# SpectacularAI/3dgs-deblur

Hardware: AMD Instinct MI355X
Metric: fwd+bwd rasterize MPix/s at 1M Gaussians, 1080p, 5 sub-poses (higher is better)
Workload: dtype f32

## Files before the change

### 3dgs-deblur_amd/csrc/binning.hip

```cpp
#include <algorithm>
#include <atomic>
#include "gs_common.h"

namespace gs {

constexpr int kScanItems = 8;
constexpr int kScanBlock = 256 * kScanItems;

__device__ __forceinline__ unsigned block_excl_scan(unsigned v, unsigned& total, unsigned* lds ) {
  const int lane = lane_id(), wave = threadIdx.x >> 6;
  unsigned inc = v;
#pragma unroll
  for (int o = 1; o < 64; o <<= 1) {
    unsigned t = __shfl_up(inc, o);
    if (lane >= o) inc += t;
  }
  if (lane == 63) lds[wave] = inc;
  __syncthreads();
  unsigned w0 = lds[0], w1 = lds[1], w2 = lds[2], w3 = lds[3];
  unsigned woff = wave == 0 ? 0u : (wave == 1 ? w0 : (wave == 2 ? w0 + w1 : w0 + w1 + w2));
  total = w0 + w1 + w2 + w3;
  __syncthreads();
  return woff + inc - v;
}
// ... 961 lines not shown
        Ellipse el2;
        el2.gx = s_gx[a]; el2.gy = s_gy[a]; el2.a = s_a[a]; el2.b = s_b[a]; el2.c = s_c[a]; el2.tau = s_tau[a];
        ellipse_derive(el2);
        if (!tile_hit(el2, tx, ty, W, H)) key = invalid_key;
      }
      keys[e] = key;
      vals[e] = s_gi[a];
    }
  }
}

template <typename KeyT, int SHIFT>
__global__ __launch_bounds__(256) void bin_edges_kernel(size_t n, const KeyT* __restrict__ keys,
                                                        int2* __restrict__ bins, unsigned num_bins,
                                                        const unsigned* __restrict__ n_dev = nullptr) {
  if (n_dev) n = min(n, (size_t)*n_dev);
  const int2 z = make_int2(0, 0);
  if (n == 0) {
    for (size_t b = (size_t)blockIdx.x * 256 + threadIdx.x; b < num_bins; b += (size_t)gridDim.x * 256) bins[b] = z;
    return;
  }
  const int lane = lane_id();
  for (size_t base = (size_t)blockIdx.x * 256 + (threadIdx.x & ~63u); base < n; base += (size_t)gridDim.x * 256) {
    const size_t i = base + lane;
    const bool valid = i < n;
    unsigned t = 0, lo = 0, hi = 0;
    if (valid) {
      t = min((unsigned)(keys[i] >> SHIFT), num_bins);
      if (i == 0) {
        if (t < num_bins) bins[t].x = 0;
        hi = t;
      } else {
        const unsigned tp = min((unsigned)(keys[i - 1] >> SHIFT), num_bins);
        if (tp != t) {
          if (t < num_bins) bins[t].x = (int)i;
          if (tp < num_bins) bins[tp].y = (int)i;
          lo = min(tp + 1u, num_bins); hi = t;
        }
      }
      if (i == n - 1 && t < num_bins) bins[t].y = (int)n;
    }
    unsigned long long m = __ballot(hi > lo);
    while (m) {
      const int src = __ffsll((long long)m) - 1;
      m &= m - 1;
      const unsigned g_lo = (unsigned)readlane_i((int)lo, src), g_hi = (unsigned)readlane_i((int)hi, src);
      for (unsigned b = g_lo + lane; b < g_hi; b += 64) bins[b] = z;
    }
    const unsigned long long last = __ballot(valid && i == n - 1);
    if (last) {
      const unsigned g_lo = min((unsigned)readlane_i((int)t, __ffsll((long long)last) - 1) + 1u, num_bins);
      for (unsigned b = g_lo + lane; b < num_bins; b += 64) bins[b] = z;
    }
  }
}

__global__ __launch_bounds__(256) void bin_edges_ids_kernel(size_t n, const unsigned* __restrict__ keys,
                                                            int2* __restrict__ bins,
                                                            const unsigned* __restrict__ sorted_vals,
                                                            const unsigned* __restrict__ gi_of_e,
                                                            unsigned* __restrict__ ids) {
  size_t i = (size_t)blockIdx.x * 256 + threadIdx.x;
  if (i >= n) {
    if (i < n + 8) ids[i] = 0u;
    return;
  }
  ids[i] = gi_of_e[sorted_vals[i]];
  unsigned t = keys[i];
  if (i == 0) {
    bins[t].x = 0;
  } else {
    unsigned tp = keys[i - 1];
    if (tp != t) { bins[t].x = (int)i; bins[tp].y = (int)i; }
  }
  if (i == n - 1) bins[t].y = (int)n;
}


__global__ void slice_plan_kernel(int P, int N, int K, const unsigned* __restrict__ cum,
                                  const unsigned* __restrict__ total, unsigned long long base,
                                  int* __restrict__ bounds, unsigned* __restrict__ rels,
                                  unsigned* __restrict__ seg_totals, const unsigned* __restrict__ n_live,
                                  unsigned* __restrict__ tail ,
                                  const unsigned* __restrict__ grand ) {
  int i = blockIdx.x * blockDim.x + threadIdx.x;
  if (i >= P * K) return;
  const int p = i / K, k = i % K;
  const unsigned* c = cum + (size_t)p * N;
  const unsigned long long tgt = base << k;
  const unsigned c0 = c[0];
  const int M = n_live ? (int)min((unsigned)N, n_live[p]) : N;
  int lo = 0, hi = M;
  while (lo < hi) {
    int mid = (lo + hi) >> 1;
    if ((unsigned long long)(unsigned)(c[mid] - c0) >= tgt) hi = mid; else lo = mid + 1;
  }
  bounds[i] = lo;
  const unsigned seg_end = (p + 1 < P) ? c[N] : *total;
  rels[i] = (lo < M ? c[lo] : seg_end) - c0;
  if (k == 0 && seg_totals) seg_totals[p] = seg_end - c0;
  if (tail) {
    if (k == 0) tail[p] = (unsigned)M;
    if (i == 0) tail[P] = grand ? *grand : *total;
  }
}

__global__ __launch_bounds__(256) void tile_sat_kernel(int tiles_x, int tiles_y, const unsigned char* __restrict__ done,
                                                       int* __restrict__ sat, unsigned long long* __restrict__ open_bits,
                                                       const int* __restrict__ gate) {
  extern __shared__ int s[];
  if (gate && *gate == 0) return;
  const int p = blockIdx.x;
  const int T = tiles_x * tiles_y, SW = tiles_x + 1, SH = tiles_y + 1;
  const unsigned char* d = done + (size_t)p * T;
  if (open_bits) {
    const int W64 = (tiles_x + 63) >> 6;
    for (int i = threadIdx.x; i < tiles_y * W64; i += 256) {
      const int y = i / W64, w = i - y * W64;
      unsigned long long m = 0ull;
      for (int b = 0; b < 64; ++b) {
        const int x = w * 64 + b;
        if (x < tiles_x && d[y * tiles_x + x] == 0) m |= 1ull << b;
      }
      open_bits[((size_t)p * tiles_y + y) * W64 + w] = m;
    }
  }
  for (int i = threadIdx.x; i < SW * SH; i += 256) {
    int y = i / SW, x = i % SW;
    s[i] = (y > 0 && x > 0) ? (d[(y - 1) * tiles_x + (x - 1)] ? 0 : 1) : 0;
  }
  __syncthreads();
  for (int y = threadIdx.x; y < SH; y += 256) {
    int run = 0;
    for (int x = 0; x < SW; ++x) { run += s[y * SW + x]; s[y * SW + x] = run; }
  }
  __syncthreads();
  for (int x = threadIdx.x; x < SW; x += 256) {
    int run = 0;
    for (int y = 0; y < SH; ++y) { run += s[y * SW + x]; s[y * SW + x] = run; }
  }
  __syncthreads();
  int* o = sat + (size_t)p * SW * SH;
  for (int i = threadIdx.x; i < SW * SH; i += 256) o[i] = s[i];
}

__global__ __launch_bounds__(256) void slice_counts_kernel(int n_slice, SliceDesc sd, int N, int tiles_x, int tiles_y,
                                                           const unsigned* __restrict__ sorted_gi,
                                                           const float* __restrict__ records,
                                                           const int* __restrict__ sat,
                                                           unsigned* __restrict__ slice_gi,
                                                           unsigned* __restrict__ counts) {
  int j = blockIdx.x * 256 + threadIdx.x;
  if (j >= n_slice) return;
  unsigned gi = sorted_gi[slice_rank(sd, j)];
  const float* rec = records + (size_t)gi * kRecFloats;
  unsigned lo = (unsigned)__float_as_int(rec[10]), hi = (unsigned)__float_as_int(rec[11]);
  int x0 = lo & 0xFFFF, y0 = lo >> 16, x1 = hi & 0xFFFF, y1 = hi >> 16;
  unsigned c = (unsigned)((x1 - x0) * (y1 - y0));
  if (sat && c) {
    const int SW = tiles_x + 1;
    const int* s = sat + (size_t)(gi / (unsigned)N) * SW * (tiles_y + 1);
    c = (unsigned)(s[y1 * SW + x1] - s[y0 * SW + x1] - s[y1 * SW + x0] + s[y0 * SW + x0]);
  }
  slice_gi[j] = gi;
  counts[j] = c;
}

constexpr int kCountSolo = 12;
constexpr int kCountSoloMax = 64;
constexpr int kCountSoloMany = 4;
constexpr int kCountMidMax = 256;
constexpr int kMaskWords = 512;

__device__ __forceinline__ unsigned long long row_window(const unsigned long long* __restrict__ row, int x0, int w) {
  const int wi = x0 >> 6, sh = x0 & 63;
  unsigned long long v = row[wi] >> sh;
  if (sh && sh + w > 64) v |= row[wi + 1] << (64 - sh);
  return w == 64 ? v : (v & ((1ull << w) - 1ull));
}

struct SweepP { const float* pix_vel; float t_min, t_max, rs_time; };

template <bool WAVE_PER_G, bool SWEEP = false>
__global__ __launch_bounds__(256) void slice_counts_exact_kernel(int n_slice, SliceDesc sd, int N, int tiles_x,
                                                                 int tiles_y, const unsigned* __restrict__ sorted_gi,
                                                                 const float* __restrict__ records,
                                                                 const int* __restrict__ sat,
                                                                 const unsigned char* __restrict__ done,
                                                                 int W, int H, unsigned* __restrict__ slice_gi,
                                                                 unsigned* __restrict__ counts,
                                                                 const unsigned* __restrict__ cum_rank,
                                                                 unsigned long long* __restrict__ masks,
                                                                 unsigned* __restrict__ mask_off,
                                                                 const unsigned long long* __restrict__ open_bits,
                                                                 const int* __restrict__ gate, SweepP sw) {
  __shared__ unsigned long long s_words[4][kMaskWords];
  __shared__ unsigned long long s_mid[WAVE_PER_G ? 1 : 4][256];
  const int lane = lane_id();
  const int j = WAVE_PER_G ? (lane == 0 ? (int)(blockIdx.x * 4 + (threadIdx.x >> 6)) : n_slice)
                           : (int)(blockIdx.x * 256 + threadIdx.x);
  if (gate && *gate == 0) {
    if (j < n_slice) counts[j] = 0u;
    return;
  }
  unsigned gi = 0, lo = 0, hi = 0, moff = 0;
  int area = 0;
  Ellipse el = {0.f, 0.f, 1.f, 0.f, 1.f, -1.f, 1.f, 1.f, 0.f, 0.f, 0.f};
  if (j < n_slice) {
    const int rank = slice_rank(sd, j);
    gi = sorted_gi[rank];
    if (masks) { moff = (cum_rank[rank] >> 6) + (unsigned)j; mask_off[j] = moff; }
    const float* rec = records + (size_t)gi * kRecFloats;
    lo = (unsigned)__float_as_int(rec[10]); hi = (unsigned)__float_as_int(rec[11]);
    const int x0 = lo & 0xFFFF, y0 = lo >> 16, x1 = hi & 0xFFFF, y1 = hi >> 16;
    area = (x1 - x0) * (y1 - y0);
    if (area > 0 && sat) {
      const int SW = tiles_x + 1;
      const int* s = sat + (size_t)(gi / (unsigned)N) * SW * (tiles_y + 1);
      if (s[y1 * SW + x1] - s[y0 * SW + x1] - s[y1 * SW + x0] + s[y0 * SW + x0] == 0) area = 0;
    }
    if (area > 0) el = make_ellipse(rec);
    if (el.tau < 0.f) area = 0;
    if (SWEEP && area > 0) {
      const unsigned g = gi % (unsigned)N;
      el.pvx = sw.pix_vel[2 * (size_t)g]; el.pvy = sw.pix_vel[2 * (size_t)g + 1];
      el.st0 = sw.t_min; el.st1 = sw.t_max; el.srs = sw.rs_time;
    }
  }
  const unsigned T = (unsigned)(tiles_x * tiles_y);
  const int W64 = (tiles_x + 63) >> 6;
  unsigned cnt = 0;
  const int solo_limit =
      (!WAVE_PER_G && __popcll(__ballot(area > kCountSolo && area <= kCountSoloMax)) >= kCountSoloMany) ? kCountSoloMax
                                                                                                       : kCountSolo;
  const int box_w = (int)(hi & 0xFFFF) - (int)(lo & 0xFFFF);
  const bool mid_box = !WAVE_PER_G && area > solo_limit && area <= kCountMidMax && box_w <= 64;
  const bool mid = mid_box && __popcll(__ballot(mid_box)) >= kCountSoloMany;
  if (area > 0 && (area <= solo_limit || mid)) {
    const int x0 = lo & 0xFFFF, y0 = lo >> 16, x1 = hi & 0xFFFF, y1 = hi >> 16;
    const int w = x1 - x0;
    const unsigned pidx = gi / (unsigned)N;
    unsigned long long m = 0ull;
    unsigned long long* mw = &s_mid[0][threadIdx.x];
    if (mid) { mw[0] = 0ull; mw[256] = 0ull; mw[512] = 0ull; mw[768] = 0ull; }
    auto put = [&](int y, unsigned long long rowbits) {
      cnt += (unsigned)__popcll(rowbits);
      const int bit0 = (y - y0) * w;
      if (!mid) { m |= rowbits << bit0; return; }
      const int wi = bit0 >> 6, sh = bit0 & 63;
      mw[wi * 256] |= rowbits << sh;
      if (sh && (rowbits >> (64 - sh))) mw[(wi + 1) * 256] |= rowbits >> (64 - sh);
    };
    if (open_bits) {
      const int wi = x0 >> 6, sh = x0 & 63, wi1 = min(wi + 1, W64 - 1);
      const unsigned long long wmask = w == 64 ? ~0ull : ((1ull << w) - 1ull);
      const unsigned long long* base = open_bits + (size_t)pidx * tiles_y * W64;
      for (int yb = y0; yb < y1; yb += 4) {
        unsigned long long a[4], b[4];
#pragma unroll
        for (int k = 0; k < 4; ++k) {
          const unsigned long long* row = base + (size_t)min(yb + k, y1 - 1) * W64;
          a[k] = row[wi]; b[k] = row[wi1];
        }
#pragma unroll
        for (int k = 0; k < 4; ++k) {
          const int y = yb + k;
          if (y >= y1) break;
          int t0, t1;
          span_tiles(el, row_span<SWEEP>(el, y, H), x0, x1, t0, t1);
          if (t1 <= t0) continue;
          unsigned long long rowbits = (t1 - t0 >= 64 ? ~0ull : ((1ull << (t1 - t0)) - 1ull)) << (t0 - x0);
          unsigned long long win = a[k] >> sh;
          if (sh && sh + w > 64) win |= b[k] << (64 - sh);
          rowbits &= win & wmask;
          if (rowbits) put(y, rowbits);
        }
      }
    } else {
      for (int y = y0; y < y1; ++y) {
        int t0, t1;
        span_tiles(el, row_span<SWEEP>(el, y, H), x0, x1, t0, t1);
        if (t1 <= t0) continue;
        put(y, (t1 - t0 >= 64 ? ~0ull : ((1ull << (t1 - t0)) - 1ull)) << (t0 - x0));
      }
    }
    if (masks) {
      if (!mid) masks[moff] = m;
      else {
        const int nwords = (area + 63) >> 6;
        for (int k = 0; k < nwords; ++k) masks[moff + (unsigned)k] = mw[k * 256];
      }
    }
  }
  unsigned long long big = __ballot(area > solo_limit && !mid);
  unsigned long long* words = s_words[threadIdx.x >> 6];
  while (big) {
    const int src = __ffsll((long long)big) - 1;
    big &= big - 1;
    const unsigned g = (unsigned)readlane_i((int)gi, src);
    const unsigned l = (unsigned)readlane_i((int)lo, src), h = (unsigned)readlane_i((int)hi, src);
    Ellipse eg;
    eg.gx = readlane_f(el.gx, src); eg.gy = readlane_f(el.gy, src); eg.a = readlane_f(el.a, src);
    eg.b = readlane_f(el.b, src); eg.c = readlane_f(el.c, src); eg.tau = readlane_f(el.tau, src);
    ellipse_derive(eg);
    if (SWEEP) {
      eg.pvx = readlane_f(el.pvx, src); eg.pvy = readlane_f(el.pvy, src);
      eg.st0 = sw.t_min; eg.st1 = sw.t_max; eg.srs = sw.rs_time;
    }
    const int x0 = l & 0xFFFF, y0 = l >> 16, x1 = h & 0xFFFF, y1 = h >> 16;
    const int w = x1 - x0, rows = y1 - y0, a = w * rows;
    const unsigned pidx = g / (unsigned)N;
    const unsigned mo = (unsigned)readlane_i((int)moff, src);
    const int nwords = (a + 63) >> 6;
    unsigned c = 0;
    if (nwords <= kMaskWords) {
      __builtin_amdgcn_wave_barrier();
      for (int k = lane; k < nwords; k += 64) words[k] = 0ull;
      __builtin_amdgcn_wave_barrier();
      for (int r = lane; r < rows; r += 64) {
        int t0, t1;
        span_tiles(eg, row_span<SWEEP>(eg, y0 + r, H), x0, x1, t0, t1);
        const unsigned long long* orow = open_bits ? open_bits + ((size_t)pidx * tiles_y + (y0 + r)) * W64 : nullptr;
        for (int c0 = 0; c0 < w; c0 += 64) {
          const int cw = min(64, w - c0);
          const int lo_c = max(t0 - x0 - c0, 0), hi_c = min(t1 - x0 - c0, cw);
          if (hi_c <= lo_c) continue;
          unsigned long long bits = (hi_c - lo_c == 64 ? ~0ull : ((1ull << (hi_c - lo_c)) - 1ull)) << lo_c;
          if (orow) bits &= row_window(orow, x0 + c0, cw);
          if (!bits) continue;
          const int bit0 = r * w + c0;
          const int wi = bit0 >> 6, sh = bit0 & 63;
          atomicOr(&words[wi], bits << sh);
          if (sh && (bits >> (64 - sh))) atomicOr(&words[wi + 1], bits >> (64 - sh));
        }
      }
      __builtin_amdgcn_wave_barrier();
      for (int k = lane; k < nwords; k += 64) {
        const unsigned long long m = words[k];
        if (masks) masks[mo + (unsigned)k] = m;
        c += (unsigned)__popcll(m);
      }
      c = (unsigned)wave_sum_i((int)c);
    } else {
      const float rw = 1.0f / (float)w;
      const unsigned pbase = pidx * T;
      for (int base = 0; base < a; base += 64) {
        const int t = base + lane;
        bool ok = false;
        if (t < a) {
          const int q = (int)(((float)t + 0.5f) * rw);
          const int tx = x0 + (t - q * w), ty = y0 + q;
          ok = tile_hit<SWEEP>(eg, tx, ty, W, H) && (!done || done[pbase + (unsigned)(ty * tiles_x + tx)] == 0);
        }
        const unsigned long long m = __ballot(ok);
        if (masks && lane == 0) masks[mo + (unsigned)(base >> 6)] = m;
        c += (unsigned)__popcll(m);
      }
    }
    if (lane == src) cnt = c;
  }
  if (j < n_slice) { slice_gi[j] = gi; counts[j] = cnt; }
}

template <bool WAVE_PER_G>
__global__ __launch_bounds__(256) void emit_open_kernel(int n_slice, int N, int T, int tiles_x,
                                                        const unsigned* __restrict__ slice_gi,
                                                        const unsigned* __restrict__ counts,
                                                        const unsigned* __restrict__ cum,
                                                        const float* __restrict__ records,
                                                        const unsigned char* __restrict__ done,
                                                        unsigned* __restrict__ keys, unsigned* __restrict__ vals,
                                                        int W, int H, unsigned invalid_key, int compact,
                                                        const unsigned long long* __restrict__ masks,
                                                        const unsigned* __restrict__ mask_off,
                                                        unsigned char* __restrict__ tile_hot) {
  const int lane = lane_id();
  const int j = WAVE_PER_G ? (lane == 0 ? (int)(blockIdx.x * 4 + (threadIdx.x >> 6)) : n_slice)
                           : (int)(blockIdx.x * 256 + threadIdx.x);
  unsigned cnt = 0, gi = 0, e0 = 0, lo = 0, hi = 0, moff = 0;
  int hot = 0;
  Ellipse el = {0.f, 0.f, 1.f, 0.f, 1.f, -1.f, 1.f, 1.f, 0.f, 0.f, 0.f};
  if (j < n_slice) {
    cnt = counts[j];
    if (cnt) {
      gi = slice_gi[j];
      e0 = cum[j];
      const float* rec = records + (size_t)gi * kRecFloats;
      lo = (unsigned)__float_as_int(rec[10]);
      hi = (unsigned)__float_as_int(rec[11]);
      hot = (tile_hot != nullptr && rec[5] > K::kAlphaMax) ? 1 : 0;
      if (masks) moff = mask_off[j];
      else if (invalid_key) el = make_ellipse(rec);
    }
  }
  if (masks && !WAVE_PER_G) {
    const int x0 = lo & 0xFFFF, y0 = lo >> 16, x1 = hi & 0xFFFF, y1 = hi >> 16;
    const int w = x1 - x0, area = w * (y1 - y0);
    const bool small = cnt != 0 && area <= kCountSoloMax;
    if (__popcll(__ballot(small)) >= kCountSoloMany) {
      if (small) {
        unsigned long long m = masks[moff];
        const float rw = 1.0f / (float)w;
        const unsigned pbase = (gi / (unsigned)N) * (unsigned)T;
        unsigned e = e0;
        while (m) {
          const int b = __ffsll((long long)m) - 1;
          m &= m - 1;
          const int q = (int)(((float)b + 0.5f) * rw);
          const unsigned k = pbase + (unsigned)((y0 + q) * tiles_x + x0 + (b - q * w));
          keys[e] = k;
          vals[e] = gi;
          if (hot) tile_hot[k] = 1;
          ++e;
        }
        cnt = 0;
      }
    }
  }
  unsigned long long todo = __ballot(cnt != 0);
  const unsigned long long lt_mask = (1ull << lane) - 1ull;
  while (todo) {
    const int src = __ffsll((long long)todo) - 1;
    todo &= todo - 1;
    const unsigned g = (unsigned)readlane_i((int)gi, src);
    unsigned e = (unsigned)readlane_i((int)e0, src);
    const unsigned l = (unsigned)readlane_i((int)lo, src), h = (unsigned)readlane_i((int)hi, src);
    Ellipse eg;
    eg.gx = readlane_f(el.gx, src); eg.gy = readlane_f(el.gy, src); eg.a = readlane_f(el.a, src);
    eg.b = readlane_f(el.b, src); eg.c = readlane_f(el.c, src); eg.tau = readlane_f(el.tau, src);
    ellipse_derive(eg);
    const int x0 = l & 0xFFFF, y0 = l >> 16, x1 = h & 0xFFFF, y1 = h >> 16;
    const int w = x1 - x0, area = w * (y1 - y0);
    const float rw = 1.0f / (float)w;
    const unsigned pbase = (g / (unsigned)N) * (unsigned)T;
    const bool hot_g = readlane_i(hot, src) != 0;
    if (masks) {
      const unsigned mo = (unsigned)readlane_i((int)moff, src);
      for (int base = 0; base < area; base += 64) {
        const unsigned long long m = masks[mo + (unsigned)(base >> 6)];
        if ((m >> lane) & 1ull) {
          const int t = base + lane;
          const int q = (int)(((float)t + 0.5f) * rw);
          const int tx = x0 + (t - q * w), ty = y0 + q;
          const unsigned dst = e + (unsigned)__popcll(m & lt_mask);
          const unsigned k = pbase + (unsigned)(ty * tiles_x + tx);
          keys[dst] = k;
          vals[dst] = g;
          if (hot_g) tile_hot[k] = 1;
        }
        e += (unsigned)__popcll(m);
      }
      continue;
    }
    for (int base = 0; base < area; base += 64) {
      const int t = base + lane;
      bool open = false;
      unsigned k = 0;
      if (t < area) {
        const int q = (int)(((float)t + 0.5f) * rw);
        const int tx = x0 + (t - q * w), ty = y0 + q;
        k = pbase + (unsigned)(ty * tiles_x + tx);
        open = !done || done[k] == 0;
        if (open && invalid_key && !tile_hit(eg, tx, ty, W, H)) {
          if (compact) open = false;
          else k = invalid_key;
        }
      }
      const unsigned long long m = __ballot(open);
      if (open) {
        const unsigned dst = e + (unsigned)__popcll(m & lt_mask);
        keys[dst] = k;
        vals[dst] = g;
        if (hot_g && (invalid_key == 0u || k != invalid_key)) tile_hot[k] = 1;
      }
      e += (unsigned)__popcll(m);
    }
  }
}

constexpr int kSelBits = 11, kSelBins = 1 << kSelBits;
struct SelSeg {
  unsigned long long hist[2][kSelBins];
};

__device__ __forceinline__ unsigned long long block_excl_scan64(unsigned long long v, unsigned long long& total,
                                                               unsigned long long* lds ) {
  const int lane = lane_id(), wave = threadIdx.x >> 6;
  unsigned long long inc = v;
#pragma unroll
  for (int o = 1; o < 64; o <<= 1) {
    const unsigned long long t = __shfl_up(inc, o);
    if (lane >= o) inc += t;
  }
  if (lane == 63) lds[wave] = inc;
  __syncthreads();
  const unsigned long long w0 = lds[0], w1 = lds[1], w2 = lds[2], w3 = lds[3];
  const unsigned long long woff = wave == 0 ? 0ull : (wave == 1 ? w0 : (wave == 2 ? w0 + w1 : w0 + w1 + w2));
  total = w0 + w1 + w2 + w3;
  __syncthreads();
  return woff + inc - v;
}

__device__ __forceinline__ unsigned sel_crossing(const unsigned long long* __restrict__ hist, unsigned long long target,
                                                 unsigned long long* s_scan , unsigned long long* s_res ,
                                                 unsigned long long& before, unsigned long long& total) {
  constexpr int PER = kSelBins / 256;
  if (threadIdx.x == 0) { s_res[0] = (unsigned long long)kSelBins; s_res[1] = 0ull; }
  unsigned long long c[PER], sum = 0ull;
#pragma unroll
  for (int j = 0; j < PER; ++j) { c[j] = hist[threadIdx.x * PER + j]; sum += c[j]; }
  unsigned long long run = block_excl_scan64(sum, total, s_scan);
#pragma unroll
  for (int j = 0; j < PER; ++j) {
    if (run < target && run + c[j] >= target) { s_res[0] = (unsigned long long)(threadIdx.x * PER + j); s_res[1] = run; }
    run += c[j];
  }
  __syncthreads();
  before = s_res[1];
  const unsigned found = (unsigned)s_res[0];
  __syncthreads();
  return found;
}

constexpr int kSelRounds = 8;
template <int LEVEL>
__global__ __launch_bounds__(256) void depth_hist_kernel(size_t seg_len, const unsigned* __restrict__ keys,
                                                         const unsigned* __restrict__ weights,
                                                         unsigned long long budget, SelSeg* __restrict__ ws) {
  __shared__ unsigned long long h[kSelBins];
  __shared__ unsigned long long s_scan[8], s_res[2];
  const unsigned seg = blockIdx.y;
  SelSeg& S = ws[seg];
  unsigned b1 = 0;
  if (LEVEL == 1) {
    unsigned long long before, total;
    b1 = sel_crossing(S.hist[0], budget, s_scan, s_res, before, total);
    if (b1 >= (unsigned)kSelBins) return;
  }
  for (int d = threadIdx.x; d < kSelBins; d += 256) h[d] = 0ull;
  __syncthreads();
  const size_t seg_base = (size_t)seg * seg_len, limit = seg_base + seg_len;
  for (size_t base = seg_base + (size_t)blockIdx.x * (256 * kSelRounds); base < limit;
       base += (size_t)gridDim.x * (256 * kSelRounds)) {
    unsigned k[kSelRounds], w[kSelRounds];
#pragma unroll
    for (int r = 0; r < kSelRounds; ++r) {
      const size_t i = base + (size_t)r * 256 + threadIdx.x;
      k[r] = keys[min(i, limit - 1)];
      if (i >= limit) k[r] = 0xFFFFFFFFu;
    }
#pragma unroll
    for (int r = 0; r < kSelRounds; ++r) {
      const size_t i = base + (size_t)r * 256 + threadIdx.x;
      const bool ok = (k[r] >> 31) == 0u && (LEVEL == 0 || (k[r] >> 20) == b1);
      w[r] = ok ? weights[min(i, limit - 1)] : 0u;
// ... 162 lines not shown
}

GS_EXPORT int gs_make_depth_keys64(long long n, int N, const unsigned* depth_keys, unsigned long long* out,
                                   void* stream) {
  if (n <= 0 || N <= 0) return GS_ERR_INVALID;
  hipLaunchKernelGGL(depth_keys64_kernel, dim3((unsigned)((n + 255) / 256)), dim3(256), 0, (hipStream_t)stream,
                     (size_t)n, N, depth_keys, out);
  return gs_launch_status();
}

GS_EXPORT int gs_gather_counts(long long n, const unsigned* sorted_gi, const int* num_tiles_hit, unsigned* counts_out,
                               void* stream) {
  if (n <= 0) return GS_ERR_INVALID;
  hipLaunchKernelGGL(gather_counts_kernel, dim3((unsigned)((n + 255) / 256)), dim3(256), 0, (hipStream_t)stream,
                     (size_t)n, sorted_gi, num_tiles_hit, counts_out);
  return gs_launch_status();
}

GS_EXPORT int gs_emit_intersects(long long n_ranked, int N, int H, int W, const unsigned* sorted_gi,
                                 const unsigned* cum_excl, const float* records, long long n_isect, unsigned* keys,
                                 unsigned* vals, unsigned invalid_key, void* stream) {
  if (n_ranked <= 0 || N <= 0) return GS_ERR_INVALID;
  if (n_isect <= 0) return GS_OK;
  int tiles_x = (W + K::kTile - 1) / K::kTile, tiles_y = (H + K::kTile - 1) / K::kTile;
  hipLaunchKernelGGL(emit_kernel, dim3((unsigned)((n_isect + kEmitChunk - 1) / kEmitChunk)), dim3(256), 0,
                     (hipStream_t)stream, (size_t)n_ranked, N, tiles_x * tiles_y, tiles_x, sorted_gi, cum_excl, records,
                     (size_t)n_isect, keys, vals, W, H, invalid_key);
  return gs_launch_status();
}

GS_EXPORT int gs_tile_bin_edges_u32(long long n, const unsigned* sorted_keys, int num_bins, int* bins,
                                    const unsigned* n_dev, void* stream) {
  if (num_bins <= 0) return GS_ERR_INVALID;
  if (n <= 0) {
    hipError_t e = hipMemsetAsync(bins, 0, (size_t)num_bins * 2 * sizeof(int), (hipStream_t)stream);
    return e == hipSuccess ? GS_OK : 1000 + (int)e;
  }
  unsigned blocks = (unsigned)((n + 255) / 256);
  if (n_dev && blocks > 8192u) blocks = 8192u;
  hipLaunchKernelGGL((bin_edges_kernel<unsigned, 0>), dim3(blocks), dim3(256), 0,
                     (hipStream_t)stream, (size_t)n, sorted_keys, reinterpret_cast<int2*>(bins), (unsigned)num_bins, n_dev);
  return gs_launch_status();
}

GS_EXPORT int gs_tile_bin_edges_ids_u32(long long n, const unsigned* sorted_keys, int num_bins, int* bins,
                                        const unsigned* sorted_vals, const unsigned* gi_of_e, unsigned* ids_out,
                                        void* stream) {
  if (num_bins <= 0 || !sorted_vals || !gi_of_e || !ids_out) return GS_ERR_INVALID;
  hipError_t e = hipMemsetAsync(bins, 0, (size_t)num_bins * 2 * sizeof(int), (hipStream_t)stream);
  if (e != hipSuccess) return 1000 + (int)e;
  if (n < 0) return GS_ERR_INVALID;
  hipLaunchKernelGGL(bin_edges_ids_kernel, dim3((unsigned)((n + 8 + 255) / 256)), dim3(256), 0, (hipStream_t)stream,
                     (size_t)n, sorted_keys, reinterpret_cast<int2*>(bins), sorted_vals, gi_of_e, ids_out);
  return gs_launch_status();
}

GS_EXPORT int gs_tile_bin_edges_u64(long long n, const unsigned long long* sorted_ids, int num_bins, int* bins,
                                    void* stream) {
  if (num_bins <= 0) return GS_ERR_INVALID;
  if (n <= 0) {
    hipError_t e = hipMemsetAsync(bins, 0, (size_t)num_bins * 2 * sizeof(int), (hipStream_t)stream);
    return e == hipSuccess ? GS_OK : 1000 + (int)e;
  }
  hipLaunchKernelGGL((bin_edges_kernel<unsigned long long, 32>), dim3((unsigned)((n + 255) / 256)), dim3(256), 0,
                     (hipStream_t)stream, (size_t)n, sorted_ids, reinterpret_cast<int2*>(bins), (unsigned)num_bins);
  return gs_launch_status();
}

GS_EXPORT int gs_map_gaussian_to_intersects(int N, const float* xys, const float* depths, const int* radii,
                                            const int* cum_tiles_hit, int H, int W, long long* isect_ids,
                                            int* gaussian_ids, void* stream) {
  if (N <= 0) return GS_ERR_INVALID;
  int tiles_x = (W + K::kTile - 1) / K::kTile, tiles_y = (H + K::kTile - 1) / K::kTile;
  hipLaunchKernelGGL(map_isect_kernel, dim3((N + 255) / 256), dim3(256), 0, (hipStream_t)stream, N, xys, depths,
                     radii, cum_tiles_hit, tiles_x, tiles_y, isect_ids, gaussian_ids);
  return gs_launch_status();
}

GS_EXPORT int gs_slice_plan(int P, int N, int K, const unsigned* cum_excl, const unsigned* total, long long base,
                            int* bounds, unsigned* rels, unsigned* seg_totals, const unsigned* n_live,
                            unsigned* tail, void* stream) {
  if (P <= 0 || N <= 0 || K <= 0 || K > 32 || base <= 0) return GS_ERR_INVALID;
  hipLaunchKernelGGL(slice_plan_kernel, dim3((P * K + 63) / 64), dim3(64), 0, (hipStream_t)stream, P, N, K, cum_excl,
                     total, (unsigned long long)base, bounds, rels, seg_totals, n_live, tail, (const unsigned*)nullptr);
  return gs_launch_status();
}

GS_EXPORT int gs_slice_plan_select(int P, int N, int K, const unsigned* cum_excl, const unsigned* total, int* bounds,
                                   unsigned* rels, unsigned* seg_totals, const unsigned* n_live, unsigned* tail,
                                   const unsigned* grand, void* stream) {
  if (P <= 0 || N <= 0 || K <= 0 || K > 32 || !n_live || !grand) return GS_ERR_INVALID;
  hipLaunchKernelGGL(slice_plan_kernel, dim3((P * K + 63) / 64), dim3(64), 0, (hipStream_t)stream, P, N, K, cum_excl,
                     total, 1ull << 40, bounds, rels, seg_totals, n_live, tail, grand);
  return gs_launch_status();
}

GS_EXPORT long long gs_depth_select_workspace_bytes(int segments) {
  return segments > 0 ? (long long)segments * (long long)sizeof(SelSeg) + 256 : 0;
}

GS_EXPORT int gs_depth_select(long long n, long long seg_len, const unsigned* keys, const unsigned* weights,
                              long long budget, unsigned* thr_out, unsigned* grand_out, void* ws, long long ws_bytes,
                              void* stream) {
  if (n <= 0 || seg_len <= 0 || n % seg_len != 0 || budget <= 0 || !keys || !weights || !thr_out || !ws)
    return GS_ERR_INVALID;
  const long long segs = n / seg_len;
  if (segs > 65535) return GS_ERR_INVALID;
  if (ws_bytes < gs_depth_select_workspace_bytes((int)segs)) return GS_ERR_WORKSPACE;
  const long long chunks = (seg_len + 256 * kSelRounds - 1) / (256 * kSelRounds);
  const unsigned gx = (unsigned)std::max(1ll, std::min((chunks + 1) / 2, std::max(1ll, 1024 / segs)));
  SelSeg* S = reinterpret_cast<SelSeg*>(ws);
  hipLaunchKernelGGL(depth_hist_kernel<0>, dim3(gx, (unsigned)segs), dim3(256), 0, (hipStream_t)stream, (size_t)seg_len,
                     keys, weights, (unsigned long long)budget, S);
  hipLaunchKernelGGL(depth_hist_kernel<1>, dim3(gx, (unsigned)segs), dim3(256), 0, (hipStream_t)stream, (size_t)seg_len,
                     keys, weights, (unsigned long long)budget, S);
  hipLaunchKernelGGL(depth_find_kernel, dim3((unsigned)segs), dim3(256), 0, (hipStream_t)stream,
                     (unsigned long long)budget, S, thr_out, grand_out);
  return gs_launch_status();
}

GS_EXPORT int gs_segmented_sort_select_u32(long long n, long long seg_len, const unsigned* keys_src, unsigned* keys0,
                                           unsigned* vals0, unsigned* keys1, unsigned* vals1, int begin_bit, int end_bit,
                                           int max_digit_bits, unsigned skip_key, const unsigned* key_lo,
                                           const unsigned* key_hi, unsigned* seg_counts, const unsigned* gather_src,
                                           unsigned* gather_out, void* ws, long long ws_bytes, int* result_buf,
                                           long long tail_cap, void* stream) {
  if (n <= 0 || seg_len <= 0 || n % seg_len != 0 || begin_bit < 0 || end_bit > 32 || !seg_counts || !keys_src ||
      tail_cap < 0)
    return GS_ERR_INVALID;
  if ((gather_src != nullptr) != (gather_out != nullptr)) return GS_ERR_INVALID;
  return radix_sort<unsigned>((size_t)n, (size_t)seg_len, keys0, vals0, keys1, vals1, 1, begin_bit, end_bit, ws,
                              (size_t)ws_bytes, result_buf, (hipStream_t)stream, max_digit_bits, gather_src,
                              gather_out, nullptr, seg_counts, (unsigned long long)skip_key, nullptr, nullptr, nullptr,
                              nullptr, keys_src, key_lo, key_hi,
                              tail_cap > 0 ? (unsigned)((tail_cap + sort_block_keys<unsigned>() - 1) / sort_block_keys<unsigned>()) : 0u);
}

GS_EXPORT int gs_tile_open_sat(int P, int H, int W, const unsigned char* tile_done, int* sat,
                               unsigned long long* open_bits, const int* gate, void* stream) {
  if (P <= 0) return GS_ERR_INVALID;
  int tiles_x = (W + K::kTile - 1) / K::kTile, tiles_y = (H + K::kTile - 1) / K::kTile;
  size_t lds = (size_t)(tiles_x + 1) * (tiles_y + 1) * sizeof(int);
  if (lds > 160 * 1024) return GS_ERR_INVALID;
  if (lds > 48 * 1024)
    (void)hipFuncSetAttribute(reinterpret_cast<const void*>(tile_sat_kernel), hipFuncAttributeMaxDynamicSharedMemorySize,
                              (int)lds);
  hipLaunchKernelGGL(tile_sat_kernel, dim3(P), dim3(256), lds, (hipStream_t)stream, tiles_x, tiles_y, tile_done, sat,
                     open_bits, gate);
  return gs_launch_status();
}

GS_EXPORT int gs_slice_counts(int n_slice, int P, int N, const int* slice_begin, const int* slice_prefix,
                              const unsigned* sorted_gi, const float* records, const int* sat, int H, int W,
                              unsigned* slice_gi, unsigned* counts, void* stream) {
  SliceDesc sd;
  if (n_slice <= 0 || !make_slice_desc(P, slice_begin, slice_prefix, sd)) return GS_ERR_INVALID;
  int tiles_x = (W + K::kTile - 1) / K::kTile, tiles_y = (H + K::kTile - 1) / K::kTile;
  hipLaunchKernelGGL(slice_counts_kernel, dim3((n_slice + 255) / 256), dim3(256), 0, (hipStream_t)stream, n_slice, sd,
                     N, tiles_x, tiles_y, sorted_gi, records, sat, slice_gi, counts);
  return gs_launch_status();
}

GS_EXPORT int gs_slice_counts_exact(int n_slice, int P, int N, const int* slice_begin, const int* slice_prefix,
                                    const unsigned* sorted_gi, const float* records, const int* sat,
                                    const unsigned char* tile_done, int H, int W, unsigned* slice_gi,
                                    unsigned* counts, int wave_per_gaussian, const unsigned* cum_rank,
                                    unsigned long long* hit_masks, unsigned* mask_off,
                                    const unsigned long long* open_bits, const int* gate, void* stream) {
  SliceDesc sd;
  if (n_slice <= 0 || !make_slice_desc(P, slice_begin, slice_prefix, sd)) return GS_ERR_INVALID;
  if (hit_masks && (!cum_rank || !mask_off)) return GS_ERR_INVALID;
  if ((tile_done != nullptr) != (open_bits != nullptr)) return GS_ERR_INVALID;
  int tiles_x = (W + K::kTile - 1) / K::kTile, tiles_y = (H + K::kTile - 1) / K::kTile;
  const SweepP none{nullptr, 0.f, 0.f, 0.f};
  if (wave_per_gaussian)
    hipLaunchKernelGGL(slice_counts_exact_kernel<true>, dim3((n_slice + 3) / 4), dim3(256), 0, (hipStream_t)stream,
                       n_slice, sd, N, tiles_x, tiles_y, sorted_gi, records, sat, tile_done, W, H, slice_gi, counts,
                       cum_rank, hit_masks, mask_off, open_bits, gate, none);
  else
    hipLaunchKernelGGL(slice_counts_exact_kernel<false>, dim3((n_slice + 255) / 256), dim3(256), 0,
                       (hipStream_t)stream, n_slice, sd, N, tiles_x, tiles_y, sorted_gi, records, sat, tile_done, W,
                       H, slice_gi, counts, cum_rank, hit_masks, mask_off, open_bits, gate, none);
  return gs_launch_status();
}

GS_EXPORT int gs_slice_counts_exact_swept(int n_slice, int P, int N, const int* slice_begin, const int* slice_prefix,
                                          const unsigned* sorted_gi, const float* records, const int* sat,
                                          const unsigned char* tile_done, int H, int W, unsigned* slice_gi,
                                          unsigned* counts, int wave_per_gaussian, const unsigned* cum_rank,
                                          unsigned long long* hit_masks, unsigned* mask_off,
                                          const unsigned long long* open_bits, const float* pix_vel, float t_min,
                                          float t_max, float rolling_shutter_time, void* stream) {
  SliceDesc sd;
  if (n_slice <= 0 || N <= 0 || !pix_vel || !hit_masks || !cum_rank || !mask_off ||
      !make_slice_desc(P, slice_begin, slice_prefix, sd))
    return GS_ERR_INVALID;
  if ((tile_done != nullptr) != (open_bits != nullptr)) return GS_ERR_INVALID;
  int tiles_x = (W + K::kTile - 1) / K::kTile, tiles_y = (H + K::kTile - 1) / K::kTile;
  const SweepP sw{pix_vel, fminf(t_min, t_max), fmaxf(t_min, t_max), rolling_shutter_time};
  if (wave_per_gaussian)
    hipLaunchKernelGGL((slice_counts_exact_kernel<true, true>), dim3((n_slice + 3) / 4), dim3(256), 0, (hipStream_t)stream,
                       n_slice, sd, N, tiles_x, tiles_y, sorted_gi, records, sat, tile_done, W, H, slice_gi, counts,
                       cum_rank, hit_masks, mask_off, open_bits, (const int*)nullptr, sw);
  else
    hipLaunchKernelGGL((slice_counts_exact_kernel<false, true>), dim3((n_slice + 255) / 256), dim3(256), 0,
                       (hipStream_t)stream, n_slice, sd, N, tiles_x, tiles_y, sorted_gi, records, sat, tile_done, W,
                       H, slice_gi, counts, cum_rank, hit_masks, mask_off, open_bits, (const int*)nullptr, sw);
  return gs_launch_status();
}

GS_EXPORT int gs_emit_open_intersects(int n_slice, int N, int H, int W, const unsigned* slice_gi,
                                      const unsigned* counts, const unsigned* cum_excl, const float* records,
                                      const unsigned char* tile_done, unsigned* keys, unsigned* vals,
                                      unsigned invalid_key, int compact, int wave_per_gaussian,
                                      const unsigned long long* hit_masks, const unsigned* mask_off,
                                      unsigned char* tile_hot, void* stream) {
  if (n_slice <= 0) return GS_ERR_INVALID;
  if (hit_masks && (!mask_off || !compact)) return GS_ERR_INVALID;
  int tiles_x = (W + K::kTile - 1) / K::kTile, tiles_y = (H + K::kTile - 1) / K::kTile;
  if (wave_per_gaussian)
    hipLaunchKernelGGL(emit_open_kernel<true>, dim3((n_slice + 3) / 4), dim3(256), 0, (hipStream_t)stream, n_slice, N,
                       tiles_x * tiles_y, tiles_x, slice_gi, counts, cum_excl, records, tile_done, keys, vals, W, H,
                       invalid_key, compact, hit_masks, mask_off, tile_hot);
  else
    hipLaunchKernelGGL(emit_open_kernel<false>, dim3((n_slice + 255) / 256), dim3(256), 0, (hipStream_t)stream, n_slice,
                       N, tiles_x * tiles_y, tiles_x, slice_gi, counts, cum_excl, records, tile_done, keys, vals, W, H,
                       invalid_key, compact, hit_masks, mask_off, tile_hot);
  return gs_launch_status();
}

GS_EXPORT const char* gs_version(void) { return "gsdeblur-hip 0.1 (gfx950, wave64)"; }
```

### 3dgs-deblur_amd/csrc/frame.hip

```cpp
#include <hip/hip_runtime.h>
#include <stdint.h>
#include <string.h>
#include <time.h>
#include <algorithm>
#include <atomic>
#include <mutex>
#include <vector>
#include "gs_internal.h"
#include "gs_math.h"

namespace {

constexpr int kTile = gs::K::kTile;
constexpr int kKMax = GS_FRAME_MAX_SLICES;
constexpr int kIdsPad = 8;

struct Arena {
  char* base;
  long long cap, off;
  bool ok;
  Arena(void* b, long long c, long long start = 0) : base((char*)b), cap(c), off(start), ok(true) {}
  static long long up(long long x) { return (x + 255) & ~255ll; }
  template <typename T> T* take(long long count) {
    const long long a = up(off), bytes = count * (long long)sizeof(T);
    if (!ok || a + bytes > cap) { ok = false; off = a + bytes; return nullptr; }
    off = a + bytes;
    return reinterpret_cast<T*>(base + a);
  }
  long long offset_of(const void* p) const { return p ? (long long)((const char*)p - base) : -1; }
};

inline int bits_for(long long n) {
  int b = 1;
  while ((1ll << b) < std::max(2ll, n)) ++b;
  return b;
}

inline int hip_status(hipError_t e) { return e == hipSuccess ? GS_OK : 1000 + (int)e; }

struct StageEvents { int stage; hipEvent_t a, b; };
std::atomic<unsigned> g_profile_mask{0};
std::mutex g_profile_mu;
std::vector<StageEvents> g_events;
std::vector<StageEvents> g_pool;

struct StageScope {
  hipStream_t st;
  bool on;
  StageEvents ev;
  StageScope(int stage, hipStream_t s) : st(s), on((g_profile_mask.load(std::memory_order_relaxed) >> stage) & 1u) {
    if (!on) return;
    bool have = false;
    {
      std::lock_guard<std::mutex> lk(g_profile_mu);
      if (!g_pool.empty()) { ev = g_pool.back(); g_pool.pop_back(); have = true; }
    }
    if (!have) { (void)hipEventCreate(&ev.a); (void)hipEventCreate(&ev.b); }
    ev.stage = stage;
    (void)hipEventRecord(ev.a, st);
  }
  ~StageScope() {
    if (!on) return;
    (void)hipEventRecord(ev.b, st);
    std::lock_guard<std::mutex> lk(g_profile_mu);
    g_events.push_back(ev);
  }
};

constexpr long long kPollTimeoutUs = 50000;

__global__ __launch_bounds__(256) void publish_words_kernel(const unsigned* __restrict__ src, unsigned* dst, int n,
                                                            unsigned seq) {
  for (int i = threadIdx.x; i < n; i += 256)
    __hip_atomic_store(dst + 1 + i, src[i], __ATOMIC_RELAXED, __HIP_MEMORY_SCOPE_SYSTEM);
  __threadfence_system();
  __syncthreads();
  if (threadIdx.x == 0) __hip_atomic_store(dst, seq, __ATOMIC_RELEASE, __HIP_MEMORY_SCOPE_SYSTEM);
}

inline long long now_us() {
  timespec ts;
  clock_gettime(CLOCK_MONOTONIC, &ts);
  return (long long)ts.tv_sec * 1000000ll + ts.tv_nsec / 1000;
}

__global__ void and_tile_done_kernel(int S, int T, const unsigned char* __restrict__ done_s, unsigned char* __restrict__ done) {
  const int t = blockIdx.x * blockDim.x + threadIdx.x;
  if (t >= T) return;
  unsigned char a = 1;
  for (int s = 0; s < S; ++s) a &= done_s[(size_t)s * T + t] != 0;
  done[t] = a;
}

inline void cpu_relax() {
#if defined(__x86_64__) || defined(__i386__)
  __builtin_ia32_pause();
#elif defined(__aarch64__)
  asm volatile("yield" ::: "memory");
#else
  asm volatile("" ::: "memory");
#endif
}

template <class Between>
inline int read_back(const unsigned* src_dev, unsigned* host_pinned, int n, bool poll, hipStream_t st, Between between) {
  if (!poll) {
    hipError_t e = hipMemcpyAsync(host_pinned + 1, src_dev, 4ll * n, hipMemcpyDeviceToHost, st);
    if (e != hipSuccess) return 1000 + (int)e;
    int rb = between();
    if (rb != GS_OK) return rb;
    return hip_status(hipStreamSynchronize(st));
  }
  volatile unsigned* seqw = host_pinned;
  *seqw = 0u;
  __atomic_thread_fence(__ATOMIC_SEQ_CST);
  hipLaunchKernelGGL(publish_words_kernel, dim3(1), dim3(256), 0, st, src_dev, host_pinned, n, 1u);
  hipError_t e = hipGetLastError();
  if (e != hipSuccess) return 1000 + (int)e;
  int rb = between();
  if (rb != GS_OK) return rb;
  const long long t0 = now_us();
  unsigned spins = 0;
  while (__atomic_load_n(host_pinned, __ATOMIC_ACQUIRE) != 1u) {
    cpu_relax();
    if ((++spins & 1023u) == 0 && now_us() - t0 > kPollTimeoutUs) {
      int r = hip_status(hipStreamSynchronize(st));
      if (r != GS_OK) return r;
      return __atomic_load_n(host_pinned, __ATOMIC_ACQUIRE) == 1u ? GS_OK : GS_ERR_INVALID;
    }
  }
  return GS_OK;
}

inline int read_back(const unsigned* src_dev, unsigned* host_pinned, int n, bool poll, hipStream_t st) {
  return read_back(src_dev, host_pinned, n, poll, st, [] { return GS_OK; });
}

#define CHECK(call)            \
  do {                         \
    int _st = (call);          \
    if (_st != GS_OK) return _st; \
  } while (0)

}

enum { ST_DEPTH_SORT = 0, ST_COUNT_SCAN, ST_PLAN, ST_COUNT, ST_EMIT, ST_TILE_SORT, ST_BIN_EDGES, ST_RASTER_FWD, ST_SAT,
       ST_RASTER_BWD, ST_REDUCE, ST_N };

GS_EXPORT int gs_frame_profile_enable(unsigned stage_mask) {
  g_profile_mask.store(stage_mask, std::memory_order_relaxed);
  return GS_OK;
}

GS_EXPORT int gs_frame_profile_read(int max_events, int* stage_ids, float* ms) {
  int n = 0;
  std::lock_guard<std::mutex> lk(g_profile_mu);
  for (StageEvents& e : g_events) {
    if (n < max_events && stage_ids && ms) {
      (void)hipEventSynchronize(e.b);
      float t = 0.f;
      (void)hipEventElapsedTime(&t, e.a, e.b);
      stage_ids[n] = e.stage;
      ms[n] = t;
      ++n;
    }
    g_pool.push_back(e);
  }
  g_events.clear();
  return n;
}

static long long slice_bytes(const gs_frame_desc& d, long long n_k, long long I_k, bool masks, long long true_total) {
  const long long P = d.P, T = (long long)((d.W + kTile - 1) / kTile) * ((d.H + kTile - 1) / kTile);
  long long b = 0;
  auto add = [&](long long bytes) { b = Arena::up(b) + bytes; };
  if (n_k > 0) {
    add(4 * n_k); add(4 * n_k);
    if (masks) { add(8 * (true_total / 64 + n_k + 2)); add(4 * n_k); }
    add(4 * n_k); add(4); add(gs_scan_workspace_bytes(n_k));
  }
  if (I_k > 0) {
    add(4 * I_k); add(4 * (I_k + kIdsPad));
    add(4 * (I_k + kIdsPad)); add(4 * I_k); add(4 * (I_k + kIdsPad));
    add(4 * (I_k + kIdsPad)); add(4 * (I_k + kIdsPad));
    add(gs_radix_sort_workspace_bytes(I_k, 0, bits_for(P * T + 1)));
    add(8 * (P * T + 1));
  } else {
    add(4); add(8 * (d.shared_list ? (long long)d.S : P) * T);
  }
  add(4ll * d.S * d.H * d.W);
  return Arena::up(b) + 256;
}

GS_EXPORT long long gs_frame_backward_bytes(const gs_frame_state* state) {
  if (!state) return 0;
  long long maxI = 0;
  for (int k = 0; k < state->n_slices; ++k) maxI = std::max(maxI, state->slice[k].I);
  const long long tpe = state->shared_list ? state->S : 1;
  long long b = Arena::up(48 * maxI * tpe) + Arena::up(maxI * tpe) + 512;
  if (state->n_slices > 1) b += 2 * Arena::up(4ll * state->S * state->H * state->W);
  return b;
}

GS_EXPORT int gs_frame_forward(const gs_frame_desc* dp, float* records, unsigned* depth_keys, const int* num_tiles_hit,
                               const float* background, const int* band_edges, const unsigned char* band_tile_done,
                               const float* color_means, const float* color_sh, const float* color_sh_rest, int color_K,
                               int color_degree,
                               const float* color_viewmats, const float* pix_vel, const float* sample_times,
                               float* out_img, float* out_T,
                               float* out_depth, float* out_combined, void* arena_ptr, long long arena_bytes, void* host_pinned, long long host_pinned_bytes,
                               gs_frame_state* state, void* stream_) {
  if (!dp || !records || !depth_keys || !num_tiles_hit || !background || !band_edges || !out_img || !out_T ||
      !arena_ptr || !host_pinned || !state)
    return GS_ERR_INVALID;
  const gs_frame_desc d = *dp;
  const bool shared = d.shared_list != 0;
  if (d.N <= 0 || d.P <= 0 || d.S <= 0 || d.R <= 0 || d.H <= 0 || d.W <= 0 || d.P > 256 || d.S > 256) return GS_ERR_INVALID;
  if (shared ? (d.P != 1 || d.R != 1 || !pix_vel || !sample_times) : (d.P != d.S * d.R)) return GS_ERR_INVALID;
  if (d.R > 1 && !band_tile_done) return GS_ERR_INVALID;
  if ((long long)d.S * d.H * d.W >= (1ll << 30)) return GS_ERR_INVALID;
  const int cams = d.cameras > 1 ? d.cameras : 1;
  if (cams > 1 && (d.S % cams != 0 || shared || pix_vel)) return GS_ERR_INVALID;
  const bool rs = pix_vel != nullptr && (d.rolling_shutter_time != 0.f || shared);
  if (rs && d.R != 1) return GS_ERR_INVALID;
  const gs_project_inputs* lazy = d.lazy_records;
  if (lazy && (pix_vel || shared)) return GS_ERR_INVALID;
  hipStream_t st = (hipStream_t)stream_;
  const int P = d.P, N = d.N, S = d.S, R = d.R, H = d.H, W = d.W;
  const long long n = (long long)P * N;
  const int tx = (W + kTile - 1) / kTile, ty = (H + kTile - 1) / kTile;
  const long long T = (long long)tx * ty;
  const long long plan_ints = 2ll * P * kKMax + 2 * P + 1;
  if (host_pinned_bytes < 4 * (plan_ints + 1) + 64) return GS_ERR_INVALID;
  memset(state, 0, sizeof(*state));
  state->P = P; state->N = N; state->S = S; state->R = R; state->H = H; state->W = W;
  state->cameras = cams;
  state->rolling_shutter_time = rs ? d.rolling_shutter_time : 0.f;
  state->shared_list = shared ? 1 : 0;
  Arena A(arena_ptr, arena_bytes);

  const bool planned = d.slice_base > 0;
  const bool select = planned && d.depth_select != 0;
  unsigned* k0s = select ? A.take<unsigned>(n) : nullptr;
  unsigned* v0 = A.take<unsigned>(n);
  unsigned* k1 = A.take<unsigned>(n);
  unsigned* v1 = A.take<unsigned>(n);
  unsigned* counts_r = A.take<unsigned>(n);
  unsigned* n_live = A.take<unsigned>(P);
  const int digit = d.depth_sort_digit >= 8 && d.depth_sort_digit <= 11 ? d.depth_sort_digit : 8;
  const long long sort_ws_b = gs_segmented_sort_compact_workspace_bytes(n, N, 0, 31, digit);
  char* sort_ws = A.take<char>(sort_ws_b);
  unsigned* cum = A.take<unsigned>(n);
  unsigned* total = A.take<unsigned>(1);
  const long long scan_ws_b = gs_scan_workspace_bytes(n);
  char* scan_ws = A.take<char>(scan_ws_b);
  float* live_T = A.take<float>((long long)S * H * W);
  int* sat = A.take<int>((long long)P * (ty + 1) * (tx + 1));
  const long long w64 = (tx + 63) / 64;
  unsigned long long* open_bits = A.take<unsigned long long>((long long)P * ty * w64);
  const long long sel_b = select ? Arena::up(gs_depth_select_workspace_bytes(P)) + 256 : 0;
  const long long flag_off = ((1 + kKMax) * P * T + 3) & ~3ll;
  char* zero_blk = A.take<char>(sel_b + flag_off + 4 * kKMax);
  unsigned char* zeros_u8 = reinterpret_cast<unsigned char*>(zero_blk) + sel_b;
  unsigned* sel_grand = select ? reinterpret_cast<unsigned*>(zero_blk + sel_b - 256) : nullptr;
  unsigned* thr_dev = select ? A.take<unsigned>(P) : nullptr;
  int* plan_dev = A.take<int>(plan_ints);
  unsigned char* tile_done_rs = R > 1 ? A.take<unsigned char>(P * T) : nullptr;
  unsigned char* tile_done_samples = shared ? A.take<unsigned char>((long long)S * T) : nullptr;
  if (!A.ok) { state->arena_required = 2 * A.off; return GS_ERR_WORKSPACE; }
  if (shared) CHECK(hip_status(hipMemsetAsync(tile_done_samples, 0, (long long)S * T, st)));
  CHECK(hip_status(hipMemsetAsync(zero_blk, 0, sel_b + flag_off + 4 * kKMax, st)));
  int* open_flags = reinterpret_cast<int*>(zeros_u8 + flag_off);
  const long long plan_tiles = (d.band_clipped && R > 1) ? (T + R - 1) / R : T;
  const long long base0 = plan_tiles * (long long)std::max(1, d.slice_base);

  const unsigned* sorted_gi = nullptr;
  bool bound_known = false;
  auto presort = [&](int phase, long long tail_cap) -> int {
    int res = 0;
    {
      StageScope sc(ST_DEPTH_SORT, st);
      if (!select) {
        CHECK(gs_segmented_sort_compact_u32(n, N, depth_keys, v0, k1, v1, 0, 31, digit, 0xFFFFFFFFu, n_live,
                                            reinterpret_cast<const unsigned*>(num_tiles_hit), counts_r, sort_ws, sort_ws_b,
                                            &res, st));
      } else {
        if (phase == 0 && !bound_known) {
          CHECK(gs_depth_select(n, N, depth_keys, reinterpret_cast<const unsigned*>(num_tiles_hit), base0, thr_dev,
                                sel_grand, zero_blk, sel_b - 256, st));
          bound_known = true;
        }
        CHECK(gs_segmented_sort_select_u32(n, N, depth_keys, k0s, v0, k1, v1, 0, 31, digit, 0xFFFFFFFFu,
                                           phase == 0 ? nullptr : thr_dev, phase == 0 ? thr_dev : nullptr, n_live,
                                           reinterpret_cast<const unsigned*>(num_tiles_hit), counts_r, sort_ws, sort_ws_b,
                                           &res, phase == 0 ? tail_cap : 0, st));
      }
    }
    sorted_gi = res == 1 ? v1 : v0;
    StageScope sc(ST_COUNT_SCAN, st);
    CHECK(gs_exclusive_scan_segments_u32(n, N, n_live, counts_r, cum, total, scan_ws, scan_ws_b, st));
    return GS_OK;
  };
  long long tail_cap = (select && d.select_cap > 0) ? (long long)d.select_cap : 0;
  CHECK(presort(0, tail_cap));

  unsigned* hp = reinterpret_cast<unsigned*>(host_pinned) + 1;
  unsigned* hp_seq = reinterpret_cast<unsigned*>(host_pinned);
  const bool poll = d.poll_readback != 0;
  const long long PK = (long long)P * kKMax;
  std::vector<long long> NV(P), seg_totals(P);
  std::vector<std::vector<long long>> bnd(P), rel(P);
  long long n_total = 0, true_total = 0;
  int K = 1;
  bool use_masks = false, rs_exact = false;
  std::vector<std::vector<int>> begins, prefixes;
  std::vector<long long> n_of, I_of;
  auto make_plan = [&](int phase) -> int {
    if (planned) {
      StageScope sc(ST_PLAN, st);
      if (select && phase == 0)
        CHECK(gs_slice_plan_select(P, N, kKMax, cum, total, plan_dev, reinterpret_cast<unsigned*>(plan_dev + PK),
                                   reinterpret_cast<unsigned*>(plan_dev + 2 * PK), n_live,
                                   reinterpret_cast<unsigned*>(plan_dev + 2 * PK + P), sel_grand, st));
      else
        CHECK(gs_slice_plan(P, N, kKMax, cum, total, phase == 0 ? base0 : 2 * base0, plan_dev,
                            reinterpret_cast<unsigned*>(plan_dev + PK), reinterpret_cast<unsigned*>(plan_dev + 2 * PK),
                            n_live, reinterpret_cast<unsigned*>(plan_dev + 2 * PK + P), st));
      CHECK(read_back(reinterpret_cast<const unsigned*>(plan_dev), hp_seq, (int)plan_ints, poll, st));
      for (int p = 0; p < P; ++p) {
        bnd[p].resize(kKMax); rel[p].resize(kKMax);
        for (int k = 0; k < kKMax; ++k) { bnd[p][k] = hp[p * kKMax + k]; rel[p][k] = hp[PK + p * kKMax + k]; }
        seg_totals[p] = hp[2 * PK + p];
        NV[p] = std::min<long long>(N, hp[2 * PK + P + p]);
      }
      if (phase == 0) n_total = hp[plan_ints - 1];
      const int k_cap = phase == 0 ? kKMax : kKMax - 1;
      K = k_cap;
      for (int k = 0; k < k_cap; ++k) {
        bool all = true;
        for (int p = 0; p < P; ++p) all = all && bnd[p][k] >= NV[p];
        if (all) { K = k + 1; break; }
      }
    } else {
      CHECK(hip_status(hipMemcpyAsync(hp, total, 4, hipMemcpyDeviceToHost, st)));
      CHECK(hip_status(hipMemcpyAsync(hp + 1, n_live, 4 * P, hipMemcpyDeviceToHost, st)));
      CHECK(hip_status(hipStreamSynchronize(st)));
      n_total = hp[0];
      for (int p = 0; p < P; ++p) { NV[p] = std::min<long long>(N, hp[1 + p]); seg_totals[p] = 0; }
      K = 1;
    }
    true_total = 0;
    for (int p = 0; p < P; ++p) true_total += seg_totals[p];
    use_masks = planned && true_total < 4294967296ll - 64;
    rs_exact = rs && use_masks;
    if (rs && !rs_exact) use_masks = false;
    begins.assign(K, std::vector<int>(P));
    prefixes.assign(K, std::vector<int>(P + 1));
    n_of.assign(K, 0); I_of.assign(K, 0);
    for (int k = 0; k < K; ++k) {
      prefixes[k][0] = 0;
      long long I_k = 0;
      for (int p = 0; p < P; ++p) {
        const long long lo = k == 0 ? 0 : std::min(bnd[p].empty() ? NV[p] : bnd[p][k - 1], NV[p]);
        const long long hi = (k == K - 1) ? NV[p] : std::min(bnd[p][k], NV[p]);
        begins[k][p] = (int)((long long)p * N + lo);
        prefixes[k][p + 1] = prefixes[k][p] + (int)std::max(0ll, hi - lo);
        if (planned) {
          const long long hi_rel = (k == K - 1) ? seg_totals[p] : rel[p][k];
          const long long lo_rel = k == 0 ? 0 : rel[p][k - 1];
          I_k += (hi_rel - lo_rel) & 0xFFFFFFFFll;
        }
      }
      n_of[k] = prefixes[k][P];
      I_of[k] = planned ? I_k : n_total;
      if (n_of[k] == 0) I_of[k] = 0;
    }
    return GS_OK;
  };
  CHECK(make_plan(0));
  if (tail_cap > 0) {
    long long most = 0;
    for (int p = 0; p < P; ++p) most = std::max(most, NV[p]);
    if (most > tail_cap) {
      state->select_overflow = 1;
      CHECK(presort(0, 0));
      CHECK(make_plan(0));
    }
  }
  for (int p = 0; p < P; ++p) state->max_selected = std::max<long long>(state->max_selected, select ? NV[p] : 0);
  state->n_total = n_total;
  state->depth_select = select ? 1 : 0;
  state->open_after_first = -1.f;
  bool rest_behind = select && ((n_total - true_total) & 0xFFFFFFFFll) != 0;

  long long maxI_issued = 0;
  auto fits = [&](long long n_s, long long I_s, int k_next) -> bool {
    if (I_s >= 2147483647ll - kIdsPad) return false;
    const long long mI = std::max(maxI_issued, I_s);
    const long long tpe = shared ? S : 1;
    const long long bwd = d.reserve_backward ? Arena::up(48 * mI * tpe) + Arena::up(mI * tpe) + 2 * Arena::up(4ll * S * H * W) + 1024 : 0;
    const long long need = Arena::up(A.off) + slice_bytes(d, n_s, I_s, use_masks, true_total) + bwd;
    if (need <= arena_bytes) return true;
    state->arena_required = need + (k_next < K && I_of[k_next] < 2147483647ll
                                        ? slice_bytes(d, n_of[k_next], I_of[k_next], use_masks, true_total) + 49 * I_of[k_next]
                                        : 0);
    return false;
  };
  auto merged = [&](int k0, int k1, std::vector<int>& beg, std::vector<int>& pre, long long& n_s, long long& I_s) {
    beg = begins[k0];
    pre.assign(P + 1, 0);
    I_s = 0;
    for (int p = 0; p < P; ++p) {
      int cnt = 0;
      for (int k = k0; k < k1; ++k) cnt += prefixes[k][p + 1] - prefixes[k][p];
      pre[p + 1] = pre[p] + cnt;
    }
    for (int k = k0; k < k1; ++k) I_s += I_of[k];
    n_s = pre[P];
    if (n_s == 0) I_s = 0;
  };

  unsigned char* tile_done = zeros_u8;
  const bool holes0 = R > 1;
  if (R > 1) {
    tile_done = tile_done_rs;
    CHECK(hip_status(hipMemcpyAsync(tile_done, band_tile_done, P * T, hipMemcpyDeviceToDevice, st)));
    CHECK(gs_tile_open_sat(P, H, W, tile_done, sat, open_bits, nullptr, st));
  }
  const unsigned invalid_key = rs ? 0u : (unsigned)(P * T);
  const int key_bits = bits_for(P * T + 1);
  int n_out = 0;
  int span = 1;
  long long open_before = (long long)S * T;
  std::vector<int> beg_s, pre_s;
  int slice_no = 0;
  bool lazy_done = false;
  for (int phase = 0; phase < 2; ++phase) {
  long long open_left = 0;
  for (int k = 0, k1 = 0; k < K; k = k1, ++slice_no) {
    long long n_k = 0, I_k = 0;
    k1 = std::min(K, k + span);
    merged(k, k1, beg_s, pre_s, n_k, I_k);
    while (k1 > k + 1 && I_k >= 2147483647ll - kIdsPad) merged(k, --k1, beg_s, pre_s, n_k, I_k);
    const bool first = slice_no == 0, last = k1 == K && !(phase == 0 && rest_behind);
    if (I_k >= 2147483647ll - kIdsPad) return GS_ERR_INVALID;
    if (shared && I_k * (long long)S >= 4294967296ll) return GS_ERR_INVALID;
    if (!fits(n_k, I_k, k1)) return GS_ERR_WORKSPACE;
    maxI_issued = std::max(maxI_issued, I_k);
    unsigned *slice_gi = nullptr, *counts = nullptr, *cum_k = nullptr, *total_k = nullptr, *mask_off = nullptr;
    unsigned long long* masks = nullptr;
    unsigned *vals = nullptr, *svals = nullptr, *sorted_ids = nullptr;
    int* bins = nullptr;
    unsigned char* tile_hot = zeros_u8 + (1 + slice_no) * P * T;
    int wave_per_g = 0;
    if (n_k > 0) {
      StageScope sc(ST_COUNT, st);
      slice_gi = A.take<unsigned>(n_k);
      counts = A.take<unsigned>(n_k);
      const bool have_holes = !first || holes0;
      long long box_total = 0;
      if (first) {
        if (!planned) box_total = n_total;
        else if (K == 1) box_total = true_total;
        else for (int p = 0; p < P; ++p) box_total += rel[p][0];
      }
      wave_per_g = (first && box_total > 128 * n_k) ? 1 : 0;
      if (use_masks) {
        masks = A.take<unsigned long long>(true_total / 64 + n_k + 2);
        mask_off = A.take<unsigned>(n_k);
      }
      cum_k = A.take<unsigned>(n_k);
      total_k = A.take<unsigned>(1);
      const long long ws_b = gs_scan_workspace_bytes(n_k);
      char* ws = A.take<char>(ws_b);
      if (!A.ok) { state->arena_required = 2 * A.off; return GS_ERR_WORKSPACE; }
      if (lazy && !lazy_done) {
        if (slice_no == 0)
          CHECK(gs_slice_project_records((int)n_k, P, N, beg_s.data(), pre_s.data(), sorted_gi, lazy, H, W, records, st));
        else {
          CHECK(gs_project_records(P, N, lazy, H, W, records, st));
          lazy_done = true;
        }
      }
      if (rs_exact)
        CHECK(gs_slice_counts_exact_swept((int)n_k, P, N, beg_s.data(), pre_s.data(), sorted_gi, records,
                                          have_holes ? sat : nullptr, have_holes ? tile_done : nullptr, H, W, slice_gi,
                                          counts, wave_per_g, cum, masks, mask_off, have_holes ? open_bits : nullptr,
                                          pix_vel, shared ? d.sweep_t_min : 0.f, shared ? d.sweep_t_max : 0.f,
                                          d.rolling_shutter_time, st));
      else if (rs)
        CHECK(gs_slice_counts((int)n_k, P, N, beg_s.data(), pre_s.data(), sorted_gi, records,
                              have_holes ? sat : nullptr, H, W, slice_gi, counts, st));
      else
        CHECK(gs_slice_counts_exact((int)n_k, P, N, beg_s.data(), pre_s.data(), sorted_gi, records,
                                    have_holes ? sat : nullptr, have_holes ? tile_done : nullptr, H, W, slice_gi, counts,
                                    wave_per_g, masks ? cum : nullptr, masks, mask_off, have_holes ? open_bits : nullptr,
                                    nullptr, st));
      CHECK(gs_exclusive_scan_u32(n_k, counts, cum_k, total_k, ws, ws_b, st));
      if (color_means && color_sh && color_viewmats)
        CHECK(gs_slice_colors((int)n_k, slice_gi, counts, N, color_means, color_sh, color_sh_rest, color_K, color_degree,
                              color_viewmats, records, st));
    }
    if (I_k > 0) {
      unsigned* keys = A.take<unsigned>(I_k);
      vals = A.take<unsigned>(I_k + kIdsPad);
      unsigned* s_v0 = A.take<unsigned>(I_k + kIdsPad);
      unsigned* s_k1 = A.take<unsigned>(I_k);
      unsigned* s_v1 = A.take<unsigned>(I_k + kIdsPad);
      unsigned* pa = A.take<unsigned>(I_k + kIdsPad);
      unsigned* pb = A.take<unsigned>(I_k + kIdsPad);
      const long long ws_b = gs_radix_sort_workspace_bytes(I_k, 0, key_bits);
      char* ws = A.take<char>(ws_b);
      bins = A.take<int>(2 * (P * T + 1));
      if (!A.ok) { state->arena_required = 2 * A.off; return GS_ERR_WORKSPACE; }
      {
        StageScope sc(ST_EMIT, st);
        if (rs && !rs_exact && first && !holes0)
          CHECK(gs_emit_intersects(n_k, N, H, W, slice_gi, cum_k, records, I_k, keys, vals, invalid_key, st));
        else
          CHECK(gs_emit_open_intersects((int)n_k, N, H, W, slice_gi, counts, cum_k, records,
                                        (!first || holes0) ? tile_done : nullptr, keys, vals, invalid_key,
                                        (rs && !rs_exact) ? 0 : 1, wave_per_g, masks, mask_off, rs ? nullptr : tile_hot, st));
      }
      int r1 = 0, r2 = 0;
      {
        StageScope sc(ST_TILE_SORT, st);
        CHECK(gs_radix_sort_pairs_carry_u32(I_k, keys, s_v0, s_k1, s_v1, 1, 0, key_bits, ws, ws_b, &r1, vals, pa, pb, &r2,
                                            total_k, st));
      }
      const unsigned* skeys = r1 == 1 ? s_k1 : keys;
      svals = r1 == 1 ? s_v1 : s_v0;
      sorted_ids = r2 == 1 ? pb : pa;
      {
        StageScope sc(ST_BIN_EDGES, st);
        CHECK(gs_tile_bin_edges_u32(I_k, skeys, (int)(P * T + 1), bins, total_k, st));
      }
    }
    if (I_k == 0 && !(first || last)) continue;
    if (I_k == 0) {
      const long long nb = (shared ? (long long)S : (long long)P) * T;
      svals = A.take<unsigned>(1 + kIdsPad);
      bins = A.take<int>(2 * nb);
      if (!A.ok) { state->arena_required = 2 * A.off; return GS_ERR_WORKSPACE; }
      CHECK(hip_status(hipMemsetAsync(svals, 0, 4 * (1 + kIdsPad), st)));
      CHECK(hip_status(hipMemsetAsync(bins, 0, 8 * nb, st)));
    }
    int* fidx = A.take<int>((long long)S * H * W);
    if (!A.ok) { state->arena_required = 2 * A.off; return GS_ERR_WORKSPACE; }
    const int fwd_variant = (I_k == 0 && d.fwd_variant == 3) ? 0 : d.fwd_variant;
    {
      StageScope sc(ST_RASTER_FWD, st);
      if (rs && I_k > 0)
        CHECK(gs_rasterize_fwd_rs_slice(records, bins, band_edges, background, S, H, W, out_img, out_T, live_T, fidx,
                                        shared ? tile_done_samples : tile_done, first ? 1 : 0, last ? 1 : 0,
                                        reinterpret_cast<const int*>(sorted_ids), (int)std::min(n, 2147483647ll), out_depth,
                                        last ? nullptr : open_flags + slice_no, pix_vel, N, d.rolling_shutter_time,
                                        shared ? sample_times : nullptr, st));
      else
      CHECK(gs_rasterize_fwd_slice(records, reinterpret_cast<const int*>(svals), bins, band_edges, background, S, R, H, W,
                                   out_img, out_T, live_T, fidx, shared ? tile_done_samples : tile_done, first ? 1 : 0,
                                   last ? 1 : 0, I_k > 0 ? reinterpret_cast<const int*>(vals) : nullptr,
                                   reinterpret_cast<const int*>(sorted_ids), I_k > 0 ? (int)std::min(n, 2147483647ll) : 0,
                                   I_k > 0 ? out_depth : nullptr, I_k > 0 ? tile_hot : nullptr,
                                   last ? nullptr : open_flags + slice_no, fwd_variant, st));
    }
    if (I_k > 0) {
      if (n_out >= GS_FRAME_MAX_SLICES) return GS_ERR_INVALID;
      gs_frame_slice& sl = state->slice[n_out++];
      sl.I = I_k; sl.n = (int)n_k; sl.wave_per_gaussian = wave_per_g; sl.first = first; sl.last = last;
      sl.svals = A.offset_of(svals); sl.bins = A.offset_of(bins); sl.fidx = A.offset_of(fidx);
      sl.gi_of_e = A.offset_of(vals); sl.sorted_ids = A.offset_of(sorted_ids); sl.slice_gi = A.offset_of(slice_gi);
      sl.counts = A.offset_of(counts); sl.cum = A.offset_of(cum_k); sl.tile_hot = A.offset_of(tile_hot);
      sl.n_emitted_dev = A.offset_of(total_k);
    }
    auto average = [&]() -> int {
      if (!out_combined) return GS_OK;
      if (cams > 1)
        return gs_combine_fwd_batched(cams, S / cams, 3ll * H * W, out_img, d.combine_gamma, d.combine_min_level,
                                      out_combined, st);
      return gs_combine_fwd(S, 3ll * H * W, out_img, d.combine_gamma, d.combine_min_level, out_combined, st);
    };
    if (last) CHECK(average());
    if (!last) {
      CHECK(read_back(reinterpret_cast<const unsigned*>(open_flags + slice_no), hp_seq, 1, poll, st, average));
      const long long open_now = hp[0];
      open_left = open_now;
      if (slice_no == 0) state->open_after_first = (float)((double)open_now / (double)((long long)S * T));
      if (open_now == 0) { ++slice_no; break; }
      span = (d.merge_open_fraction > 0.f && (double)open_now >= (double)d.merge_open_fraction * (double)open_before)
                 ? 2 * (k1 - k) : 1;
      open_before = open_now;
      StageScope sc(ST_SAT, st);
      if (shared)
        hipLaunchKernelGGL(and_tile_done_kernel, dim3((unsigned)((T + 255) / 256)), dim3(256), 0, st, S, (int)T,
                           tile_done_samples, tile_done);
      CHECK(gs_tile_open_sat(P, H, W, tile_done, sat, open_bits, nullptr, st));
    }
  }
  if (!(phase == 0 && rest_behind && open_left > 0)) break;
  state->depth_select = 2;
  rest_behind = false;
  span = 1;
  CHECK(presort(1, 0));
  CHECK(make_plan(1));
  }
  state->n_slices = n_out;
  state->arena_used = Arena::up(A.off);
  return GS_OK;
}

GS_EXPORT int gs_frame_backward_depth(const gs_frame_state* state, const float* records, const float* background,
                                      const int* band_edges, const float* out_T, const float* v_img, const float* v_alpha,
                                      const float* cmb_scale, float cmb_gamma, float cmb_min_level, int bwd_variant,
                                      float* v_records, unsigned char* touched, const float* pix_vel,
                                      const float* sample_times, void* arena_ptr, long long arena_bytes,
                                      const float* v_depth, void* stream_) {
  if (!state || !records || !background || !band_edges || !out_T || !v_img || !v_records || !arena_ptr)
    return GS_ERR_INVALID;
  hipStream_t st = (hipStream_t)stream_;
  const int S = state->S, R = state->R, H = state->H, W = state->W;
  const long long n_rec = (long long)state->P * state->N;
  Arena A(arena_ptr, arena_bytes, state->arena_used);
  char* base = (char*)arena_ptr;
  long long maxI = 0;
  for (int k = 0; k < state->n_slices; ++k) maxI = std::max(maxI, state->slice[k].I);
  float *bwd_T = nullptr, *bwd_B = nullptr;
  if (state->n_slices > 1) {
    bwd_T = A.take<float>((long long)S * H * W);
    bwd_B = A.take<float>((long long)S * H * W);
  }
  const bool shared = state->shared_list != 0;
  if (shared && (!pix_vel || !sample_times)) return GS_ERR_INVALID;
  if ((bwd_variant & GS_BWD_ABSGRAD) && (state->rolling_shutter_time != 0.f || shared)) return GS_ERR_INVALID;
  const long long tpe = shared ? S : 1;
  float* tuples = A.take<float>(12 * maxI * tpe);
  unsigned char* flags = A.take<unsigned char>((maxI * tpe + 15) & ~15ll);
  if (!A.ok) return GS_ERR_WORKSPACE;
  if (bwd_T) {
    CHECK(hip_status(hipMemcpyAsync(bwd_T, out_T, 4ll * S * H * W, hipMemcpyDeviceToDevice, st)));
    CHECK(hip_status(hipMemsetAsync(bwd_B, 0, 4ll * S * H * W, st)));
  }
  for (int k = state->n_slices - 1; k >= 0; --k) {
    const gs_frame_slice& sl = state->slice[k];
    CHECK(hip_status(hipMemsetAsync(flags, 0, (sl.I * tpe + 15) & ~15ll, st)));
    {
      StageScope sc(ST_RASTER_BWD, st);
      if (state->rolling_shutter_time != 0.f || shared) {
        if (!pix_vel) return GS_ERR_INVALID;
        CHECK(gs_rasterize_bwd_rs_slice_depth(records, reinterpret_cast<const int*>(base + sl.svals),
                                        reinterpret_cast<const int*>(base + sl.bins), band_edges, background, S, H, W, out_T,
                                        reinterpret_cast<const int*>(base + sl.fidx), v_img, v_alpha, bwd_T, bwd_B, tuples,
                                        flags, reinterpret_cast<const int*>(base + sl.sorted_ids),
                                        (int)std::min(n_rec, 2147483647ll), bwd_variant & GS_VARIANT_CLAMP_GRAD, cmb_scale, cmb_gamma,
                                        cmb_min_level, pix_vel, state->N, state->rolling_shutter_time,
                                        shared ? sample_times : nullptr, v_depth, st));
      } else
      CHECK(gs_rasterize_bwd_slice_depth(records, reinterpret_cast<const int*>(base + sl.svals),
                                   reinterpret_cast<const int*>(base + sl.bins), band_edges, background, S, R, H, W, out_T,
                                   reinterpret_cast<const int*>(base + sl.fidx), v_img, v_alpha, bwd_T, bwd_B, v_records,
                                   reinterpret_cast<const int*>(base + sl.gi_of_e), tuples, flags,
                                   reinterpret_cast<const int*>(base + sl.sorted_ids), (int)std::min(n_rec, 2147483647ll),
                                   reinterpret_cast<const unsigned char*>(base + sl.tile_hot), bwd_variant, cmb_scale,
                                   cmb_gamma, cmb_min_level, v_depth, state->cameras, st));
    }
    {
      StageScope sc(ST_REDUCE, st);
      CHECK(gs_reduce_grad_tuples_depth(sl.n, reinterpret_cast<const unsigned*>(base + sl.slice_gi),
                                  reinterpret_cast<const unsigned*>(base + sl.counts),
                                  reinterpret_cast<const unsigned*>(base + sl.cum), tuples, flags, v_records, touched,
                                  (sl.wave_per_gaussian || (R > 1 && sl.n < (1 << 19))) ? sl.I : 0, records, (int)tpe,
                                  v_depth != nullptr, st));
    }
  }
  return GS_OK;
}

GS_EXPORT int gs_frame_backward(const gs_frame_state* state, const float* records, const float* background,
                                const int* band_edges, const float* out_T, const float* v_img, const float* v_alpha,
                                const float* cmb_scale, float cmb_gamma, float cmb_min_level, int bwd_variant,
                                float* v_records, unsigned char* touched, const float* pix_vel,
                                const float* sample_times, void* arena_ptr, long long arena_bytes, void* stream_) {
  return gs_frame_backward_depth(state, records, background, band_edges, out_T, v_img, v_alpha, cmb_scale, cmb_gamma,
                                 cmb_min_level, bwd_variant, v_records, touched, pix_vel, sample_times, arena_ptr,
                                 arena_bytes, nullptr, stream_);
}
```

### 3dgs-deblur_amd/csrc/gs_common.h

```cpp
#pragma once
#include <hip/hip_runtime.h>
#include <stdint.h>
#include "gs_math.h"
#include "gs_internal.h"

namespace gs {

constexpr int kWave = 64;

__device__ __forceinline__ int lane_id() { return (int)(threadIdx.x & 63); }

template <int CTRL, int ROW_MASK>
__device__ __forceinline__ float dpp_add(float v) {
  int moved = __builtin_amdgcn_update_dpp(0, __float_as_int(v), CTRL, ROW_MASK, 0xf, false);
  return v + __int_as_float(moved);
}

__device__ __forceinline__ float wave_sum_to_lane63(float v) {
  v = dpp_add<0x111, 0xf>(v);
  v = dpp_add<0x112, 0xf>(v);
  v = dpp_add<0x114, 0xf>(v);
  v = dpp_add<0x118, 0xf>(v);
  v = dpp_add<0x142, 0xa>(v);
  v = dpp_add<0x143, 0xc>(v);
  return v;
}

__device__ __forceinline__ float wave_sum_uniform(float v) {
  v = wave_sum_to_lane63(v);
  return __int_as_float(__builtin_amdgcn_readlane(__float_as_int(v), 63));
}

__device__ __forceinline__ float readlane_f(float v, int l) {
  return __int_as_float(__builtin_amdgcn_readlane(__float_as_int(v), l));
}
__device__ __forceinline__ int readlane_i(int v, int l) { return __builtin_amdgcn_readlane(v, l); }

__device__ __forceinline__ int wave_sum_i(int v) {
#pragma unroll
  for (int o = 32; o > 0; o >>= 1) v += __shfl_xor(v, o);
  return v;
}

__device__ __forceinline__ int wave_max_i(int v) {
#pragma unroll
  for (int o = 32; o > 0; o >>= 1) {
    int t = __shfl_xor(v, o);
    v = v > t ? v : t;
  }
  return v;
}

__device__ __forceinline__ void atomic_add_f32(float* p, float v) {
  __hip_atomic_fetch_add(p, v, __ATOMIC_RELAXED, __HIP_MEMORY_SCOPE_AGENT);
}

__device__ __forceinline__ unsigned xcd_remap(unsigned b, unsigned n) {
  const unsigned X = 8;
  unsigned q = n / X, r = n % X;
  unsigned xcd = b % X, i = b / X;
  unsigned base = xcd < r ? xcd * (q + 1) : r * (q + 1) + (xcd - r) * q;
  return base + i;
}

constexpr int kMaxSubposes = 256;
struct SliceDesc {
  int begin[kMaxSubposes];
  int prefix[kMaxSubposes + 1];
  int P;
};

static inline bool make_slice_desc(int P, const int* begin, const int* prefix, SliceDesc& sd) {
  if (P <= 0 || P > kMaxSubposes || !begin || !prefix) return false;
  for (int p = 0; p < P; ++p) { sd.begin[p] = begin[p]; sd.prefix[p] = prefix[p]; }
  sd.prefix[P] = prefix[P];
  sd.P = P;
  return true;
}

__device__ __forceinline__ int slice_rank(const SliceDesc& sd, int j) {
  int p = 0;
  while (p + 1 < sd.P && j >= sd.prefix[p + 1]) ++p;
  return sd.begin[p] + (j - sd.prefix[p]);
}

}
```

### 3dgs-deblur_amd/csrc/gs_internal.h

```cpp
#pragma once
#include <hip/hip_runtime.h>
#include "../../include/gsdeblur.h"

#define GS_OK 0
#define GS_ERR_INVALID 1
#define GS_ERR_WORKSPACE 3

#define GS_EXPORT extern "C" __attribute__((visibility("default")))

static inline int gs_launch_status() {
  hipError_t e = hipGetLastError();
  return e == hipSuccess ? GS_OK : 1000 + (int)e;
}

constexpr int GS_VARIANT_ROUND1_PLAIN = 1;
constexpr int GS_VARIANT_ROUND1 = 2;
constexpr int GS_VARIANT_CLAMP_GRAD = 256;
constexpr int GS_VARIANT_SPLAT = 1024;

extern "C" int gs_rasterize_bwd_slice_depth(const float* records, const int* sorted_vals, const int* tile_bins,
                                            const int* band_edges, const float* background, int S, int R, int H, int W,
                                            const float* out_T, const int* final_idx, const float* v_img,
                                            const float* v_alpha, float* bwd_T, float* bwd_B, float* v_records,
                                            const int* gi_of_e, float* tuples, unsigned char* flags,
                                            const int* sorted_ids, int n_records, const unsigned char* tile_hot,
                                            int variant, const float* cmb_scale, float cmb_gamma, float cmb_min_level,
                                            const float* v_depth, int cameras, void* stream);
extern "C" int gs_rasterize_bwd_rs_slice_depth(const float* records, const int* sorted_vals, const int* tile_bins,
                                               const int* band_edges, const float* background, int S, int H, int W,
                                               const float* out_T, const int* final_idx, const float* v_img,
                                               const float* v_alpha, float* bwd_T, float* bwd_B, float* tuples,
                                               unsigned char* flags, const int* sorted_ids, int n_records, int variant,
                                               const float* cmb_scale, float cmb_gamma, float cmb_min_level,
                                               const float* pix_vel, int N, float rolling_shutter_time,
                                               const float* shared_list_times, const float* v_depth, void* stream);
extern "C" int gs_reduce_grad_tuples_depth(int n_slice, const unsigned* slice_gi, const unsigned* counts,
                                           const unsigned* cum_excl, const float* tuples, const unsigned char* flags,
                                           float* v_records, unsigned char* touched, long long n_isect,
                                           const float* records, int tuples_per_entry, int depth, void* stream);
```

### 3dgs-deblur_amd/csrc/project.hip

```cpp
#include "gs_common.h"

namespace gs {

__global__ void subpose_fwd_kernel(int P, const float* __restrict__ V0, const float* __restrict__ lin,
                                   const float* __restrict__ ang, const float* __restrict__ times,
                                   float* __restrict__ out) {
  int p = blockIdx.x * blockDim.x + threadIdx.x;
  if (p >= P) return;
  float v0[12], l[3], a[3], o[12];
  for (int j = 0; j < 12; ++j) v0[j] = V0[j];
  for (int j = 0; j < 3; ++j) { l[j] = lin[j]; a[j] = ang[j]; }
  subpose_viewmat<float>(v0, l, a, times[p], o);
  for (int j = 0; j < 12; ++j) out[16 * p + j] = o[j];
  out[16 * p + 12] = 0.f; out[16 * p + 13] = 0.f; out[16 * p + 14] = 0.f; out[16 * p + 15] = 1.f;
}

template <bool TIMES>
__global__ __launch_bounds__(256) void subpose_bwd_kernel(int P, const float* __restrict__ V0, const float* __restrict__ lin,
                                   const float* __restrict__ ang, const float* __restrict__ times,
                                   const float* __restrict__ v_out, float* __restrict__ v_V0,
                                   float* __restrict__ v_lin, float* __restrict__ v_ang, float* __restrict__ v_times,
                                   int store) {
  constexpr int NT = TIMES ? 19 : 18;
  extern __shared__ float sp_part[];
// ... 778 lines not shown
  const int base = blockIdx.x * kFusedChunk;
  const int g_first = base + (int)threadIdx.x;
  unsigned any_m = 0u;
  for (int p = 0; p < fp.P; ++p) {
    const unsigned char* t = touched + (size_t)p * fp.N;
    unsigned char v[kFusedChunk / 256];
#pragma unroll
    for (int r = 0; r < kFusedChunk / 256; ++r) v[r] = t[min(g_first + r * 256, fp.N - 1)];
#pragma unroll
    for (int r = 0; r < kFusedChunk / 256; ++r) any_m |= (v[r] != 0 && g_first + r * 256 < fp.N) ? (1u << r) : 0u;
  }
  if (ZERO_FILL) {
    const size_t g0 = (size_t)base, cnt = (size_t)min(kFusedChunk, fp.N - base);
    const size_t sh_row = out.v_sh_rest ? 3 : (size_t)fp.K_stride * 3, rest_row = (size_t)(fp.K_stride - 1) * 3;
    bool stream = true;
    if (out.dirty) {
      if (threadIdx.x == 0) n_dirty = 0;
      __syncthreads();
      unsigned char d[kFusedChunk / 256];
#pragma unroll
      for (int r = 0; r < kFusedChunk / 256; ++r) d[r] = out.dirty[min(g_first + r * 256, fp.N - 1)];
      unsigned dirty_m = 0u;
#pragma unroll
      for (int r = 0; r < kFusedChunk / 256; ++r) dirty_m |= (d[r] != 0 && g_first + r * 256 < fp.N) ? (1u << r) : 0u;
      if (dirty_m) atomicAdd(&n_dirty, __popc(dirty_m));
      __syncthreads();
      stream = (size_t)n_dirty * 4 > cnt;
      if (!stream) {
        for (int r = 0; r < kFusedChunk / 256; ++r) {
          if (!((dirty_m >> r) & 1u)) continue;
          const size_t g = (size_t)(g_first + r * 256);
          zero_span(out.v_means, 3 * g, 3);
          zero_span(out.v_scales, 3 * g, 3);
          zero_span(out.v_quats, 4 * g, 4);
          out.v_opac[g] = 0.f;
          zero_span(out.v_sh, sh_row * g, sh_row);
          if (out.v_sh_rest) zero_span(out.v_sh_rest, rest_row * g, rest_row);
        }
      }
      for (int r = 0; r < kFusedChunk / 256; ++r)
        if (((dirty_m ^ any_m) >> r) & 1u) out.dirty[g_first + r * 256] = (unsigned char)((any_m >> r) & 1u);
    }
    if (stream) {
      zero_rows(out.v_means, 3 * g0, 3 * cnt);
      zero_rows(out.v_scales, 3 * g0, 3 * cnt);
      zero_rows(out.v_quats, 4 * g0, 4 * cnt);
      zero_rows(out.v_opac, g0, cnt);
      zero_rows(out.v_sh, sh_row * g0, sh_row * cnt);
      if (out.v_sh_rest) zero_rows(out.v_sh_rest, rest_row * g0, rest_row * cnt);
    }
    zero_rows(out.v_xy_sum, 2 * g0, 2 * cnt);
    __threadfence_block();
  }
#pragma unroll
  for (int r = 0; r < kFusedChunk / 256; ++r) {
    const unsigned long long bal = __ballot((any_m >> r) & 1u);
    if (lane == 0) wave_cnt[r][wave] = __popcll(bal);
  }
  __syncthreads();
  int n_list = 0;
#pragma unroll
  for (int r = 0; r < kFusedChunk / 256; ++r) {
    const bool any = (any_m >> r) & 1u;
    const unsigned long long bal = __ballot(any);
    int off = n_list, total = 0;
#pragma unroll
    for (int w = 0; w < 4; ++w) { const int c = wave_cnt[r][w]; if (w < wave) off += c; total += c; }
    if (any) list[off + __popcll(bal & ((1ull << lane) - 1ull))] = g_first + r * 256;
    n_list += total;
  }
  __syncthreads();
  for (int k0 = 0; k0 < n_list; k0 += 256) {
    const int k = k0 + (int)threadIdx.x;
    const bool live = k < n_list;
    fused_bwd_body<MAXB, DEPTH>(fp, records, v_records, out, touched, live ? list[k] : 0, live, lds, blk_acc);
    if (out.clear_touched && live)
      for (int p = 0; p < fp.P; ++p) touched[(size_t)p * fp.N + list[k]] = 0;
  }
  __syncthreads();
  for (int k = threadIdx.x; k < slots * 12; k += 256) out.pose_partial[(size_t)blockIdx.x * slots * 12 + k] = blk_acc[k];
}

__global__ __launch_bounds__(256) void slice_records_kernel(int n_slice, SliceDesc sd, const unsigned* __restrict__ sorted_gi,
                                                            FusedParams fp, float* __restrict__ records) {
  const int j = blockIdx.x * 256 + threadIdx.x;
  if (j >= n_slice) return;
  const unsigned gi = sorted_gi[slice_rank(sd, j)];
  const int p = (int)(gi / (unsigned)fp.N), i = (int)(gi - (unsigned)p * (unsigned)fp.N);
  float m[3] = {fp.means[3 * i], fp.means[3 * i + 1], fp.means[3 * i + 2]};
  float sc[3];
  load_scales(fp, i, sc);
  float q[4] = {fp.quats[4 * i], fp.quats[4 * i + 1], fp.quats[4 * i + 2], fp.quats[4 * i + 3]};
  const float opac = load_opacity(fp, i);
  float R[9], qn[4], inv, M[9], c3[6];
  quat_to_rotmat(q, R, qn, &inv);
  scale_rot_to_cov3d(sc, fp.glob, R, M, c3);
  const float* V = fp.viewmats + 16 * p;
  float Vm[12];
#pragma unroll
  for (int k = 0; k < 12; ++k) Vm[k] = V[k];
  Proj o; ProjCtx k;
  bool ok = project_one(m, c3, Vm, fp.in.fx, fp.in.fy, fp.in.cx, fp.in.cy, fp.in.W, fp.in.H, fp.in.tiles_x,
                        fp.in.tiles_y, fp.in.clip, o, k);
  if (ok && fp.rs_bands > 1) {
    const int rb = p % fp.rs_bands;
    const int by0 = (rb * fp.in.tiles_y) / fp.rs_bands, by1 = ((rb + 1) * fp.in.tiles_y) / fp.rs_bands;
    o.tmin_y = max(o.tmin_y, by0);
    o.tmax_y = min(o.tmax_y, by1);
    ok = o.tmax_y > o.tmin_y;
  }
  float4* r = reinterpret_cast<float4*>(records + (size_t)gi * kRecFloats);
  if (ok) {
    const float op = fp.antialiased ? opac * o.comp : opac;
    float aux[4];
    rec_aux(op, o.conic_x, o.conic_z, aux);
    r[0] = make_float4(o.x, o.y, o.conic_x, o.conic_y);
    r[1] = make_float4(o.conic_z, op, 0.f, 0.f);
    r[2] = make_float4(0.f, o.depth, __int_as_float(o.tmin_x | (o.tmin_y << 16)),
                       __int_as_float(o.tmax_x | (o.tmax_y << 16)));
    r[3] = make_float4(aux[0], aux[1], aux[2], aux[3]);
  } else {
    const float4 z = make_float4(0.f, 0.f, 0.f, 0.f);
    r[0] = z; r[1] = z; r[2] = z; r[3] = z;
  }
}

template <int MAXB> constexpr int slice_colors_waves() { return MAXB <= 16 ? 4 : 2; }

template <int MAXB>
__global__ __launch_bounds__(256) void slice_colors_kernel(int n_slice, const unsigned* __restrict__ slice_gi,
                                                           const unsigned* __restrict__ counts, int N,
                                                           const float* __restrict__ means,
                                                           const float* __restrict__ sh,
                                                           const float* __restrict__ sh_rest, int K_stride, int deg,
                                                           const float* __restrict__ viewmats,
                                                           float* __restrict__ records) {
  constexpr int kRow = MAXB * 3 + 1;
  constexpr int kRowPad = (kRow & 1) ? kRow : kRow + 1;
  __shared__ float s_coef[slice_colors_waves<MAXB>()][64 * kRowPad];
  const int lane = threadIdx.x & 63;
  float* rows = s_coef[threadIdx.x >> 6];
  const int j = blockIdx.x * blockDim.x + threadIdx.x;
  const bool active = j < n_slice && counts[j] != 0;
  const unsigned gi = active ? slice_gi[j] : 0u;
  const unsigned p = gi / (unsigned)N, g = gi - p * (unsigned)N;
  const int nb = (deg + 1) * (deg + 1);
  const int grp = lane >> 4, q = lane & 15;
#pragma unroll 4
  for (int it = 0; it < 16; ++it) {
    const int r = it * 4 + grp;
    const unsigned g_r = (unsigned)__shfl((int)g, r);
    const int act_r = __shfl((int)active, r);
    if (act_r) {
      const float *r0, *r1;
      sh_rows(sh, sh_rest, K_stride, (size_t)g_r, r0, r1);
      for (int b = q; b < nb; b += 16) {
        const float* c = b == 0 ? r0 : r1 + 3 * (b - 1);
        const float c0 = c[0], c1 = c[1], c2 = c[2];
        float* d = rows + r * kRowPad + 3 * b;
        d[0] = c0; d[1] = c1; d[2] = c2;
      }
    }
  }
  __builtin_amdgcn_wave_barrier();
  if (!active) return;
  const float* V = viewmats + 16 * p;
  const float m0 = means[3 * g], m1 = means[3 * g + 1], m2 = means[3 * g + 2];
  float cxw = -(V[0] * V[3] + V[4] * V[7] + V[8] * V[11]);
  float cyw = -(V[1] * V[3] + V[5] * V[7] + V[9] * V[11]);
  float czw = -(V[2] * V[3] + V[6] * V[7] + V[10] * V[11]);
  float dx = m0 - cxw, dy = m1 - cyw, dz = m2 - czw;
  float dinv = 1.0f / sqrtf(dx * dx + dy * dy + dz * dz);
  float B[MAXB];
  sh_basis(deg, dx * dinv, dy * dinv, dz * dinv, B);
  const float* coef = rows + lane * kRowPad;
  float cr = 0.5f, cg = 0.5f, cb = 0.5f;
#pragma unroll
  for (int b = 0; b < MAXB; ++b) {
    if (b < nb) { cr += B[b] * coef[3 * b]; cg += B[b] * coef[3 * b + 1]; cb += B[b] * coef[3 * b + 2]; }
  }
  float* r = records + (size_t)gi * kRecFloats;
  r[6] = fmaxf(cr, 0.f); r[7] = fmaxf(cg, 0.f); r[8] = fmaxf(cb, 0.f);
}

}

using namespace gs;

static inline Intrin make_intrin(float fx, float fy, float cx, float cy, int H, int W, float clip) {
  Intrin in;
  in.fx = fx; in.fy = fy; in.cx = cx; in.cy = cy; in.W = W; in.H = H;
  in.tiles_x = (W + K::kTile - 1) / K::kTile; in.tiles_y = (H + K::kTile - 1) / K::kTile; in.clip = clip;
  return in;
}

GS_EXPORT int gs_subpose_viewmats_fwd(int P, const float* viewmat, const float* lin_vel, const float* ang_vel,
                                      const float* times, float* out_viewmats, void* stream) {
  if (P <= 0) return GS_ERR_INVALID;
  hipLaunchKernelGGL(subpose_fwd_kernel, dim3((P + 63) / 64), dim3(64), 0, (hipStream_t)stream, P, viewmat, lin_vel,
                     ang_vel, times, out_viewmats);
  return gs_launch_status();
}

GS_EXPORT int gs_subpose_viewmats_bwd(int P, const float* viewmat, const float* lin_vel, const float* ang_vel,
                                      const float* times, const float* v_out, float* v_viewmat, float* v_lin,
                                      float* v_ang, void* stream) {
  if (P <= 0) return GS_ERR_INVALID;
  hipLaunchKernelGGL(subpose_bwd_kernel<false>, dim3(1), dim3(256), (size_t)P * 18 * sizeof(float), (hipStream_t)stream, P, viewmat, lin_vel,
                     ang_vel, times, v_out, v_viewmat, v_lin, v_ang, (float*)nullptr, 0);
  return gs_launch_status();
}

GS_EXPORT int gs_subpose_viewmats_bwd_store(int P, const float* viewmat, const float* lin_vel, const float* ang_vel,
                                            const float* times, const float* v_out, float* v_viewmat, float* v_lin,
                                            float* v_ang, void* stream) {
  if (P <= 0 || !v_viewmat || !v_lin || !v_ang) return GS_ERR_INVALID;
  hipLaunchKernelGGL(subpose_bwd_kernel<false>, dim3(1), dim3(256), (size_t)P * 18 * sizeof(float), (hipStream_t)stream, P, viewmat, lin_vel,
                     ang_vel, times, v_out, v_viewmat, v_lin, v_ang, (float*)nullptr, 1);
  return gs_launch_status();
// ... 40 lines not shown
  return gs_launch_status();
}

GS_EXPORT int gs_sh_fwd(int N, int K_stride, int degrees_to_use, const float* dirs, const float* coeffs,
                        float* colors, void* stream) {
  if (N <= 0 || degrees_to_use < 0 || degrees_to_use > 4 || (degrees_to_use + 1) * (degrees_to_use + 1) > K_stride)
    return GS_ERR_INVALID;
  hipLaunchKernelGGL(sh_fwd_kernel, dim3((N + 255) / 256), dim3(256), 0, (hipStream_t)stream, N, K_stride,
                     degrees_to_use, dirs, coeffs, colors);
  return gs_launch_status();
}

GS_EXPORT int gs_sh_bwd(int N, int K_stride, int degrees_to_use, const float* dirs, const float* v_colors,
                        float* v_coeffs, void* stream) {
  if (N <= 0 || degrees_to_use < 0 || degrees_to_use > 4 || (degrees_to_use + 1) * (degrees_to_use + 1) > K_stride)
    return GS_ERR_INVALID;
  hipLaunchKernelGGL(sh_bwd_kernel, dim3((N + 255) / 256), dim3(256), 0, (hipStream_t)stream, N, K_stride,
                     degrees_to_use, dirs, v_colors, v_coeffs);
  return gs_launch_status();
}

GS_EXPORT int gs_pack_records(int N, const float* xys, const float* depths, const int* radii, const float* conics,
                              const float* colors, const float* opacity, int H, int W, float* records,
                              unsigned* depth_keys, int* ntiles, void* stream) {
  if (N <= 0) return GS_ERR_INVALID;
  int tiles_x = (W + K::kTile - 1) / K::kTile, tiles_y = (H + K::kTile - 1) / K::kTile;
  hipLaunchKernelGGL(pack_records_kernel, dim3((N + 255) / 256), dim3(256), 0, (hipStream_t)stream, N, xys, depths,
                     radii, conics, colors, opacity, tiles_x, tiles_y, records, depth_keys, ntiles);
  return gs_launch_status();
}

GS_EXPORT int gs_unpack_record_grads(int N, const float* v_records, float* v_xys, float* v_conics, float* v_colors,
                                     float* v_opacity, void* stream) {
  if (N <= 0) return GS_ERR_INVALID;
  hipLaunchKernelGGL(unpack_grads_kernel, dim3((N + 255) / 256), dim3(256), 0, (hipStream_t)stream, N, v_records,
                     v_xys, v_conics, v_colors, v_opacity);
  return gs_launch_status();
}

static inline FusedParams make_fused(int N, int P, const float* means, const float* scales, float glob,
                                     const float* quats, const float* opac, const float* sh, int K_stride, int deg,
                                     const float* viewmats, float fx, float fy, float cx, float cy, int H, int W,
                                     float clip, int antialiased, int defer_color = 0) {
  FusedParams fp;
  fp.N = N; fp.P = P; fp.means = means; fp.scales = scales; fp.quats = quats; fp.opacities = opac; fp.sh = sh;
  fp.viewmats = viewmats; fp.glob = glob; fp.K_stride = K_stride; fp.deg = deg; fp.antialiased = antialiased;
  fp.defer_color = defer_color & 1;
  fp.skip_culled = (defer_color >> 1) & 1;
  fp.no_records = (defer_color >> 4) & 1;
  fp.records_only = 0;
  fp.rs_bands = (defer_color & 4) ? ((defer_color >> 8) & 0xFFFF) : 0;
  fp.in = make_intrin(fx, fy, cx, cy, H, W, clip);
  fp.pixvel = 0; fp.twist = nullptr; fp.times = nullptr; fp.flags = 0; fp.rs_half = 0.f; fp.pix_vel_out = nullptr;
  fp.act = 0; fp.sh_rest = nullptr;
  return fp;
}

static int launch_fused_fwd(const FusedParams& fp, float* records, unsigned* depth_keys, int* num_tiles_hit, int* radii,
                            void* stream) {
  hipLaunchKernelGGL((fp.defer_color ? project_fused_fwd_kernel<16, true>
                      : fp.deg <= 3  ? project_fused_fwd_kernel<16, false> : project_fused_fwd_kernel<25, false>),
                     dim3((fp.N + 255) / 256), dim3(256), 0, (hipStream_t)stream, fp, records, depth_keys, num_tiles_hit,
                     radii);
  return gs_launch_status();
}

GS_EXPORT int gs_project_fused_fwd(int N, int P, const float* means, const float* scales, float glob_scale,
                                   const float* quats, const float* opacities, const float* sh, int K_stride,
                                   int sh_degree, const float* viewmats, float fx, float fy, float cx, float cy,
                                   int H, int W, float clip, int antialiased, int defer_color, float* records,
                                   unsigned* depth_keys, int* num_tiles_hit, int* radii, const float* sh_rest,
                                   int param_flags, void* stream) {
  if (N <= 0 || P <= 0 || sh_degree < 0 || sh_degree > 4 || (sh_degree + 1) * (sh_degree + 1) > K_stride)
    return GS_ERR_INVALID;
  FusedParams fp = make_fused(N, P, means, scales, glob_scale, quats, opacities, sh, K_stride, sh_degree, viewmats,
                              fx, fy, cx, cy, H, W, clip, antialiased, defer_color);
  fp.act = param_flags; fp.sh_rest = sh_rest;
  return launch_fused_fwd(fp, records, depth_keys, num_tiles_hit, radii, stream);
}

GS_EXPORT int gs_slice_project_records(int n_slice, int P, int N, const int* slice_begin, const int* slice_prefix,
                                       const unsigned* sorted_gi, const gs_project_inputs* in, int H, int W,
                                       float* records, void* stream) {
  SliceDesc sd;
  if (n_slice <= 0 || N <= 0 || !in || !sorted_gi || !records || !make_slice_desc(P, slice_begin, slice_prefix, sd))
    return GS_ERR_INVALID;
  if (!in->means || !in->scales || !in->quats || !in->opacities || !in->viewmats) return GS_ERR_INVALID;
  FusedParams fp = make_fused(N, P, in->means, in->scales, in->glob_scale, in->quats, in->opacities, nullptr, 1, 0,
                              in->viewmats, in->fx, in->fy, in->cx, in->cy, H, W, in->clip_thresh, in->antialiased,
                              in->defer_color | 1);
  fp.act = in->param_flags;
  hipLaunchKernelGGL(slice_records_kernel, dim3((n_slice + 255) / 256), dim3(256), 0, (hipStream_t)stream, n_slice, sd,
                     sorted_gi, fp, records);
  return gs_launch_status();
}

GS_EXPORT int gs_project_records(int P, int N, const gs_project_inputs* in, int H, int W, float* records, void* stream) {
  if (P <= 0 || N <= 0 || !in || !records) return GS_ERR_INVALID;
  if (!in->means || !in->scales || !in->quats || !in->opacities || !in->viewmats) return GS_ERR_INVALID;
  FusedParams fp = make_fused(N, P, in->means, in->scales, in->glob_scale, in->quats, in->opacities, nullptr, 1, 0,
                              in->viewmats, in->fx, in->fy, in->cx, in->cy, H, W, in->clip_thresh, in->antialiased,
                              (in->defer_color | 1 | 2) & ~16);
  fp.act = in->param_flags;
  fp.records_only = 1;
  return launch_fused_fwd(fp, records, nullptr, nullptr, nullptr, stream);
}

GS_EXPORT int gs_slice_colors(int n_slice, const unsigned* slice_gi, const unsigned* counts, int N,
                              const float* means, const float* sh, const float* sh_rest, int K_stride, int sh_degree,
                              const float* viewmats, float* records, void* stream) {
  if (n_slice <= 0 || N <= 0 || sh_degree < 0 || sh_degree > 4 || (sh_degree + 1) * (sh_degree + 1) > K_stride)
    return GS_ERR_INVALID;
  const bool low = sh_degree <= 3;
  const int th = 64 * (low ? slice_colors_waves<16>() : slice_colors_waves<25>());
  hipLaunchKernelGGL(low ? slice_colors_kernel<16> : slice_colors_kernel<25>, dim3((n_slice + th - 1) / th), dim3(th), 0,
                     (hipStream_t)stream, n_slice, slice_gi, counts, N, means, sh, sh_rest, K_stride, sh_degree, viewmats,
                     records);
  return gs_launch_status();
}

constexpr int GS_FLAG_XY_PER_CAMERA = 128;
constexpr int GS_FLAG_ZERO_FILL = 32;

static long long pose_scratch_bytes(int N, int P, bool pixvel, bool with_touched) {
  const long long blocks = with_touched ? (N + kFusedChunk - 1) / kFusedChunk : (N + 255) / 256;
  return blocks * (long long)(pixvel ? 2 : P) * 12 * (long long)sizeof(float);
}

static int launch_fused_bwd(const FusedParams& fp, int sh_degree, const float* records, const float* v_records,
                            FusedOut out, const unsigned char* touched_in, void* scratch, long long scratch_bytes,
                            hipStream_t st, int clear_touched = 0) {
  unsigned char* touched = const_cast<unsigned char*>(touched_in);
  const bool needles = !(fp.flags & GS_FLAG_NO_NEEDLE_HP);
  out.clear_touched = (clear_touched == 1 && !needles) ? 1 : 0;
  const int needle_clears = (clear_touched == 1 && needles) ? 1 : 0;
  dim3 block(256);
  const int N = fp.N;
  const bool pose = out.v_viewmats || out.v_twist;
  const int slots = pose ? (fp.pixvel ? 2 : fp.P) : 0;
  const size_t lds = (size_t)slots * 12 * sizeof(float);
  if (pose) {
    if (!scratch || scratch_bytes < pose_scratch_bytes(N, fp.P, fp.pixvel != 0, touched != nullptr)) return GS_ERR_WORKSPACE;
    out.pose_partial = reinterpret_cast<float*>(scratch);
  }
  dim3 grid(touched ? (N + kFusedChunk - 1) / kFusedChunk : (N + 255) / 256);
  const bool depth = (fp.flags & GS_FLAG_DEPTH_GRAD) != 0;
  const bool low = sh_degree <= 3;
  if (touched) {
    const bool zf = (fp.flags & GS_FLAG_ZERO_FILL) != 0;
    const auto kernel =
        depth ? (low ? (zf ? project_fused_bwd_sparse_kernel<16, true, true> : project_fused_bwd_sparse_kernel<16, false, true>)
                     : (zf ? project_fused_bwd_sparse_kernel<25, true, true> : project_fused_bwd_sparse_kernel<25, false, true>))
              : (low ? (zf ? project_fused_bwd_sparse_kernel<16, true, false> : project_fused_bwd_sparse_kernel<16, false, false>)
                     : (zf ? project_fused_bwd_sparse_kernel<25, true, false> : project_fused_bwd_sparse_kernel<25, false, false>));
    hipLaunchKernelGGL(kernel, grid, block, lds, st, fp, records, v_records, out, touched);
  } else {
    const auto kernel = depth ? (low ? project_fused_bwd_kernel<16, true> : project_fused_bwd_kernel<25, true>)
                              : (low ? project_fused_bwd_kernel<16, false> : project_fused_bwd_kernel<25, false>);
    hipLaunchKernelGGL(kernel, grid, block, lds, st, fp, records, v_records, out);
  }
  if (pose) {
    PoseDst dst{out.v_viewmats, fp.pixvel ? out.v_twist : nullptr, fp.pixvel ? 0 : 16, (!fp.pixvel && out.dirty) ? 1 : 0};
    hipLaunchKernelGGL(pose_reduce_kernel, dim3(slots), dim3(256), 0, st, out.pose_partial, (int)grid.x, slots, dst);
  }
  if (needles)
    hipLaunchKernelGGL(depth ? project_needle_hp_kernel<true> : project_needle_hp_kernel<false>,
                       dim3((N + kNeedleChunk - 1) / kNeedleChunk), dim3(256), 0, st, fp, records, v_records, out.v_means,
                       out.v_scales, out.v_quats, touched, kNeedleRatio, needle_clears);
  return gs_launch_status();
}

__global__ __launch_bounds__(256) void xy_grad_cams_kernel(int N, int P, int B, const float* __restrict__ v_records,
                                                           unsigned char* __restrict__ touched,
                                                           float* __restrict__ v_xy, int clear_touched) {
  const int i = blockIdx.x * blockDim.x + threadIdx.x;
  if (i >= N) return;
  const int Pc = P / B;
  for (int b = 0; b < B; ++b) {
    float vxs = 0.f, vys = 0.f;
    for (int p = b * Pc; p < (b + 1) * Pc; ++p) {
      const size_t idx = (size_t)p * N + i;
      if (!touched[idx]) continue;
      if (clear_touched) touched[idx] = 0;
      const float2 g = *reinterpret_cast<const float2*>(v_records + idx * kGradFloats);
      vxs += g.x; vys += g.y;
    }
    *reinterpret_cast<float2*>(v_xy + ((size_t)b * N + i) * 2) = make_float2(vxs, vys);
  }
}

__global__ __launch_bounds__(256) void xy_absgrad_cams_kernel(int N, int P, int B, const float* __restrict__ v_records,
                                                              const unsigned char* __restrict__ touched,
                                                              float* __restrict__ out) {
  const int i = blockIdx.x * blockDim.x + threadIdx.x;
  if (i >= N) return;
  const int Pc = P / B;
  for (int b = 0; b < B; ++b) {
    float ax = 0.f, ay = 0.f;
    for (int p = b * Pc; p < (b + 1) * Pc; ++p) {
      const size_t idx = (size_t)p * N + i;
// ... 121 lines not shown
```

### 3dgs-deblur_amd/ops.py

```python
from __future__ import annotations

import ctypes
import math
from collections import namedtuple
from dataclasses import dataclass
from typing import NamedTuple, Optional, Tuple

import torch
from torch import Tensor
from torch.autograd import Function

from . import _lib

import os
import threading

TILE = 16
REC = 16
GRAD = 12
MAX_SUBPOSES = 256
SLICE_BASE = int(os.environ.get("GSD_SLICE_BASE", "512"))
SLICE_ADAPT = int(os.environ.get("GSD_SLICE_ADAPT", "1"))
SLICE_GROW_OPEN = float(os.environ.get("GSD_SLICE_GROW_OPEN", "0.5"))
_state_lock = threading.RLock()


class FrameHints:

    __slots__ = ("mult", "age", "arena_bytes", "arena_retries", "frames", "box_share", "last_slices", "select_misses",
                 "select_cap", "select_overflows", "_recent", "_lock", "_views")

    def __init__(self):
        self.mult, self.age, self.arena_bytes, self.arena_retries, self.frames = 1, 0, 0, 0, 0
        self.box_share = None
        self.last_slices = None
        self.select_misses = 0
        self.select_cap = 0
        self.select_overflows = 0
        self._recent = []
        self._lock = threading.Lock()
        self._views = {}

    def slice_base(self) -> int:
        return SLICE_BASE * (self.mult if SLICE_ADAPT and SLICE_BASE > 0 else 1)

    def feedback(self, n_issued: int, retries: int = 0, box_share: Optional[float] = None, select_state: int = 0,
                 open_after_first: Optional[float] = None, max_selected: int = 0, select_overflow: int = 0) -> None:
        with self._lock:
            self.frames += 1
            self.last_slices = int(n_issued)
            if select_state == 2:
                self.select_misses += 1
            if max_selected > 0:
                want = int(1.5 * max_selected) + 4096
                self.select_cap = want if (select_overflow or want > self.select_cap) else max(want, int(0.9 * self.select_cap))
            self.select_overflows += int(bool(select_overflow))
            if box_share is not None:
                self.box_share = float(box_share)
            self.arena_retries += retries
            self._recent = (self._recent + [(int(n_issued), self.mult, int(retries))])[-4:]
            if SLICE_ADAPT and SLICE_BASE > 0:
                grow = n_issued >= 2 and self.mult < 8 and (open_after_first is None or open_after_first < 0
                                                            or open_after_first >= SLICE_GROW_OPEN)
                if self.age >= 255:
                    self.mult, self.age = 1, 0
                else:
                    self.mult, self.age = (self.mult * 2 if grow else self.mult), self.age + 1

    @property
    def settled(self) -> bool:
        with self._lock:
            r = self._recent
            return (len(r) >= 2 and r[-1][0] == r[-2][0] and r[-1][1] == r[-2][1] == self.mult
                    and r[-1][2] == 0 and r[-2][2] == 0)

    def lazy_records(self) -> bool:
        return self.mult == 1 and (self.box_share is None or self.box_share < 0.25)

    def depth_select(self) -> bool:
        return self.last_slices == 1 and self.box_share is not None and self.box_share < 0.5

    def view(self, key) -> "ViewHints":
        with self._lock:
            v = self._views.get(key)
            if v is None:
                if len(self._views) >= 16384:
                    self._views.clear()
                v = self._views[key] = ViewHints(self)
                v.box_share, v.last_slices, v.select_cap = self.box_share, self.last_slices, self.select_cap
            return v

    def reset(self) -> None:
        with self._lock:
            self.mult, self.age, self.arena_bytes, self._recent, self.box_share = 1, 0, 0, [], None
            self.last_slices, self.select_cap = None, 0
            self._views.clear()


class ViewHints:

    __slots__ = ("scene", "box_share", "last_slices", "select_cap")

    def __init__(self, scene: "FrameHints"):
        self.scene = scene
        self.box_share, self.last_slices, self.select_cap = None, None, 0

    arena_bytes = property(lambda self: self.scene.arena_bytes,
                           lambda self, v: setattr(self.scene, "arena_bytes", v))
    mult = property(lambda self: self.scene.mult)
    frames = property(lambda self: self.scene.frames)
    arena_retries = property(lambda self: self.scene.arena_retries)
    select_misses = property(lambda self: self.scene.select_misses)
    select_overflows = property(lambda self: self.scene.select_overflows)
    settled = property(lambda self: self.scene.settled)

    def slice_base(self) -> int:
        return self.scene.slice_base()

    def lazy_records(self) -> bool:
        return self.scene.mult == 1 and (self.box_share is None or self.box_share < 0.25)

    def depth_select(self) -> bool:
        return self.last_slices == 1 and self.box_share is not None and self.box_share < 0.5

    def view(self, key) -> "ViewHints":
        return self.scene.view(key)

    def feedback(self, n_issued: int, retries: int = 0, box_share: Optional[float] = None, select_state: int = 0,
                 open_after_first: Optional[float] = None, max_selected: int = 0, select_overflow: int = 0) -> None:
        sc = self.scene
        with sc._lock:
            self.last_slices = int(n_issued)
            if box_share is not None:
                self.box_share = float(box_share)
            if max_selected > 0:
                want = int(1.5 * max_selected) + 4096
                self.select_cap = want if (select_overflow or want > self.select_cap) else max(want, int(0.9 * self.select_cap))
        sc.feedback(n_issued, retries, box_share, select_state, open_after_first, max_selected, select_overflow)


_hints = {}


def hints_for(key) -> FrameHints:
    with _state_lock:
        h = _hints.get(key)
        if h is None:
            if len(_hints) >= 64:
                _hints.clear()
            h = _hints[key] = FrameHints()
        return h


SLICE_MERGE = float(os.environ.get("GSD_SLICE_MERGE", "0.75"))
FRAME_POLL = int(os.environ.get("GSD_FRAME_POLL", "1"))


def _host_cores() -> int:
    try:
        return len(os.sched_getaffinity(0))
    except (AttributeError, OSError):
        return os.cpu_count() or 1


def frame_poll() -> int:
    if "GSD_FRAME_POLL" in os.environ or not FRAME_POLL:
        return int(FRAME_POLL)
    local_world = max(1, int(os.environ.get("LOCAL_WORLD_SIZE", "1") or 1))
    return 1 if _host_cores() >= 2 * local_world else 0


def readback_mode() -> dict:
    return {"poll": bool(frame_poll()), "host_cores": _host_cores(),
            "local_rank": int(os.environ.get("LOCAL_RANK", "0") or 0),
            "local_world": int(os.environ.get("LOCAL_WORLD_SIZE", "1") or 1),
            "forced": "GSD_FRAME_POLL" in os.environ}
DEPTH_SORT_DIGIT = 8
UPSTREAM_GRADS = int(os.environ.get("GSD_UPSTREAM_GRADS", "6"))


BAND_AWARE = int(os.environ.get("GSD_BAND_AWARE", "1"))
LAZY_RECORDS = int(os.environ.get("GSD_LAZY_RECORDS", "1"))
DEPTH_SELECT = int(os.environ.get("GSD_DEPTH_SELECT", "1"))
NEEDLE_HP = int(os.environ.get("GSD_NEEDLE_HP", "1"))


def _proj_grad_flags() -> int:
    return (UPSTREAM_GRADS & 1) | (0 if NEEDLE_HP else 8)


BWD_SPLAT = int(os.environ.get("GSD_BWD_SPLAT", "0"))


BWD_ABSGRAD = 2048


def _bwd_variant(absgrad: bool = False) -> int:
    if absgrad:
        return (256 if (UPSTREAM_GRADS & 4) else 0) | BWD_ABSGRAD
    return (256 if (UPSTREAM_GRADS & 4) else 0) | (1024 if BWD_SPLAT else 0)
_slice_totals = []


def __getattr__(name):
    if name == "last_slice_intersects":
        for i, v in enumerate(_slice_totals):
            if isinstance(v, torch.Tensor):
                _slice_totals[i] = int(v.item()) & 0xFFFFFFFF
        return list(_slice_totals)
    raise AttributeError(name)


from ._profile import FRAME_STAGES, StageProfiler, _NULL

profiler: Optional[StageProfiler] = None
last_num_intersects: int = 0
last_depth_select: int = 0


def _stage(name: str):
    return _NULL if profiler is None else profiler.stage(name)


def _L():
    return _lib.load()


def _ptr(t: Optional[Tensor]):
    return None if t is None else ctypes.c_void_p(t.data_ptr())


def _stream():
    return ctypes.c_void_p(torch.cuda.current_stream().cuda_stream)


def _f32(t: Tensor, name: str) -> Tensor:
    if not t.is_cuda:
        raise ValueError(f"{name} must be a CUDA(HIP) tensor: the HIP path has no CPU fallback")
    if t.dtype != torch.float32:
        raise ValueError(f"{name} must be float32, got {t.dtype}")
    return t.contiguous()


def _tiles(h: int, w: int) -> Tuple[int, int]:
    return (w + TILE - 1) // TILE, (h + TILE - 1) // TILE


IDS_PAD = 8


def _padded_i32(n: int, dev) -> Tensor:
    return torch.empty(n + IDS_PAD, dtype=torch.int32, device=dev)[:n]


def _bits(n: int) -> int:
    return max(1, int(math.ceil(math.log2(max(2, n)))))


SYNC_CHECK = int(os.environ.get("GSD_SYNC_CHECK", "0"))


def _check(st: int, what: str):
    _lib.check(st, what)
    if SYNC_CHECK:
        try:
            torch.cuda.synchronize()
        except RuntimeError as e:
            raise _lib.HipLibraryError(f"asynchronous HIP fault surfaced right after stage '{what}': {e}") from e


def _pose_scratch(N: int, P: int, with_touched: bool, dev) -> Tensor:
    return torch.empty(int(_L().gs_project_pose_scratch_bytes(int(N), int(P), int(bool(with_touched)))), dtype=torch.uint8,
                       device=dev)


def _viewmat16(viewmat: Tensor) -> Tensor:
    v = _f32(viewmat, "viewmat")
    if v.shape[-2:] == (3, 4):
        pad = torch.tensor([[0.0, 0.0, 0.0, 1.0]], device=v.device, dtype=v.dtype)
        v = torch.cat([v, pad.expand(v.shape[:-2] + (1, 4))], dim=-2).contiguous()
    if v.shape[-2:] != (4, 4):
        raise ValueError("viewmat must be [4,4] (or [3,4])")
    return v


def exclusive_scan_u32(x: Tensor) -> Tuple[Tensor, Tensor]:
    assert x.dtype == torch.int32 and x.is_cuda and x.is_contiguous()
    n = x.numel()
    out = torch.empty_like(x)
    if n == 0:
        return out, torch.zeros(1, dtype=torch.int32, device=x.device)
    total = torch.empty(1, dtype=torch.int32, device=x.device)
    ws_bytes = _L().gs_scan_workspace_bytes(n)
    ws = torch.empty(ws_bytes, dtype=torch.uint8, device=x.device)
    _check(_L().gs_exclusive_scan_u32(n, _ptr(x), _ptr(out), _ptr(total), _ptr(ws), ws_bytes, _stream()), "scan")
    return out, total


def radix_sort_pairs(keys: Tensor, vals: Optional[Tensor], begin_bit: int, end_bit: int,
                     gather_src: Optional[Tensor] = None, n_dev: Optional[Tensor] = None,
# ... 59 lines not shown
    bins = torch.empty(P * T, 2, dtype=torch.int32, device=dev)
    if n_isect == 0:
        bins.zero_()
        z = torch.zeros(1, dtype=torch.int32, device=dev)
        return (z, bins, 0, z.clone()) + ((None,) if with_emission else ())
    if n_isect < 0:
        raise OverflowError("more than 2^31-1 tile intersections; chunk the sub-poses")
    with _stage("emit"):
        keys = torch.empty(n_isect, dtype=torch.int32, device=dev)
        vals = _padded_i32(n_isect, dev)
        _check(L.gs_emit_intersects(n, N, img_height, img_width, _ptr(sorted_gi), _ptr(cum), _ptr(records), n_isect,
                                    _ptr(keys), _ptr(vals), 0, _stream()), "emit intersects")
    extra = None
    with _stage("tile_sort"):
        if with_emission:
            skeys, eids, svals = radix_sort_pairs(keys, None, 0, _bits(P * T), carry=vals)
            extra = dict(eids=eids, sorted_gi=sorted_gi, counts=counts, cum=cum)
        else:
            skeys, svals = radix_sort_pairs(keys, vals, 0, _bits(P * T))
    with _stage("bin_edges"):
        _check(L.gs_tile_bin_edges_u32(n_isect, _ptr(skeys), P * T, _ptr(bins), None, _stream()), "bin edges")
    return (svals, bins, n_isect, skeys) + ((extra,) if with_emission else ())


_band_edge_cache = {}


def _band_edges(img_height: int, rs_bands: int, device) -> Tensor:
    key = (int(img_height), max(1, int(rs_bands)), str(device))
    t = _band_edge_cache.get(key)
    if t is None:
        _, ty = _tiles(img_height, 1)
        R = key[1]
        t = torch.tensor([(r * ty) // R for r in range(R + 1)], dtype=torch.int32, device=device)
        if len(_band_edge_cache) > 64:
            _band_edge_cache.clear()
        _band_edge_cache[key] = t
    return t


_band_done_cache = {}


def _band_tile_done(S: int, R: int, ty: int, tx: int, dev) -> Tensor:
    key = (S, R, ty, tx, str(dev))
    t = _band_done_cache.get(key)
    if t is None:
        e = [(r * ty) // R for r in range(R + 1)]
        rows = torch.arange(ty, device=dev)
        band_open = torch.stack([(rows >= e[r]) & (rows < e[r + 1]) for r in range(R)])
        t = (~band_open).to(torch.uint8)[None, :, :, None].expand(S, R, ty, tx).reshape(-1).contiguous()
        if len(_band_done_cache) > 16:
            _band_done_cache.clear()
        _band_done_cache[key] = t
    return t


def _background(background: Optional[Tensor], device) -> Tensor:
    if background is None:
        return torch.zeros(3, dtype=torch.float32, device=device)
    bg = background.detach().to(device=device, dtype=torch.float32).contiguous()
    if bg.numel() != 3:
        raise ValueError("background must have 3 channels")
    return bg


frame_backend = None


class _FrameDesc(ctypes.Structure):
    _fields_ = [(k, ctypes.c_int) for k in ("N", "P", "S", "R", "H", "W", "slice_base", "depth_sort_digit",
                                             "fwd_variant", "reserve_backward")] + [("merge_open_fraction", ctypes.c_float),
                                                                                     ("rolling_shutter_time", ctypes.c_float),
                                                                                     ("poll_readback", ctypes.c_int),
                                                                                     ("shared_list", ctypes.c_int),
                                                                                     ("combine_gamma", ctypes.c_float),
                                                                                     ("combine_min_level", ctypes.c_float),
                                                                                     ("band_clipped", ctypes.c_int),
                                                                                     ("depth_select", ctypes.c_int),
                                                                                     ("select_cap", ctypes.c_int),
                                                                                     ("sweep_t_min", ctypes.c_float),
                                                                                     ("sweep_t_max", ctypes.c_float),
                                                                                     ("lazy_records", ctypes.c_void_p),
                                                                                     ("cameras", ctypes.c_int)]


class _ProjectInputs(ctypes.Structure):
    _fields_ = ([(k, ctypes.c_void_p) for k in ("means", "scales", "quats", "opacities", "viewmats")] +
                [(k, ctypes.c_float) for k in ("glob_scale", "fx", "fy", "cx", "cy", "clip_thresh")] +
                [(k, ctypes.c_int) for k in ("antialiased", "defer_color", "param_flags")])


class _FrameSlice(ctypes.Structure):
    _fields_ = ([("I", ctypes.c_longlong)] + [(k, ctypes.c_int) for k in ("n", "wave_per_gaussian", "first", "last")] +
                [(k, ctypes.c_longlong) for k in ("svals", "bins", "fidx", "gi_of_e", "sorted_ids", "slice_gi", "counts",
                                                  "cum", "tile_hot", "n_emitted_dev")])


class _FrameState(ctypes.Structure):
    _fields_ = ([(k, ctypes.c_int) for k in ("n_slices", "P", "N", "S", "R", "H", "W")] +
                [("rolling_shutter_time", ctypes.c_float), ("shared_list", ctypes.c_int), ("depth_select", ctypes.c_int),
                 ("select_overflow", ctypes.c_int), ("open_after_first", ctypes.c_float)] +
                [(k, ctypes.c_longlong) for k in ("n_total", "max_selected", "arena_used", "arena_required")] +
                [("slice", _FrameSlice * 16), ("cameras", ctypes.c_int)])


def _box_share(state) -> Optional[float]:
    n_total = int(state.n_total)
    if n_total <= 0:
        return None
    held = sum(int(state.slice[i].I) for i in range(int(state.n_slices)))
    return min(1.0, held / n_total)


class _ArenaTooSmall(Exception):
    pass


_ARENA_ATTEMPTS = 16
_arena_pool = {}


class _Arena:
    __slots__ = ("tensor", "gen")

    def __init__(self, tensor):
        self.tensor, self.gen = tensor, 0

    def numel(self):
        return self.tensor.numel()

    def data_ptr(self):
        return self.tensor.data_ptr()


_lease_counter = 0


class _ArenaLease:
    __slots__ = ("arena", "key", "gen")

    def __init__(self, arena: _Arena, key):
        global _lease_counter
        self.arena, self.key = arena, key
        with _state_lock:
            _lease_counter += 1
            self.gen = arena.gen = _lease_counter

    @property
    def tensor(self):
        a = self.arena
        return None if a is None else a.tensor

    def release(self):
        try:
            with _state_lock:
                a, self.arena = self.arena, None
                if a is None:
                    return
                free = _arena_pool.setdefault(self.key, [])
                free.append(a)
                if len(free) > 2:
                    free.remove(min(free, key=lambda x: x.numel()))
        except Exception:
            pass

    __del__ = release


def _arena_acquire(dev, want_bytes: int) -> _ArenaLease:
    key = (str(dev), torch.cuda.current_stream(dev).cuda_stream)
    with _state_lock:
        free = _arena_pool.setdefault(key, [])
        free[:] = [x if isinstance(x, _Arena) else _Arena(x) for x in free]
        a = max(free, key=lambda x: x.numel()) if free else None
        if a is not None:
            free.remove(a)
    if a is None or a.numel() < want_bytes:
        a = None
        a = _Arena(torch.empty(int(want_bytes), dtype=torch.uint8, device=dev))
    return _ArenaLease(a, key)


def _arena_relend(frame) -> bool:
    a = frame["arena_obj"]
    with _state_lock:
        free = _arena_pool.get(frame["lease"].key, [])
# ... 27 lines not shown
def _storage_use_count(t: Tensor) -> int:
    fn = getattr(torch._C, "_storage_Use_Count", None)
    if fn is None:
        return 1 << 30
    return int(fn(t.untyped_storage()._cdata))


_STORAGE_FREE = _storage_use_count(torch.empty(1))


class _GradEntry:
    __slots__ = ("pool_key", "shape_key", "flat", "dirty", "touched", "version", "valid")

    def __init__(self, pool_key, shape_key, flat, dirty, touched):
        self.pool_key, self.shape_key = pool_key, shape_key
        self.flat, self.dirty, self.touched = flat, dirty, touched
        self.version, self.valid = flat._version, False

    def recyclable(self) -> bool:
        return (self.valid and self.flat._version == self.version
                and _storage_use_count(self.flat) <= _STORAGE_FREE)


def _grad_pool_acquire(dev, N: int, P: int, K: int, split: bool, alloc=None) -> _GradEntry:
    stream = torch.cuda.current_stream(dev).cuda_stream if torch.device(dev).type == "cuda" else 0
    pool_key, shape_key = (str(dev), stream), (int(N), int(P), int(K), bool(split))
    with _state_lock:
        entries = _grad_pool.setdefault(pool_key, [])
        hit = None
        for e in list(entries):
            if e.shape_key == shape_key and e.recyclable():
                hit = hit or e
            elif not e.valid or e.flat._version != e.version or e.shape_key != shape_key:
                entries.remove(e)
        if hit is not None:
            entries.remove(hit)
            hit.valid = False
            return hit
    n_flat = (3 + 3 + 4 + 1 + 3 * K) * N
    if alloc is not None:
        flat, dirty, touched = alloc(n_flat, N, P)
    else:
        flat = torch.empty(n_flat, device=dev)
        dirty = torch.ones(N, dtype=torch.uint8, device=dev)
        touched = torch.zeros(P * N, dtype=torch.uint8, device=dev)
    return _GradEntry(pool_key, shape_key, flat, dirty, touched)


def _grad_pool_commit(entry: _GradEntry) -> None:
    with _state_lock:
        entry.version, entry.valid = entry.flat._version, True
        entries = _grad_pool.setdefault(entry.pool_key, [])
        if entry not in entries:
            entries.append(entry)
        while len(entries) > _GRAD_POOL_KEEP:
            entries.pop(0)


def grad_pool_invalidate(t: Tensor) -> None:
    ptr = t.untyped_storage().data_ptr()
    with _state_lock:
        for entries in _grad_pool.values():
            for e in list(entries):
                if e.flat.untyped_storage().data_ptr() == ptr:
                    e.valid = False
                    entries.remove(e)


_pinned_cache = {}


def _profile_mask() -> int:
    if profiler is None:
        return 0
    names = FRAME_STAGES if profiler.only is None else [n for n in FRAME_STAGES if n in profiler.only]
    return sum(1 << FRAME_STAGES.index(n) for n in names)


def native_frame_forward(records: Tensor, depth_keys: Tensor, num_tiles_hit: Tensor, P: int, N: int, S: int, R: int,
                         H: int, W: int, bg: Tensor, edges: Tensor, slice_base: int, color=None,
                         out_depth: Optional[Tensor] = None, reserve_backward: bool = True, rs=None, combine=None,
                         hints: Optional[FrameHints] = None, band_clipped: bool = False, lazy=None,
                         depth_select: Optional[bool] = None, cameras: int = 1):
    global last_num_intersects, _slice_totals, last_depth_select
    L = _L()
    dev = records.device
    tx, ty = _tiles(H, W)
    shared = rs is not None and len(rs) > 2 and rs[2] is not None
    if hints is None:
        hints = hints_for((str(dev), N, P, S, H, W, shared))
    if depth_select is None:
        depth_select = bool(DEPTH_SELECT == 2 or (DEPTH_SELECT and hints.depth_select()))
    n = P * N
    nbytes = hints.arena_bytes
    if not nbytes:
        I0 = max(1, slice_base) * tx * ty * P
        nbytes = 44 * n + 16 * S * H * W + (80 + (56 * S if shared else 0)) * I0 + (64 << 20)
    lease = _arena_acquire(dev, nbytes)
    arena = lease.tensor
    nbytes = arena.numel()
    pin_key = (str(dev), threading.get_ident(), torch.cuda.current_stream().cuda_stream)
    pin = _pinned_cache.get(pin_key)
    need_pin = 4 * (2 * P * 16 + 2 * P + 2) + 64
    if pin is None or pin.numel() < need_pin:
        pin = _pinned_cache[pin_key] = torch.empty(max(8192, need_pin), dtype=torch.uint8, pin_memory=True)
    desc = _FrameDesc(N, P, S, R, H, W, int(slice_base), DEPTH_SORT_DIGIT, 0, int(reserve_backward),
                      float(SLICE_MERGE), float(rs[1]) if rs is not None else 0.0, frame_poll(), int(shared),
                      float(combine[0]) if combine is not None else 1.0, float(combine[1]) if combine is not None else 0.0,
                      int(bool(band_clipped)), int(bool(depth_select and slice_base > 0)),
                      int(min(hints.select_cap, 2 ** 31 - 1)) if depth_select else 0,
                      float(rs[3][0]) if shared and len(rs) > 3 else 0.0, float(rs[3][1]) if shared and len(rs) > 3 else 0.0,
                      ctypes.addressof(lazy) if lazy is not None else None, int(cameras))
    state = _FrameState()
    out_img = torch.empty(S, H, W, 3, device=dev)
    out_T = torch.empty(S, H, W, device=dev)
    band_done = _band_tile_done(S, R, ty, tx, dev) if R > 1 else None
    c_means = c_sh = c_rest = c_V = None
    c_K = c_deg = 0
    if color is not None:
        c_means, c_sh, c_rest, c_K, c_deg, c_V = color
    L.gs_frame_profile_enable(_profile_mask())
    st = L.gs_frame_forward(ctypes.byref(desc), _ptr(records), _ptr(depth_keys), _ptr(num_tiles_hit), _ptr(bg), _ptr(edges),
                            _ptr(band_done), _ptr(c_means), _ptr(c_sh), _ptr(c_rest), int(c_K), int(c_deg), _ptr(c_V),
                            _ptr(rs[0]) if rs is not None else None, _ptr(rs[2]) if shared else None, _ptr(out_img),
                            _ptr(out_T), _ptr(out_depth), _ptr(combine[2]) if combine is not None else None,
                            _ptr(arena), arena.numel(), ctypes.c_void_p(pin.data_ptr()), pin.numel(), ctypes.byref(state),
                            _stream())
    if st == 3:
        hints.arena_bytes = max(int(state.arena_required * 1.15) + (32 << 20), int(nbytes * 1.5))
        raise _ArenaTooSmall()
    _check(st, "frame_forward")
    hints.arena_bytes = max(int(hints.arena_bytes),
                            int((state.arena_used + L.gs_frame_backward_bytes(ctypes.byref(state))) * 1.15))
    last_num_intersects = int(state.n_total)
    last_depth_select = int(state.depth_select)
    _slice_totals = [arena[sl.n_emitted_dev:sl.n_emitted_dev + 4].view(torch.int32)
                     for sl in (state.slice[i] for i in range(state.n_slices))]
    return out_img, out_T, dict(arena=arena, arena_obj=lease.arena, lease=lease, gen=lease.gen, state=state,
                                pix_vel=rs[0] if rs is not None else None,
                                sample_times=rs[2] if shared else None)


def native_frame_backward(frame, records: Tensor, bg: Tensor, edges: Tensor, out_T: Tensor, v_img: Tensor,
                          v_alpha: Optional[Tensor], v_records: Tensor, touched: Tensor, combine=None,
                          v_depth: Optional[Tensor] = None, absgrad: bool = False):
    L = _L()
    cmb = combine if combine is not None else (None, 1.0, 0.0)
    arena, state = frame["arena"], frame["state"]
    lease = frame["lease"]
    relent = lease.arena is None and _arena_relend(frame)
    try:
        _native_frame_backward(L, frame, arena, state, records, bg, edges, out_T, v_img, v_alpha, v_records, touched, cmb,
                               v_depth, absgrad)
    finally:
        if relent:
            _arena_return(frame)
        else:
            lease.release()


def _native_frame_backward(L, frame, arena, state, records, bg, edges, out_T, v_img, v_alpha, v_records, touched, cmb,
                           v_depth=None, absgrad=False):
    L.gs_frame_profile_enable(_profile_mask())
    if v_depth is None:
        st = L.gs_frame_backward(ctypes.byref(state), _ptr(records), _ptr(bg), _ptr(edges), _ptr(out_T), _ptr(v_img),
                                 _ptr(v_alpha), _ptr(cmb[0]), float(cmb[1]), float(cmb[2]), _bwd_variant(absgrad),
                                 _ptr(v_records), _ptr(touched), _ptr(frame.get("pix_vel")), _ptr(frame.get("sample_times")), _ptr(arena),
                                 arena.numel(), _stream())
    else:
        st = L.gs_frame_backward_depth(ctypes.byref(state), _ptr(records), _ptr(bg), _ptr(edges), _ptr(out_T),
                                       _ptr(v_img), _ptr(v_alpha), _ptr(cmb[0]), float(cmb[1]), float(cmb[2]),
                                       _bwd_variant(absgrad), _ptr(v_records), _ptr(touched),
                                       _ptr(frame.get("pix_vel")),
                                       _ptr(frame.get("sample_times")), _ptr(arena), arena.numel(), _ptr(v_depth),
                                       _stream())
    if st == 3:
        raise _lib.HipLibraryError("frame_backward: the forward's arena cannot hold the backward's buffers "
                                   "(call native_frame_forward with reserve_backward=True)")
    _check(st, "frame_backward")


class _ProjectGaussians(Function):
    @staticmethod
    def forward(ctx, means3d, scales, glob_scale, quats, viewmat, fx, fy, cx, cy, img_height, img_width,
                block_width, clip_thresh):
        if block_width != TILE:
            raise ValueError("only block_width=16 is supported")
        means3d, scales, quats = _f32(means3d, "means3d"), _f32(scales, "scales"), _f32(quats, "quats")
        V = _viewmat16(viewmat)
        N = means3d.shape[0]
        dev = means3d.device
        xys = torch.empty(N, 2, device=dev)
        depths = torch.empty(N, device=dev)
        radii = torch.empty(N, dtype=torch.int32, device=dev)
        conics = torch.empty(N, 3, device=dev)
        comp = torch.empty(N, device=dev)
        ntiles = torch.empty(N, dtype=torch.int32, device=dev)
        cov3d = torch.empty(N, 6, device=dev)
        _check(_L().gs_project_fwd(N, _ptr(means3d), _ptr(scales), float(glob_scale), _ptr(quats), _ptr(V),
                                   float(fx), float(fy), float(cx), float(cy), int(img_height), int(img_width),
                                   float(clip_thresh), _ptr(xys), _ptr(depths), _ptr(radii), _ptr(conics),
                                   _ptr(comp), _ptr(ntiles), _ptr(cov3d), None, _stream()), "project_fwd")
        ctx.save_for_backward(means3d, scales, quats, V)
        ctx.args = (float(glob_scale), float(fx), float(fy), float(cx), float(cy), int(img_height),
                    int(img_width), float(clip_thresh))
        ctx.mark_non_differentiable(radii, ntiles)
        return xys, depths, radii, conics, comp, ntiles, cov3d

    @staticmethod
    def backward(ctx, v_xys, v_depths, v_radii, v_conics, v_comp, v_ntiles, v_cov3d):
        means3d, scales, quats, V = ctx.saved_tensors
        glob, fx, fy, cx, cy, H, W, clip = ctx.args
        N = means3d.shape[0]
        dev = means3d.device

        def z(g, shape):
            return torch.zeros(shape, device=dev) if g is None else g.contiguous().float()
        v_xys, v_depths, v_conics, v_comp = z(v_xys, (N, 2)), z(v_depths, (N,)), z(v_conics, (N, 3)), z(v_comp, (N,))
# ... 413 lines not shown
        P = 1
    if pixvel:
        V = _viewmat16(viewmats).reshape(4, 4)
        twist = torch.cat([_f32(lin_vel, "lin_vel").reshape(3), _f32(ang_vel, "ang_vel").reshape(3)]).contiguous()
        times = _f32(times, "times").reshape(-1)
        if times.numel() != P:
            raise ValueError(f"times must hold {P} sub-pose times")
    else:
        V = _f32(viewmats, "viewmats")
        twist = None
        if V.shape != (P, 4, 4):
            raise ValueError(f"viewmats must be [{P},4,4]")
    dev = means.device
    L = _L()
    records = torch.empty(P * N, REC, device=dev)
    dkeys = torch.empty(P * N, dtype=torch.int32, device=dev)
    ntiles = torch.empty(P * N, dtype=torch.int32, device=dev)
    radii = torch.empty(P, N, dtype=torch.int32, device=dev)
    backend = frame_backend if (frame_backend is not None and not frame_backend.native_ok()) else None
    defer_flags = 3 if backend is None else backend.defer_flags()
    if backend is None and R > 1 and BAND_AWARE:
        defer_flags |= 4 | (R << 8)
    if backend is None and hints is None:
        key = (str(dev), N, P, S, H, W, shared is not None, means.untyped_storage().data_ptr())
        hints = hints_for(key if B == 1 else key + (B,))
    lazy = None
    if (backend is None and not pixvel and LAZY_RECORDS and hints.slice_base() > 0
            and (LAZY_RECORDS == 2 or hints.lazy_records())):
        defer_flags |= 16
    pix_vel = torch.empty(N, 2, device=dev) if (rs_time != 0.0 or shared is not None) else None
    rs = None if pix_vel is None else (pix_vel, rs_time) + ((shared[0], shared[2]) if shared is not None else ())
    box_sweep = shared[1] if shared is not None else rs_time

    def _project():
        if pixvel:
            _check(L.gs_project_pixvel_fwd(N, P, _ptr(means), _ptr(scales), spec.glob_scale, _ptr(quats),
                                           _ptr(opacities), _ptr(sh), K, spec.sh_degree, _ptr(V), _ptr(twist),
                                           _ptr(times), spec.fx, spec.fy, spec.cx, spec.cy, H, W, spec.clip_thresh,
                                           spec.antialiased, defer_flags, _ptr(records), _ptr(dkeys), _ptr(ntiles),
                                           _ptr(radii), box_sweep, _ptr(pix_vel), _ptr(sh_rest), param_flags, _stream()),
                   "project_pixvel_fwd")
        else:
            _check(L.gs_project_fused_fwd(N, P, _ptr(means), _ptr(scales), spec.glob_scale, _ptr(quats), _ptr(opacities),
                                          _ptr(sh), K, spec.sh_degree, _ptr(V), spec.fx, spec.fy, spec.cx, spec.cy, H, W,
                                          spec.clip_thresh, spec.antialiased, defer_flags, _ptr(records), _ptr(dkeys),
                                          _ptr(ntiles), _ptr(radii), _ptr(sh_rest), param_flags, _stream()),
                   "project_fused_fwd")

    with _stage("project_fwd"):
        _project()
    if defer_flags & 16:
        lazy = _ProjectInputs(means.data_ptr(), scales.data_ptr(), quats.data_ptr(), opacities.data_ptr(),
                              V.data_ptr(), spec.glob_scale, spec.fx, spec.fy, spec.cx, spec.cy, spec.clip_thresh,
                              spec.antialiased, defer_flags & ~16, param_flags)
    bg = _background(background, dev)
    edges = _band_edges(H, R, dev)
    V_col = V.reshape(1, 16).expand(P, 16).contiguous() if pixvel else V
    color = (means, sh, sh_rest, K, spec.sh_degree, V_col) if (defer_flags & 1) else None
    depth_acc = torch.zeros(S, H, W, device=dev) if spec.return_depth else None
    m = spec.min_rgb_level / 255.0
    prealloc = frame = None
    if backend is None:
        if want and GRAD_POOL and not pixvel:
            entry = _grad_pool_acquire(dev, N, P, K, sh_rest is not None)
            prealloc = {"entry": entry, "touched": entry.touched, "v_records": torch.empty(P * N, GRAD, device=dev),
                        "pose_scratch": _pose_scratch(N, P, True, dev)}
        elif want:
            t_len = (P * N + 15) // 16 * 16
            zbuf = torch.zeros(t_len + 4 * (16 * P + 12), dtype=torch.uint8, device=dev)
            zf = zbuf[t_len:].view(torch.float32)
            prealloc = {"touched": zbuf[:P * N], "v_records": torch.empty(P * N, GRAD, device=dev), "v_V": zf[:16 * P],
                        "v_tw": zf[16 * P:16 * P + 12], "pose_scratch": _pose_scratch(N, P, True, dev)}
        averaged = None
        if spec.gamma is not None:
            averaged = (spec.gamma, m, torch.empty((H, W, 3) if B == 1 else (B, H, W, 3), device=dev))
        retries = 0
        for attempt in range(_ARENA_ATTEMPTS):
            try:
                out_img, out_T, frame = native_frame_forward(records, dkeys, ntiles, P, N, S, R, H, W, bg, edges,
                                                             hints.slice_base(), color, depth_acc, bool(want), rs,
                                                             averaged, hints, bool(defer_flags & 4), lazy, cameras=B)
                st = frame["state"]
                hints.feedback(int(st.n_slices), retries, _box_share(st), int(st.depth_select),
                               float(st.open_after_first), int(st.max_selected), int(st.select_overflow))
                break
            except _ArenaTooSmall:
                retries += 1
                if attempt == _ARENA_ATTEMPTS - 1:
                    raise _lib.HipLibraryError("frame_forward: the arena estimate did not converge")
                if depth_acc is not None:
                    depth_acc.zero_()
                with _stage("project_fwd"):
                    _project()
        slices = []
    else:
        prealloc = {} if want else None
        out_img, out_T, slices = backend.sliced_forward(records, dkeys, ntiles, P, N, S, R, H, W, bg, edges, SLICE_BASE,
                                                        color, depth_acc, prealloc, rs)
    first, samples, rgb = out_img, None, None
    if spec.gamma is not None:
        samples = out_img
        if backend is None:
            first = rgb = averaged[2]
        else:
            first = rgb = torch.empty(H, W, 3, device=dev)
            with _stage("combine"):
                _check(L.gs_combine_fwd(S, H * W * 3, _ptr(out_img), spec.gamma, m, _ptr(first), _stream()),
                       "combine_fwd")
    state = FrameSaved(spec, N, P, K, want, background is not None and "background" in want, frame, backend, slices,
                       prealloc, rs, xy_grad_out, xy_absgrad_out)
    tensors = FrameTensors(means, scales, quats, opacities, sh, sh_rest, V, twist, times, records, edges, bg, out_T,
                           samples, rgb)
    return (first, (1.0 - out_T) if spec.return_alpha else None, radii, depth_acc), state, tensors


def frame_backward(state: FrameSaved, tensors: FrameTensors, v_img, v_alpha, v_depth=None) -> FrameGrads:
    if v_img is None and v_alpha is None and v_depth is None:
        return FrameGrads()
    spec, N, P, K = state.spec, state.N, state.P, state.K
    S, R, H, W, B = spec.S, spec.R, spec.H, spec.W, spec.cameras
    (means, scales, quats, opacities, sh, sh_rest, V, twist, times, records, edges, bg, out_T, samples,
     rgb) = tensors
    dev = means.device
    L = _L()
    if v_depth is not None:
        if state.frame is None:
            raise NotImplementedError("a depth gradient needs the native frame backward (gs_frame_backward_depth); "
                                      "the frame backend in use has no depth channel")
        v_depth = v_depth.contiguous().float()
    if v_img is None:
        v_img = torch.zeros((S, H, W, 3) if spec.gamma is None else ((H, W, 3) if B == 1 else (B, H, W, 3)), device=dev)
    else:
        v_img = v_img.contiguous().float()
    v_al = None if v_alpha is None else v_alpha.contiguous().float()
    combine = None
    if spec.gamma is not None:
        gamma, m = spec.gamma, spec.min_rgb_level / 255.0
        bwd, bwd_scale, dims, tag = ((L.gs_combine_bwd_batched, L.gs_combine_bwd_scale_batched,
                                      (B, S // B, rgb.numel() // B), "_batched") if B > 1 else
                                     (L.gs_combine_bwd, L.gs_combine_bwd_scale, (S, rgb.numel()), ""))
        if state.bg_grad:
            v_samples = torch.empty_like(samples)
            _check(bwd(*dims, _ptr(samples), gamma, m, _ptr(rgb), _ptr(v_img), _ptr(v_samples), _stream()),
                   "combine_bwd" + tag)
            v_img = v_samples
        else:
            scale = torch.empty_like(rgb)
            with _stage("combine"):
                _check(bwd_scale(*dims, gamma, _ptr(rgb), _ptr(v_img), _ptr(scale), _stream()),
                       "combine_bwd_scale" + tag)
            combine = (scale, gamma, m)
            v_img = samples
    all_tuples = state.frame is not None or all(sl["gi_of_e"] is not None for sl in state.slices)
    pre = state.prealloc if state.prealloc else {}
    state.prealloc = None
    entry = None
    if all_tuples and pre.get("entry") is not None and state.frame is not None:
        entry = pre["entry"]
        v_records, touched = pre["v_records"], entry.touched
    elif all_tuples and "touched" in pre:
        v_records, touched = pre["v_records"], pre["touched"]
    elif all_tuples:
        v_records = torch.empty(P * N, GRAD, device=dev)
        touched = torch.zeros(P * N, dtype=torch.uint8, device=dev)
    else:
        v_records = torch.zeros(P * N, GRAD, device=dev)
        touched = None
# ... 199 lines not shown
```

### include/gsdeblur.h

```cpp
#ifndef GSDEBLUR_H
#define GSDEBLUR_H

#ifdef __cplusplus
extern "C" {
#endif

#define GS_BWD_ABSGRAD 2048

const char* gs_version(void);

int gs_subpose_viewmats_fwd(int P, const float* viewmat , const float* lin_vel ,
                            const float* ang_vel , const float* times ,
                            float* out_viewmats , void* stream);
int gs_subpose_viewmats_bwd(int P, const float* viewmat, const float* lin_vel, const float* ang_vel,
                            const float* times, const float* v_out , float* v_viewmat,
                            float* v_lin, float* v_ang, void* stream);
int gs_subpose_viewmats_bwd_store(int P, const float* viewmat, const float* lin_vel, const float* ang_vel,
                                  const float* times, const float* v_out , float* v_viewmat,
                                  float* v_lin, float* v_ang, void* stream);
int gs_subpose_viewmats_bwd_times(int P, const float* viewmat, const float* lin_vel, const float* ang_vel,
                                  const float* times, const float* v_out , float* v_viewmat ,
                                  float* v_lin , float* v_ang , float* v_times , void* stream);

int gs_project_fwd(int N, const float* means3d , const float* scales , float glob_scale,
// ... 233 lines not shown
                              void* stream);
int gs_rasterize_bwd_rs_slice(const float* records, const int* sorted_vals, const int* tile_bins, const int* band_edges,
                              const float* background, int S, int img_height, int img_width, const float* out_T,
                              const int* final_idx, const float* v_img, const float* v_alpha, float* bwd_T, float* bwd_B,
                              float* tuples, unsigned char* flags, const int* sorted_ids, int n_records, int variant,
                              const float* cmb_scale, float cmb_gamma, float cmb_min_level, const float* pix_vel, int N,
                              float rolling_shutter_time,
                              const float* shared_list_times ,
                              void* stream);
int gs_rasterize_bwd_slice(const float* records, const int* sorted_vals, const int* tile_bins,
                           const int* band_edges, const float* background, int S, int R, int img_height,
                           int img_width, const float* out_T, const int* final_idx, const float* v_img,
                           const float* v_alpha, float* bwd_T, float* bwd_B, float* v_records,
                           const int* gi_of_e ,
                           float* tuples , unsigned char* flags ,
                           const int* sorted_ids , int n_records,
                           const unsigned char* tile_hot ,
                           int variant ,
                           const float* cmb_scale ,
                           float cmb_gamma, float cmb_min_level, void* stream);

int gs_reduce_grad_tuples(int n_slice, const unsigned* slice_gi, const unsigned* counts,
                          const unsigned* cum_excl, const float* tuples, const unsigned char* flags,
                          float* v_records, unsigned char* touched ,
                          long long n_isect ,
                          const float* records ,
                          int tuples_per_entry ,
                          void* stream);

int gs_combine_fwd(int S, long long n, const float* samples , float gamma, float min_level,
                   float* out , void* stream);
int gs_combine_bwd(int S, long long n, const float* samples, float gamma, float min_level,
                   const float* out, const float* v_out, float* v_samples , void* stream);
int gs_combine_bwd_scale(int S, long long n, float gamma, const float* out, const float* v_out,
                         float* scale , void* stream);
int gs_combine_fwd_batched(int B, int S, long long n, const float* samples, float gamma, float min_level,
                           float* out, void* stream);
int gs_combine_bwd_batched(int B, int S, long long n, const float* samples, float gamma, float min_level,
                           const float* out, const float* v_out, float* v_samples, void* stream);
int gs_combine_bwd_scale_batched(int B, int S, long long n, float gamma, const float* out, const float* v_out,
                                 float* scale, void* stream);

int gs_dp_row_mask(int N, int n_tensors, float* const* grads, const int* widths,
                   unsigned char* mask , void* stream);
int gs_dp_pack_rows(long long M, const long long* row_idx , int n_tensors,
                    float* const* grads, const int* widths, float* payload , void* stream);
int gs_dp_scatter_add_rows(long long M, const float* payload, int n_tensors, float* const* grads,
                           const int* widths, float scale, void* stream);
int gs_dp_pack_masked_rows(int N, const unsigned char* mask, const int* pos, int cap, int* idx_ws, int n_tensors,
                           float* const* grads, const int* widths, float* payload, void* stream);
int gs_dp_scatter_add_payload(int cap, const float* payload, int n_tensors, float* const* grads, const int* widths,
                              float scale, void* stream);

typedef struct gs_project_inputs {
  const float *means, *scales, *quats, *opacities, *viewmats;
  float glob_scale, fx, fy, cx, cy, clip_thresh;
  int antialiased, defer_color, param_flags;
} gs_project_inputs;
int gs_slice_project_records(int n_slice, int P, int N, const int* slice_begin, const int* slice_prefix,
                             const unsigned* sorted_gi, const gs_project_inputs* in, int img_height, int img_width,
                             float* records, void* stream);
int gs_project_records(int P, int N, const struct gs_project_inputs* in, int img_height, int img_width, float* records,
                       void* stream);

#define GS_FRAME_MAX_SLICES 16
typedef struct gs_frame_desc {
  int N, P, S, R, H, W;
  int slice_base;
  int depth_sort_digit;
  int fwd_variant;
  int reserve_backward;
  float merge_open_fraction;
  float rolling_shutter_time;
  int poll_readback;
  int shared_list;
  float combine_gamma;
  float combine_min_level;
  int band_clipped;
  int depth_select;
  int select_cap;
  float sweep_t_min, sweep_t_max;
  const struct gs_project_inputs* lazy_records;
  int cameras;
} gs_frame_desc;
typedef struct gs_frame_slice {
  long long I;
  int n, wave_per_gaussian, first, last;
  long long svals, bins, fidx, gi_of_e, sorted_ids, slice_gi, counts, cum, tile_hot, n_emitted_dev;
} gs_frame_slice;
typedef struct gs_frame_state {
  int n_slices, P, N, S, R, H, W;
  float rolling_shutter_time;
  int shared_list;
  int depth_select;
  int select_overflow;
  float open_after_first;
  long long n_total;
  long long max_selected;
  long long arena_used;
  long long arena_required;
  gs_frame_slice slice[GS_FRAME_MAX_SLICES];
  int cameras;
} gs_frame_state;
int gs_frame_forward(const gs_frame_desc* desc, float* records, unsigned* depth_keys, const int* num_tiles_hit,
                     const float* background , const int* band_edges , const unsigned char* band_tile_done,
                     const float* color_means, const float* color_sh, const float* color_sh_rest , int color_K_stride, int color_sh_degree,
                     const float* color_viewmats ,
                     const float* pix_vel ,
                     const float* sample_times ,
                     float* out_img , float* out_T , float* out_depth,
                     float* out_combined ,
                     void* arena, long long arena_bytes, void* host_pinned,
                     long long host_pinned_bytes, gs_frame_state* state, void* stream);
long long gs_frame_backward_bytes(const gs_frame_state* state);
int gs_frame_backward(const gs_frame_state* state, const float* records, const float* background, const int* band_edges,
                      const float* out_T, const float* v_img, const float* v_alpha, const float* cmb_scale,
                      float cmb_gamma, float cmb_min_level, int bwd_variant, float* v_records, unsigned char* touched,
                      const float* pix_vel , const float* sample_times ,
                      void* arena, long long arena_bytes, void* stream);
int gs_frame_backward_depth(const gs_frame_state* state, const float* records, const float* background,
                            const int* band_edges, const float* out_T, const float* v_img, const float* v_alpha,
                            const float* cmb_scale, float cmb_gamma, float cmb_min_level, int bwd_variant,
                            float* v_records, unsigned char* touched, const float* pix_vel, const float* sample_times,
                            void* arena, long long arena_bytes, const float* v_depth , void* stream);
int gs_xy_absgrad_sum(int N, int P, int cameras, const float* v_records ,
                      const unsigned char* touched , float* out , void* stream);
int gs_frame_profile_enable(unsigned stage_mask);
int gs_frame_profile_read(int max_events, int* stage_ids, float* ms);

long long gs_image_loss_workspace_bytes(int img_height, int img_width);
int gs_image_loss_fwd_bwd(int img_height, int img_width, const float* pred, const float* gt, float ssim_lambda,
                          float* v_pred, float* loss_out, void* workspace, long long workspace_bytes, void* stream);
int gs_adam_step(int count, float* const* params, const float* const* grads, float* const* exp_avg,
                 float* const* exp_avg_sq, const long long* numel, const float* lr, double beta1, double beta2, double eps,
                 int step, void* stream);
int gs_adam_step_rows(int count, int N, const unsigned char* mask , float* const* params,
                      const float* const* grads, float* const* exp_avg, float* const* exp_avg_sq,
                      const int* widths, const float* lr, double beta1, double beta2, double eps, int step,
                      void* ws, long long ws_bytes, void* stream);
long long gs_adam_step_rows_workspace_bytes(int N);
int gs_visible_rows(int M, int N, const int* radii, unsigned char* mask, void* stream);

int gs_mcmc_inject_noise(int N, float* means, const float* log_scales, const float* quats, const float* opacity_logits,
                         float scaler, long long seed, long long step, const float* noise_in, float* noise_out,
                         void* stream);
int gs_mcmc_relocation(int M, const float* opacities, const float* scales, const int* ratios, float* new_opacities,
                       float* new_scales, void* stream);

int gs_bilagrid_slice_fwd(int B, int H, int W, int G, int GW, int GH, int L, const float* grids, const int* grid_idx,
                          const float* rgb, float* out, void* stream);
long long gs_bilagrid_slice_bwd_workspace_bytes(int B, int H, int W, int G, int GW, int GH, int L);
int gs_bilagrid_slice_bwd(int B, int H, int W, int G, int GW, int GH, int L, const float* grids, const int* grid_idx,
                          const float* rgb, const float* v_out, float* v_rgb, float* v_grids, void* ws,
                          long long ws_bytes, void* stream);
long long gs_bilagrid_tv_workspace_bytes(int G, int GW, int GH, int L);
int gs_bilagrid_tv_fwd_bwd(int G, int GW, int GH, int L, const float* grids, float weight, float* loss_out,
                           float* v_grids, void* ws, long long ws_bytes, void* stream);

#ifdef __cplusplus
}
#endif
#endif
```

Baseline: 1235.

## Speculatively plan depth-select slices on device to skip host readback

Adds a speculative path in which the slice-plan kernel builds the slice descriptor (per-subpose begins, prefix sums, total slice count, capacity-miss flags) on the device. The count and emit kernels then read that descriptor directly instead of waiting for a host readback of the plan. Emit writes are clamped to an entry cap, and host hints use the previous frame's wave mode to decide whether to speculate. This is meant to remove a host-device synchronization round trip in forward binning. In exchange it adds miss detection and fallback logic, and grids sized from capacity bounds launch waves that only exit early.

```diff
diff --git a/3dgs-deblur_amd/csrc/binning.hip b/3dgs-deblur_amd/csrc/binning.hip
--- a/3dgs-deblur_amd/csrc/binning.hip
+++ b/3dgs-deblur_amd/csrc/binning.hip
@@ -1067,7 +1067,46 @@
                                   int* __restrict__ bounds, unsigned* __restrict__ rels,
                                   unsigned* __restrict__ seg_totals, const unsigned* __restrict__ n_live,
                                   unsigned* __restrict__ tail ,
-                                  const unsigned* __restrict__ grand ) {
+                                  const unsigned* __restrict__ grand ,
+                                  SliceDescDev* __restrict__ dd ,
+                                  unsigned pair_cap, unsigned long long box_cap, unsigned entry_cap) {
+  if (dd && blockIdx.x == 0) {
+    const int lane = (int)threadIdx.x;
+    int run = 0, miss = 0;
+    unsigned long long boxes = 0ull;
+    for (int q0 = 0; q0 < P; q0 += 64) {
+      const int q = q0 + lane;
+      unsigned live = 0u, box = 0u;
+      if (q < P) {
+        const unsigned* cq = cum + (size_t)q * N;
+        live = min((unsigned)N, n_live[q]);
+        box = ((q + 1 < P) ? cq[N] : *total) - cq[0];
+      }
+      if (__ballot(live > pair_cap)) miss |= 1;
+      const unsigned take = min(live, pair_cap);
+      unsigned inc = take;
+#pragma unroll
+      for (int o = 1; o < 64; o <<= 1) {
+        const unsigned t = __shfl_up(inc, o);
+        if (lane >= o) inc += t;
+      }
+      if (q < P) { dd->begin[q] = q * N; dd->prefix[q] = run + (int)(inc - take); }
+      run += (int)__shfl(inc, 63);
+      unsigned long long b = box;
+#pragma unroll
+      for (int o = 32; o > 0; o >>= 1) b += __shfl_xor(b, o);
+      boxes += b;
+    }
+    if (boxes > box_cap) miss |= 2;
+    if (lane == 0) {
+      dd->prefix[P] = run;
+      dd->n_slice = miss ? 0 : run;
+      dd->miss = miss;
+      dd->entry_cap = entry_cap;
+      dd->P = P;
+      dd->box_total = boxes;
+    }
+  }
   int i = blockIdx.x * blockDim.x + threadIdx.x;
   if (i >= P * K) return;
   const int p = i / K, k = i % K;
@@ -1178,12 +1217,19 @@
                                                                  unsigned long long* __restrict__ masks,
                                                                  unsigned* __restrict__ mask_off,
                                                                  const unsigned long long* __restrict__ open_bits,
-                                                                 const int* __restrict__ gate, SweepP sw) {
+                                                                 const int* __restrict__ gate, SweepP sw,
+                                                                 const SliceDescDev* __restrict__ dd ) {
   __shared__ unsigned long long s_words[4][kMaskWords];
   __shared__ unsigned long long s_mid[WAVE_PER_G ? 1 : 4][256];
   const int lane = lane_id();
-  const int j = WAVE_PER_G ? (lane == 0 ? (int)(blockIdx.x * 4 + (threadIdx.x >> 6)) : n_slice)
+  const int n_cap = n_slice;
+  if (dd) n_slice = min(dd->n_slice, n_cap);
+  const int j = WAVE_PER_G ? (lane == 0 ? (int)(blockIdx.x * 4 + (threadIdx.x >> 6)) : n_cap)
                            : (int)(blockIdx.x * 256 + threadIdx.x);
+  if (dd && __ballot(j < n_slice) == 0ull) {
+    if (j < n_cap) counts[j] = 0u;
+    return;
+  }
   if (gate && *gate == 0) {
     if (j < n_slice) counts[j] = 0u;
     return;
@@ -1192,7 +1238,7 @@
   int area = 0;
   Ellipse el = {0.f, 0.f, 1.f, 0.f, 1.f, -1.f, 1.f, 1.f, 0.f, 0.f, 0.f};
   if (j < n_slice) {
-    const int rank = slice_rank(sd, j);
+    const int rank = dd ? slice_rank(dd, j) : slice_rank(sd, j);
     gi = sorted_gi[rank];
     if (masks) { moff = (cum_rank[rank] >> 6) + (unsigned)j; mask_off[j] = moff; }
     const float* rec = records + (size_t)gi * kRecFloats;
@@ -1345,6 +1391,7 @@
     if (lane == src) cnt = c;
   }
   if (j < n_slice) { slice_gi[j] = gi; counts[j] = cnt; }
+  else if (dd && j < n_cap) counts[j] = 0u;
 }
 
 template <bool WAVE_PER_G>
@@ -1358,10 +1405,14 @@
                                                         int W, int H, unsigned invalid_key, int compact,
                                                         const unsigned long long* __restrict__ masks,
                                                         const unsigned* __restrict__ mask_off,
-                                                        unsigned char* __restrict__ tile_hot) {
+                                                        unsigned char* __restrict__ tile_hot,
+                                                        const SliceDescDev* __restrict__ dd) {
   const int lane = lane_id();
+  unsigned e_cap = 0xFFFFFFFFu;
+  if (dd) { n_slice = min(dd->n_slice, n_slice); e_cap = dd->entry_cap; }
   const int j = WAVE_PER_G ? (lane == 0 ? (int)(blockIdx.x * 4 + (threadIdx.x >> 6)) : n_slice)
                            : (int)(blockIdx.x * 256 + threadIdx.x);
+  if (dd && __ballot(j < n_slice) == 0ull) return;
   unsigned cnt = 0, gi = 0, e0 = 0, lo = 0, hi = 0, moff = 0;
   int hot = 0;
   Ellipse el = {0.f, 0.f, 1.f, 0.f, 1.f, -1.f, 1.f, 1.f, 0.f, 0.f, 0.f};
@@ -1393,8 +1444,10 @@
           m &= m - 1;
           const int q = (int)(((float)b + 0.5f) * rw);
           const unsigned k = pbase + (unsigned)((y0 + q) * tiles_x + x0 + (b - q * w));
-          keys[e] = k;
-          vals[e] = gi;
+          if (e < e_cap) {
+            keys[e] = k;
+            vals[e] = gi;
+          }
           if (hot) tile_hot[k] = 1;
           ++e;
         }
@@ -1429,8 +1482,10 @@
           const int tx = x0 + (t - q * w), ty = y0 + q;
           const unsigned dst = e + (unsigned)__popcll(m & lt_mask);
           const unsigned k = pbase + (unsigned)(ty * tiles_x + tx);
-          keys[dst] = k;
-          vals[dst] = g;
+          if (dst < e_cap) {
+            keys[dst] = k;
+            vals[dst] = g;
+          }
           if (hot_g) tile_hot[k] = 1;
         }
         e += (unsigned)__popcll(m);
@@ -1454,8 +1509,10 @@
       const unsigned long long m = __ballot(open);
       if (open) {
         const unsigned dst = e + (unsigned)__popcll(m & lt_mask);
-        keys[dst] = k;
-        vals[dst] = g;
+        if (dst < e_cap) {
+          keys[dst] = k;
+          vals[dst] = g;
+        }
         if (hot_g && (invalid_key == 0u || k != invalid_key)) tile_hot[k] = 1;
       }
       e += (unsigned)__popcll(m);
@@ -1784,16 +1841,30 @@
                             unsigned* tail, void* stream) {
   if (P <= 0 || N <= 0 || K <= 0 || K > 32 || base <= 0) return GS_ERR_INVALID;
   hipLaunchKernelGGL(slice_plan_kernel, dim3((P * K + 63) / 64), dim3(64), 0, (hipStream_t)stream, P, N, K, cum_excl,
-                     total, (unsigned long long)base, bounds, rels, seg_totals, n_live, tail, (const unsigned*)nullptr);
+                     total, (unsigned long long)base, bounds, rels, seg_totals, n_live, tail, (const unsigned*)nullptr,
+                     (SliceDescDev*)nullptr, 0u, 0ull, 0u);
   return gs_launch_status();
 }
 
 GS_EXPORT int gs_slice_plan_select(int P, int N, int K, const unsigned* cum_excl, const unsigned* total, int* bounds,
                                    unsigned* rels, unsigned* seg_totals, const unsigned* n_live, unsigned* tail,
                                    const unsigned* grand, void* stream) {
+  return gs_slice_plan_select_dev(P, N, K, cum_excl, total, bounds, rels, seg_totals, n_live, tail, grand, nullptr, 0, 0, 0,
+                                  stream);
+}
+
+extern "C" int gs_slice_plan_select_dev(int P, int N, int K, const unsigned* cum_excl, const unsigned* total, int* bounds,
+                                        unsigned* rels, unsigned* seg_totals, const unsigned* n_live, unsigned* tail,
+                                        const unsigned* grand, void* desc_dev, long long pair_cap, long long box_cap,
+                                        long long entry_cap, void* stream) {
   if (P <= 0 || N <= 0 || K <= 0 || K > 32 || !n_live || !grand) return GS_ERR_INVALID;
+  if (desc_dev && (P > kMaxSubposes || pair_cap <= 0 || pair_cap > N || box_cap <= 0 || entry_cap <= 0 ||
+                   entry_cap > 0xFFFFFFFFll || !total))
+    return GS_ERR_INVALID;
   hipLaunchKernelGGL(slice_plan_kernel, dim3((P * K + 63) / 64), dim3(64), 0, (hipStream_t)stream, P, N, K, cum_excl,
-                     total, 1ull << 40, bounds, rels, seg_totals, n_live, tail, grand);
+                     total, 1ull << 40, bounds, rels, seg_totals, n_live, tail, grand,
+                     reinterpret_cast<SliceDescDev*>(desc_dev), (unsigned)pair_cap, (unsigned long long)box_cap,
+                     (unsigned)entry_cap);
   return gs_launch_status();
 }
 
@@ -1869,8 +1940,27 @@
                                     unsigned* counts, int wave_per_gaussian, const unsigned* cum_rank,
                                     unsigned long long* hit_masks, unsigned* mask_off,
                                     const unsigned long long* open_bits, const int* gate, void* stream) {
+  return gs_slice_counts_exact_dev(n_slice, P, N, slice_begin, slice_prefix, sorted_gi, records, sat, tile_done, H, W,
+                                   slice_gi, counts, wave_per_gaussian, cum_rank, hit_masks, mask_off, open_bits, gate,
+                                   nullptr, stream);
+}
+
+extern "C" int gs_slice_counts_exact_dev(int n_slice, int P, int N, const int* slice_begin, const int* slice_prefix,
+                                         const unsigned* sorted_gi, const float* records, const int* sat,
+                                         const unsigned char* tile_done, int H, int W, unsigned* slice_gi,
+                                         unsigned* counts, int wave_per_gaussian, const unsigned* cum_rank,
+                                         unsigned long long* hit_masks, unsigned* mask_off,
+                                         const unsigned long long* open_bits, const int* gate, const void* desc_dev,
+                                         void* stream) {
   SliceDesc sd;
-  if (n_slice <= 0 || !make_slice_desc(P, slice_begin, slice_prefix, sd)) return GS_ERR_INVALID;
+  const SliceDescDev* dd = reinterpret_cast<const SliceDescDev*>(desc_dev);
+  if (n_slice <= 0) return GS_ERR_INVALID;
+  if (dd) {
+    if (P <= 0 || P > kMaxSubposes || gate) return GS_ERR_INVALID;
+    sd = SliceDesc{};
+    sd.P = P;
+  }
+  else if (!make_slice_desc(P, slice_begin, slice_prefix, sd)) return GS_ERR_INVALID;
   if (hit_masks && (!cum_rank || !mask_off)) return GS_ERR_INVALID;
   if ((tile_done != nullptr) != (open_bits != nullptr)) return GS_ERR_INVALID;
   int tiles_x = (W + K::kTile - 1) / K::kTile, tiles_y = (H + K::kTile - 1) / K::kTile;
@@ -1878,11 +1968,11 @@
   if (wave_per_gaussian)
     hipLaunchKernelGGL(slice_counts_exact_kernel<true>, dim3((n_slice + 3) / 4), dim3(256), 0, (hipStream_t)stream,
                        n_slice, sd, N, tiles_x, tiles_y, sorted_gi, records, sat, tile_done, W, H, slice_gi, counts,
-                       cum_rank, hit_masks, mask_off, open_bits, gate, none);
+                       cum_rank, hit_masks, mask_off, open_bits, gate, none, dd);
   else
     hipLaunchKernelGGL(slice_counts_exact_kernel<false>, dim3((n_slice + 255) / 256), dim3(256), 0,
                        (hipStream_t)stream, n_slice, sd, N, tiles_x, tiles_y, sorted_gi, records, sat, tile_done, W,
-                       H, slice_gi, counts, cum_rank, hit_masks, mask_off, open_bits, gate, none);
+                       H, slice_gi, counts, cum_rank, hit_masks, mask_off, open_bits, gate, none, dd);
   return gs_launch_status();
 }
 
@@ -1903,11 +1993,13 @@
   if (wave_per_gaussian)
     hipLaunchKernelGGL((slice_counts_exact_kernel<true, true>), dim3((n_slice + 3) / 4), dim3(256), 0, (hipStream_t)stream,
                        n_slice, sd, N, tiles_x, tiles_y, sorted_gi, records, sat, tile_done, W, H, slice_gi, counts,
-                       cum_rank, hit_masks, mask_off, open_bits, (const int*)nullptr, sw);
+                       cum_rank, hit_masks, mask_off, open_bits, (const int*)nullptr, sw,
+                       (const SliceDescDev*)nullptr);
   else
     hipLaunchKernelGGL((slice_counts_exact_kernel<false, true>), dim3((n_slice + 255) / 256), dim3(256), 0,
                        (hipStream_t)stream, n_slice, sd, N, tiles_x, tiles_y, sorted_gi, records, sat, tile_done, W,
-                       H, slice_gi, counts, cum_rank, hit_masks, mask_off, open_bits, (const int*)nullptr, sw);
+                       H, slice_gi, counts, cum_rank, hit_masks, mask_off, open_bits, (const int*)nullptr, sw,
+                       (const SliceDescDev*)nullptr);
   return gs_launch_status();
 }
 
@@ -1917,17 +2009,29 @@
                                       unsigned invalid_key, int compact, int wave_per_gaussian,
                                       const unsigned long long* hit_masks, const unsigned* mask_off,
                                       unsigned char* tile_hot, void* stream) {
+  return gs_emit_open_intersects_dev(n_slice, N, H, W, slice_gi, counts, cum_excl, records, tile_done, keys, vals,
+                                     invalid_key, compact, wave_per_gaussian, hit_masks, mask_off, tile_hot, nullptr,
+                                     stream);
+}
+
+extern "C" int gs_emit_open_intersects_dev(int n_slice, int N, int H, int W, const unsigned* slice_gi,
+                                           const unsigned* counts, const unsigned* cum_excl, const float* records,
+                                           const unsigned char* tile_done, unsigned* keys, unsigned* vals,
+                                           unsigned invalid_key, int compact, int wave_per_gaussian,
+                                           const unsigned long long* hit_masks, const unsigned* mask_off,
+                                           unsigned char* tile_hot, const void* desc_dev, void* stream) {
+  const SliceDescDev* dd = reinterpret_cast<const SliceDescDev*>(desc_dev);
   if (n_slice <= 0) return GS_ERR_INVALID;
   if (hit_masks && (!mask_off || !compact)) return GS_ERR_INVALID;
   int tiles_x = (W + K::kTile - 1) / K::kTile, tiles_y = (H + K::kTile - 1) / K::kTile;
   if (wave_per_gaussian)
     hipLaunchKernelGGL(emit_open_kernel<true>, dim3((n_slice + 3) / 4), dim3(256), 0, (hipStream_t)stream, n_slice, N,
                        tiles_x * tiles_y, tiles_x, slice_gi, counts, cum_excl, records, tile_done, keys, vals, W, H,
-                       invalid_key, compact, hit_masks, mask_off, tile_hot);
+                       invalid_key, compact, hit_masks, mask_off, tile_hot, dd);
   else
     hipLaunchKernelGGL(emit_open_kernel<false>, dim3((n_slice + 255) / 256), dim3(256), 0, (hipStream_t)stream, n_slice,
                        N, tiles_x * tiles_y, tiles_x, slice_gi, counts, cum_excl, records, tile_done, keys, vals, W, H,
-                       invalid_key, compact, hit_masks, mask_off, tile_hot);
+                       invalid_key, compact, hit_masks, mask_off, tile_hot, dd);
   return gs_launch_status();
 }
 
diff --git a/3dgs-deblur_amd/csrc/frame.hip b/3dgs-deblur_amd/csrc/frame.hip
--- a/3dgs-deblur_amd/csrc/frame.hip
+++ b/3dgs-deblur_amd/csrc/frame.hip
@@ -8,12 +8,14 @@
 #include <vector>
 #include "gs_internal.h"
 #include "gs_math.h"
+#include "gs_common.h"
 
 namespace {
 
 constexpr int kTile = gs::K::kTile;
 constexpr int kKMax = GS_FRAME_MAX_SLICES;
 constexpr int kIdsPad = 8;
+constexpr int kSpecMiss = -1;
 
 struct Arena {
   char* base;
@@ -102,6 +104,20 @@
 #endif
 }
 
+inline int wait_words(unsigned* host_pinned, hipStream_t st) {
+  const long long t0 = now_us();
+  unsigned spins = 0;
+  while (__atomic_load_n(host_pinned, __ATOMIC_ACQUIRE) != 1u) {
+    cpu_relax();
+    if ((++spins & 1023u) == 0 && now_us() - t0 > kPollTimeoutUs) {
+      int r = hip_status(hipStreamSynchronize(st));
+      if (r != GS_OK) return r;
+      return __atomic_load_n(host_pinned, __ATOMIC_ACQUIRE) == 1u ? GS_OK : GS_ERR_INVALID;
+    }
+  }
+  return GS_OK;
+}
+
 template <class Between>
 inline int read_back(const unsigned* src_dev, unsigned* host_pinned, int n, bool poll, hipStream_t st, Between between) {
   if (!poll) {
@@ -119,21 +135,50 @@
   if (e != hipSuccess) return 1000 + (int)e;
   int rb = between();
   if (rb != GS_OK) return rb;
-  const long long t0 = now_us();
-  unsigned spins = 0;
-  while (__atomic_load_n(host_pinned, __ATOMIC_ACQUIRE) != 1u) {
-    cpu_relax();
-    if ((++spins & 1023u) == 0 && now_us() - t0 > kPollTimeoutUs) {
-      int r = hip_status(hipStreamSynchronize(st));
-      if (r != GS_OK) return r;
-      return __atomic_load_n(host_pinned, __ATOMIC_ACQUIRE) == 1u ? GS_OK : GS_ERR_INVALID;
-    }
-  }
-  return GS_OK;
+  return wait_words(host_pinned, st);
 }
 
 inline int read_back(const unsigned* src_dev, unsigned* host_pinned, int n, bool poll, hipStream_t st) {
   return read_back(src_dev, host_pinned, n, poll, st, [] { return GS_OK; });
+}
+
+struct PubSrc { const unsigned* p[3]; int n[3]; };
+
+__global__ __launch_bounds__(256) void publish_gather_kernel(PubSrc s, unsigned* dst, unsigned seq) {
+  int off = 1;
+  for (int k = 0; k < 3; ++k) {
+    for (int i = threadIdx.x; i < s.n[k]; i += 256)
+      __hip_atomic_store(dst + off + i, s.p[k][i], __ATOMIC_RELAXED, __HIP_MEMORY_SCOPE_SYSTEM);
+    off += s.n[k];
+  }
+  __threadfence_system();
+  __syncthreads();
+  if (threadIdx.x == 0) __hip_atomic_store(dst, seq, __ATOMIC_RELEASE, __HIP_MEMORY_SCOPE_SYSTEM);
+}
+
+template <class Between>
+inline int read_back_gather(const PubSrc& s, unsigned* host_pinned, bool poll, hipStream_t st, Between between) {
+  if (!poll) {
+    long long off = 1;
+    for (int k = 0; k < 3; ++k) {
+      if (s.n[k] <= 0) continue;
+      hipError_t e = hipMemcpyAsync(host_pinned + off, s.p[k], 4ll * s.n[k], hipMemcpyDeviceToHost, st);
+      if (e != hipSuccess) return 1000 + (int)e;
+      off += s.n[k];
+    }
+    int rb = between();
+    if (rb != GS_OK) return rb;
+    return hip_status(hipStreamSynchronize(st));
+  }
+  volatile unsigned* seqw = host_pinned;
+  *seqw = 0u;
+  __atomic_thread_fence(__ATOMIC_SEQ_CST);
+  hipLaunchKernelGGL(publish_gather_kernel, dim3(1), dim3(256), 0, st, s, host_pinned, 1u);
+  hipError_t e = hipGetLastError();
+  if (e != hipSuccess) return 1000 + (int)e;
+  int rb = between();
+  if (rb != GS_OK) return rb;
+  return wait_words(host_pinned, st);
 }
 
 #define CHECK(call)            \
@@ -267,12 +312,17 @@
   int* plan_dev = A.take<int>(plan_ints);
   unsigned char* tile_done_rs = R > 1 ? A.take<unsigned char>(P * T) : nullptr;
   unsigned char* tile_done_samples = shared ? A.take<unsigned char>((long long)S * T) : nullptr;
+  const long long plan_tiles = (d.band_clipped && R > 1) ? (T + R - 1) / R : T;
+  const long long base0 = plan_tiles * (long long)std::max(1, d.slice_base);
+  const long long pair_cap = std::min<long long>(d.select_cap, N), n_cap = P * pair_cap;
+  const long long I_cap = P * (base0 + 4 * plan_tiles), box_cap = 2 * I_cap;
+  const bool spec = d.spec_plan != 0 && select && d.select_cap > 0 && !pix_vel && !shared && R == 1 && cams == 1 &&
+                    I_cap < 2147483647ll - kIdsPad && box_cap < 4294967296ll - 64 && n_cap < 2147483647ll;
+  void* desc_dev = spec ? static_cast<void*>(A.take<char>((long long)sizeof(gs::SliceDescDev))) : nullptr;
   if (!A.ok) { state->arena_required = 2 * A.off; return GS_ERR_WORKSPACE; }
   if (shared) CHECK(hip_status(hipMemsetAsync(tile_done_samples, 0, (long long)S * T, st)));
   CHECK(hip_status(hipMemsetAsync(zero_blk, 0, sel_b + flag_off + 4 * kKMax, st)));
   int* open_flags = reinterpret_cast<int*>(zeros_u8 + flag_off);
-  const long long plan_tiles = (d.band_clipped && R > 1) ? (T + R - 1) / R : T;
-  const long long base0 = plan_tiles * (long long)std::max(1, d.slice_base);
 
   const unsigned* sorted_gi = nullptr;
   bool bound_known = false;
@@ -315,18 +365,19 @@
   bool use_masks = false, rs_exact = false;
   std::vector<std::vector<int>> begins, prefixes;
   std::vector<long long> n_of, I_of;
-  auto make_plan = [&](int phase) -> int {
+  auto launch_plan = [&](int phase, void* dd) -> int {
+    StageScope sc(ST_PLAN, st);
+    if (select && phase == 0)
+      return gs_slice_plan_select_dev(P, N, kKMax, cum, total, plan_dev, reinterpret_cast<unsigned*>(plan_dev + PK),
+                                      reinterpret_cast<unsigned*>(plan_dev + 2 * PK), n_live,
+                                      reinterpret_cast<unsigned*>(plan_dev + 2 * PK + P), sel_grand, dd, pair_cap, box_cap,
+                                      I_cap, st);
+    return gs_slice_plan(P, N, kKMax, cum, total, phase == 0 ? base0 : 2 * base0, plan_dev,
+                         reinterpret_cast<unsigned*>(plan_dev + PK), reinterpret_cast<unsigned*>(plan_dev + 2 * PK),
+                         n_live, reinterpret_cast<unsigned*>(plan_dev + 2 * PK + P), st);
+  };
+  auto parse_plan = [&](int phase) -> int {
     if (planned) {
-      StageScope sc(ST_PLAN, st);
-      if (select && phase == 0)
-        CHECK(gs_slice_plan_select(P, N, kKMax, cum, total, plan_dev, reinterpret_cast<unsigned*>(plan_dev + PK),
-                                   reinterpret_cast<unsigned*>(plan_dev + 2 * PK), n_live,
-                                   reinterpret_cast<unsigned*>(plan_dev + 2 * PK + P), sel_grand, st));
-      else
-        CHECK(gs_slice_plan(P, N, kKMax, cum, total, phase == 0 ? base0 : 2 * base0, plan_dev,
-                            reinterpret_cast<unsigned*>(plan_dev + PK), reinterpret_cast<unsigned*>(plan_dev + 2 * PK),
-                            n_live, reinterpret_cast<unsigned*>(plan_dev + 2 * PK + P), st));
-      CHECK(read_back(reinterpret_cast<const unsigned*>(plan_dev), hp_seq, (int)plan_ints, poll, st));
       for (int p = 0; p < P; ++p) {
         bnd[p].resize(kKMax); rel[p].resize(kKMax);
         for (int k = 0; k < kKMax; ++k) { bnd[p][k] = hp[p * kKMax + k]; rel[p][k] = hp[PK + p * kKMax + k]; }
@@ -377,21 +428,48 @@
     }
     return GS_OK;
   };
-  CHECK(make_plan(0));
-  if (tail_cap > 0) {
-    long long most = 0;
-    for (int p = 0; p < P; ++p) most = std::max(most, NV[p]);
-    if (most > tail_cap) {
-      state->select_overflow = 1;
-      CHECK(presort(0, 0));
-      CHECK(make_plan(0));
-    }
-  }
-  for (int p = 0; p < P; ++p) state->max_selected = std::max<long long>(state->max_selected, select ? NV[p] : 0);
-  state->n_total = n_total;
-  state->depth_select = select ? 1 : 0;
-  state->open_after_first = -1.f;
-  bool rest_behind = select && ((n_total - true_total) & 0xFFFFFFFFll) != 0;
+  auto make_plan = [&](int phase) -> int {
+    if (planned) {
+      CHECK(launch_plan(phase, nullptr));
+      CHECK(read_back(reinterpret_cast<const unsigned*>(plan_dev), hp_seq, (int)plan_ints, poll, st));
+    }
+    return parse_plan(phase);
+  };
+  bool rest_behind = false;
+  auto plan_known = [&]() {
+    state->max_selected = 0;
+    for (int p = 0; p < P; ++p) state->max_selected = std::max<long long>(state->max_selected, select ? NV[p] : 0);
+    state->n_total = n_total;
+    state->depth_select = select ? 1 : 0;
+    state->open_after_first = -1.f;
+    rest_behind = select && ((n_total - true_total) & 0xFFFFFFFFll) != 0;
+  };
+  auto plan_first = [&]() -> int {
+    CHECK(make_plan(0));
+    if (tail_cap > 0) {
+      long long most = 0;
+      for (int p = 0; p < P; ++p) most = std::max(most, NV[p]);
+      if (most > tail_cap) {
+        state->select_overflow = 1;
+        CHECK(presort(0, 0));
+        CHECK(make_plan(0));
+      }
+    }
+    plan_known();
+    return GS_OK;
+  };
+  const long long off_presort = A.off;
+  if (spec) {
+    CHECK(launch_plan(0, desc_dev));
+    K = 1;
+    use_masks = true; rs_exact = false;
+    true_total = box_cap;
+    rest_behind = true;
+    state->depth_select = 1;
+    state->open_after_first = -1.f;
+  } else {
+    CHECK(plan_first());
+  }
 
   long long maxI_issued = 0;
   auto fits = [&](long long n_s, long long I_s, int k_next) -> bool {
@@ -430,6 +508,9 @@
   const unsigned invalid_key = rs ? 0u : (unsigned)(P * T);
   const int key_bits = bits_for(P * T + 1);
   int n_out = 0;
+  auto issue = [&](const bool ahead) -> int {
+  n_out = 0;
+  maxI_issued = 0;
   int span = 1;
   long long open_before = (long long)S * T;
   std::vector<int> beg_s, pre_s;
@@ -440,8 +521,17 @@
   for (int k = 0, k1 = 0; k < K; k = k1, ++slice_no) {
     long long n_k = 0, I_k = 0;
     k1 = std::min(K, k + span);
-    merged(k, k1, beg_s, pre_s, n_k, I_k);
-    while (k1 > k + 1 && I_k >= 2147483647ll - kIdsPad) merged(k, --k1, beg_s, pre_s, n_k, I_k);
+    const bool ahead_k = ahead && slice_no == 0;
+    const void* dd = ahead_k ? desc_dev : nullptr;
+    if (ahead_k) {
+      beg_s.assign(P, 0);
+      pre_s.assign(P + 1, 0);
+      for (int p = 0; p < P; ++p) { beg_s[p] = (int)((long long)p * N); pre_s[p + 1] = pre_s[p] + (int)pair_cap; }
+      n_k = n_cap; I_k = I_cap;
+    } else {
+      merged(k, k1, beg_s, pre_s, n_k, I_k);
+      while (k1 > k + 1 && I_k >= 2147483647ll - kIdsPad) merged(k, --k1, beg_s, pre_s, n_k, I_k);
+    }
     const bool first = slice_no == 0, last = k1 == K && !(phase == 0 && rest_behind);
     if (I_k >= 2147483647ll - kIdsPad) return GS_ERR_INVALID;
     if (shared && I_k * (long long)S >= 4294967296ll) return GS_ERR_INVALID;
@@ -465,6 +555,7 @@
         else for (int p = 0; p < P; ++p) box_total += rel[p][0];
       }
       wave_per_g = (first && box_total > 128 * n_k) ? 1 : 0;
+      if (ahead_k) wave_per_g = d.spec_wave_per_g != 0 ? 1 : 0;
       if (use_masks) {
         masks = A.take<unsigned long long>(true_total / 64 + n_k + 2);
         mask_off = A.take<unsigned>(n_k);
@@ -476,7 +567,8 @@
       if (!A.ok) { state->arena_required = 2 * A.off; return GS_ERR_WORKSPACE; }
       if (lazy && !lazy_done) {
         if (slice_no == 0)
-          CHECK(gs_slice_project_records((int)n_k, P, N, beg_s.data(), pre_s.data(), sorted_gi, lazy, H, W, records, st));
+          CHECK(gs_slice_project_records_dev((int)n_k, P, N, beg_s.data(), pre_s.data(), sorted_gi, lazy, H, W, records,
+                                             dd, st));
         else {
           CHECK(gs_project_records(P, N, lazy, H, W, records, st));
           lazy_done = true;
@@ -492,14 +584,14 @@
         CHECK(gs_slice_counts((int)n_k, P, N, beg_s.data(), pre_s.data(), sorted_gi, records,
                               have_holes ? sat : nullptr, H, W, slice_gi, counts, st));
       else
-        CHECK(gs_slice_counts_exact((int)n_k, P, N, beg_s.data(), pre_s.data(), sorted_gi, records,
-                                    have_holes ? sat : nullptr, have_holes ? tile_done : nullptr, H, W, slice_gi, counts,
-                                    wave_per_g, masks ? cum : nullptr, masks, mask_off, have_holes ? open_bits : nullptr,
-                                    nullptr, st));
+        CHECK(gs_slice_counts_exact_dev((int)n_k, P, N, beg_s.data(), pre_s.data(), sorted_gi, records,
+                                        have_holes ? sat : nullptr, have_holes ? tile_done : nullptr, H, W, slice_gi,
+                                        counts, wave_per_g, masks ? cum : nullptr, masks, mask_off,
+                                        have_holes ? open_bits : nullptr, nullptr, dd, st));
       CHECK(gs_exclusive_scan_u32(n_k, counts, cum_k, total_k, ws, ws_b, st));
       if (color_means && color_sh && color_viewmats)
-        CHECK(gs_slice_colors((int)n_k, slice_gi, counts, N, color_means, color_sh, color_sh_rest, color_K, color_degree,
-                              color_viewmats, records, st));
+        CHECK(gs_slice_colors_dev((int)n_k, slice_gi, counts, N, color_means, color_sh, color_sh_rest, color_K,
+                                  color_degree, color_viewmats, records, dd, st));
     }
     if (I_k > 0) {
       unsigned* keys = A.take<unsigned>(I_k);
@@ -518,9 +610,10 @@
         if (rs && !rs_exact && first && !holes0)
           CHECK(gs_emit_intersects(n_k, N, H, W, slice_gi, cum_k, records, I_k, keys, vals, invalid_key, st));
         else
-          CHECK(gs_emit_open_intersects((int)n_k, N, H, W, slice_gi, counts, cum_k, records,
-                                        (!first || holes0) ? tile_done : nullptr, keys, vals, invalid_key,
-                                        (rs && !rs_exact) ? 0 : 1, wave_per_g, masks, mask_off, rs ? nullptr : tile_hot, st));
+          CHECK(gs_emit_open_intersects_dev((int)n_k, N, H, W, slice_gi, counts, cum_k, records,
+                                            (!first || holes0) ? tile_done : nullptr, keys, vals, invalid_key,
+                                            (rs && !rs_exact) ? 0 : 1, wave_per_g, masks, mask_off,
+                                            rs ? nullptr : tile_hot, dd, st));
       }
       int r1 = 0, r2 = 0;
       {
@@ -582,8 +675,35 @@
     };
     if (last) CHECK(average());
     if (!last) {
-      CHECK(read_back(reinterpret_cast<const unsigned*>(open_flags + slice_no), hp_seq, 1, poll, st, average));
-      const long long open_now = hp[0];
+      long long open_now = 0;
+      if (!ahead_k) {
+        CHECK(read_back(reinterpret_cast<const unsigned*>(open_flags + slice_no), hp_seq, 1, poll, st, average));
+        open_now = hp[0];
+      } else {
+        const PubSrc src{{reinterpret_cast<const unsigned*>(plan_dev), reinterpret_cast<const unsigned*>(open_flags),
+                          total_k}, {(int)plan_ints, 1, 1}};
+        CHECK(read_back_gather(src, hp_seq, poll, st, average));
+        open_now = hp[plan_ints];
+        const long long emitted = hp[plan_ints + 1];
+        CHECK(parse_plan(0));
+        plan_known();
+        int why = 0;
+        for (int p = 0; p < P; ++p) if (NV[p] > tail_cap) why |= 1;
+        if (K != 1 || n_of[0] <= 0 || I_of[0] <= 0 || !rest_behind) why |= 8;
+        if (!(why & 9)) {
+          if (((I_of[0] > 128 * n_of[0]) ? 1 : 0) != wave_per_g) why |= 2;
+          if (emitted > I_cap || I_of[0] > box_cap || !use_masks || I_of[0] >= 2147483647ll - kIdsPad) why |= 4;
+        }
+        if (why) { state->spec_plan_why = why; return kSpecMiss; }
+        state->spec_plan = 1;
+        gs_frame_slice& sl = state->slice[n_out - 1];
+        sl.I = I_of[0]; sl.n = (int)n_of[0];
+        maxI_issued = I_of[0];
+        if (d.reserve_backward) {
+          const long long need = Arena::up(A.off) + Arena::up(48 * sl.I) + Arena::up(sl.I) + 2 * Arena::up(4ll * S * H * W) + 1024;
+          if (need > arena_bytes) { state->arena_required = need; return GS_ERR_WORKSPACE; }
+        }
+      }
       open_left = open_now;
       if (slice_no == 0) state->open_after_first = (float)((double)open_now / (double)((long long)S * T));
       if (open_now == 0) { ++slice_no; break; }
@@ -604,6 +724,17 @@
   CHECK(presort(1, 0));
   CHECK(make_plan(1));
   }
+  return GS_OK;
+  };
+  int rc = issue(spec);
+  if (rc == kSpecMiss) {
+    state->spec_plan_miss = 1;
+    A.off = off_presort;
+    CHECK(hip_status(hipMemsetAsync(zeros_u8, 0, flag_off + 4 * kKMax, st)));
+    CHECK(plan_first());
+    rc = issue(false);
+  }
+  if (rc != GS_OK) return rc;
   state->n_slices = n_out;
   state->arena_used = Arena::up(A.off);
   return GS_OK;
diff --git a/3dgs-deblur_amd/csrc/gs_common.h b/3dgs-deblur_amd/csrc/gs_common.h
--- a/3dgs-deblur_amd/csrc/gs_common.h
+++ b/3dgs-deblur_amd/csrc/gs_common.h
@@ -84,4 +84,20 @@
   return sd.begin[p] + (j - sd.prefix[p]);
 }
 
+struct SliceDescDev {
+  int n_slice;
+  int miss;
+  unsigned entry_cap;
+  int P;
+  unsigned long long box_total;
+  int begin[kMaxSubposes];
+  int prefix[kMaxSubposes + 1];
+};
+
+__device__ __forceinline__ int slice_rank(const SliceDescDev* __restrict__ dd, int j) {
+  int p = 0;
+  while (p + 1 < dd->P && j >= dd->prefix[p + 1]) ++p;
+  return dd->begin[p] + (j - dd->prefix[p]);
 }
+
+}
diff --git a/3dgs-deblur_amd/csrc/gs_internal.h b/3dgs-deblur_amd/csrc/gs_internal.h
--- a/3dgs-deblur_amd/csrc/gs_internal.h
+++ b/3dgs-deblur_amd/csrc/gs_internal.h
@@ -34,6 +34,30 @@
                                                const float* cmb_scale, float cmb_gamma, float cmb_min_level,
                                                const float* pix_vel, int N, float rolling_shutter_time,
                                                const float* shared_list_times, const float* v_depth, void* stream);
+extern "C" int gs_slice_plan_select_dev(int P, int N, int K, const unsigned* cum_excl, const unsigned* total, int* bounds,
+                                        unsigned* rels, unsigned* seg_totals, const unsigned* n_live, unsigned* tail,
+                                        const unsigned* grand, void* desc_dev, long long pair_cap, long long box_cap,
+                                        long long entry_cap, void* stream);
+extern "C" int gs_slice_project_records_dev(int n_slice, int P, int N, const int* slice_begin, const int* slice_prefix,
+                                            const unsigned* sorted_gi, const struct gs_project_inputs* in, int H, int W,
+                                            float* records, const void* desc_dev, void* stream);
+extern "C" int gs_slice_counts_exact_dev(int n_slice, int P, int N, const int* slice_begin, const int* slice_prefix,
+                                         const unsigned* sorted_gi, const float* records, const int* sat,
+                                         const unsigned char* tile_done, int H, int W, unsigned* slice_gi,
+                                         unsigned* counts, int wave_per_gaussian, const unsigned* cum_rank,
+                                         unsigned long long* hit_masks, unsigned* mask_off,
+                                         const unsigned long long* open_bits, const int* gate, const void* desc_dev,
+                                         void* stream);
+extern "C" int gs_slice_colors_dev(int n_slice, const unsigned* slice_gi, const unsigned* counts, int N,
+                                   const float* means, const float* sh, const float* sh_rest, int K_stride,
+                                   int sh_degree, const float* viewmats, float* records, const void* desc_dev,
+                                   void* stream);
+extern "C" int gs_emit_open_intersects_dev(int n_slice, int N, int H, int W, const unsigned* slice_gi,
+                                           const unsigned* counts, const unsigned* cum_excl, const float* records,
+                                           const unsigned char* tile_done, unsigned* keys, unsigned* vals,
+                                           unsigned invalid_key, int compact, int wave_per_gaussian,
+                                           const unsigned long long* hit_masks, const unsigned* mask_off,
+                                           unsigned char* tile_hot, const void* desc_dev, void* stream);
 extern "C" int gs_reduce_grad_tuples_depth(int n_slice, const unsigned* slice_gi, const unsigned* counts,
                                            const unsigned* cum_excl, const float* tuples, const unsigned char* flags,
                                            float* v_records, unsigned char* touched, long long n_isect,
diff --git a/3dgs-deblur_amd/csrc/project.hip b/3dgs-deblur_amd/csrc/project.hip
--- a/3dgs-deblur_amd/csrc/project.hip
+++ b/3dgs-deblur_amd/csrc/project.hip
@@ -884,10 +884,12 @@
 }
 
 __global__ __launch_bounds__(256) void slice_records_kernel(int n_slice, SliceDesc sd, const unsigned* __restrict__ sorted_gi,
-                                                            FusedParams fp, float* __restrict__ records) {
+                                                            FusedParams fp, float* __restrict__ records,
+                                                            const SliceDescDev* __restrict__ dd ) {
   const int j = blockIdx.x * 256 + threadIdx.x;
+  if (dd) n_slice = min(dd->n_slice, n_slice);
   if (j >= n_slice) return;
-  const unsigned gi = sorted_gi[slice_rank(sd, j)];
+  const unsigned gi = sorted_gi[dd ? slice_rank(dd, j) : slice_rank(sd, j)];
   const int p = (int)(gi / (unsigned)fp.N), i = (int)(gi - (unsigned)p * (unsigned)fp.N);
   float m[3] = {fp.means[3 * i], fp.means[3 * i + 1], fp.means[3 * i + 2]};
   float sc[3];
@@ -936,7 +938,12 @@
                                                            const float* __restrict__ sh,
                                                            const float* __restrict__ sh_rest, int K_stride, int deg,
                                                            const float* __restrict__ viewmats,
-                                                           float* __restrict__ records) {
+                                                           float* __restrict__ records,
+                                                           const SliceDescDev* __restrict__ dd ) {
+  if (dd) {
+    n_slice = min(dd->n_slice, n_slice);
+    if ((int)(blockIdx.x * blockDim.x) >= n_slice) return;
+  }
   constexpr int kRow = MAXB * 3 + 1;
   constexpr int kRowPad = (kRow & 1) ? kRow : kRow + 1;
   __shared__ float s_coef[slice_colors_waves<MAXB>()][64 * kRowPad];
@@ -1143,16 +1150,28 @@
 GS_EXPORT int gs_slice_project_records(int n_slice, int P, int N, const int* slice_begin, const int* slice_prefix,
                                        const unsigned* sorted_gi, const gs_project_inputs* in, int H, int W,
                                        float* records, void* stream) {
+  return gs_slice_project_records_dev(n_slice, P, N, slice_begin, slice_prefix, sorted_gi, in, H, W, records, nullptr,
+                                      stream);
+}
+
+extern "C" int gs_slice_project_records_dev(int n_slice, int P, int N, const int* slice_begin, const int* slice_prefix,
+                                            const unsigned* sorted_gi, const gs_project_inputs* in, int H, int W,
+                                            float* records, const void* desc_dev, void* stream) {
   SliceDesc sd;
-  if (n_slice <= 0 || N <= 0 || !in || !sorted_gi || !records || !make_slice_desc(P, slice_begin, slice_prefix, sd))
-    return GS_ERR_INVALID;
+  const SliceDescDev* dd = reinterpret_cast<const SliceDescDev*>(desc_dev);
+  if (n_slice <= 0 || N <= 0 || !in || !sorted_gi || !records) return GS_ERR_INVALID;
+  if (dd) {
+    if (P <= 0 || P > kMaxSubposes) return GS_ERR_INVALID;
+    sd = SliceDesc{};
+    sd.P = P;
+  } else if (!make_slice_desc(P, slice_begin, slice_prefix, sd)) return GS_ERR_INVALID;
   if (!in->means || !in->scales || !in->quats || !in->opacities || !in->viewmats) return GS_ERR_INVALID;
   FusedParams fp = make_fused(N, P, in->means, in->scales, in->glob_scale, in->quats, in->opacities, nullptr, 1, 0,
                               in->viewmats, in->fx, in->fy, in->cx, in->cy, H, W, in->clip_thresh, in->antialiased,
                               in->defer_color | 1);
   fp.act = in->param_flags;
   hipLaunchKernelGGL(slice_records_kernel, dim3((n_slice + 255) / 256), dim3(256), 0, (hipStream_t)stream, n_slice, sd,
-                     sorted_gi, fp, records);
+                     sorted_gi, fp, records, dd);
   return gs_launch_status();
 }
 
@@ -1170,13 +1189,21 @@
 GS_EXPORT int gs_slice_colors(int n_slice, const unsigned* slice_gi, const unsigned* counts, int N,
                               const float* means, const float* sh, const float* sh_rest, int K_stride, int sh_degree,
                               const float* viewmats, float* records, void* stream) {
+  return gs_slice_colors_dev(n_slice, slice_gi, counts, N, means, sh, sh_rest, K_stride, sh_degree, viewmats, records,
+                             nullptr, stream);
+}
+
+extern "C" int gs_slice_colors_dev(int n_slice, const unsigned* slice_gi, const unsigned* counts, int N,
+                                   const float* means, const float* sh, const float* sh_rest, int K_stride,
+                                   int sh_degree, const float* viewmats, float* records, const void* desc_dev,
+                                   void* stream) {
   if (n_slice <= 0 || N <= 0 || sh_degree < 0 || sh_degree > 4 || (sh_degree + 1) * (sh_degree + 1) > K_stride)
     return GS_ERR_INVALID;
   const bool low = sh_degree <= 3;
   const int th = 64 * (low ? slice_colors_waves<16>() : slice_colors_waves<25>());
   hipLaunchKernelGGL(low ? slice_colors_kernel<16> : slice_colors_kernel<25>, dim3((n_slice + th - 1) / th), dim3(th), 0,
                      (hipStream_t)stream, n_slice, slice_gi, counts, N, means, sh, sh_rest, K_stride, sh_degree, viewmats,
-                     records);
+                     records, reinterpret_cast<const SliceDescDev*>(desc_dev));
   return gs_launch_status();
 }
 
diff --git a/3dgs-deblur_amd/ops.py b/3dgs-deblur_amd/ops.py
--- a/3dgs-deblur_amd/ops.py
+++ b/3dgs-deblur_amd/ops.py
@@ -28,7 +28,8 @@
 class FrameHints:
 
     __slots__ = ("mult", "age", "arena_bytes", "arena_retries", "frames", "box_share", "last_slices", "select_misses",
-                 "select_cap", "select_overflows", "_recent", "_lock", "_views")
+                 "select_cap", "select_overflows", "spec_wave", "spec_hold", "spec_plans", "spec_plan_misses", "_recent",
+                 "_lock", "_views")
 
     def __init__(self):
         self.mult, self.age, self.arena_bytes, self.arena_retries, self.frames = 1, 0, 0, 0, 0
@@ -37,6 +38,10 @@
         self.select_misses = 0
         self.select_cap = 0
         self.select_overflows = 0
+        self.spec_wave = None
+        self.spec_hold = False
+        self.spec_plans = 0
+        self.spec_plan_misses = 0
         self._recent = []
         self._lock = threading.Lock()
         self._views = {}
@@ -44,8 +49,12 @@
     def slice_base(self) -> int:
         return SLICE_BASE * (self.mult if SLICE_ADAPT and SLICE_BASE > 0 else 1)
 
+    def spec_promise(self) -> Optional[int]:
+        return _spec_promise(self)
+
     def feedback(self, n_issued: int, retries: int = 0, box_share: Optional[float] = None, select_state: int = 0,
-                 open_after_first: Optional[float] = None, max_selected: int = 0, select_overflow: int = 0) -> None:
+                 open_after_first: Optional[float] = None, max_selected: int = 0, select_overflow: int = 0,
+                 first_wave: Optional[int] = None, spec_plan: int = 0, spec_plan_miss: int = 0) -> None:
         with self._lock:
             self.frames += 1
             self.last_slices = int(n_issued)
@@ -55,6 +64,9 @@
                 want = int(1.5 * max_selected) + 4096
                 self.select_cap = want if (select_overflow or want > self.select_cap) else max(want, int(0.9 * self.select_cap))
             self.select_overflows += int(bool(select_overflow))
+            _spec_feedback(self, first_wave, spec_plan_miss)
+            self.spec_plans += int(bool(spec_plan))
+            self.spec_plan_misses += int(bool(spec_plan_miss))
             if box_share is not None:
                 self.box_share = float(box_share)
             self.arena_retries += retries
@@ -88,22 +100,25 @@
                     self._views.clear()
                 v = self._views[key] = ViewHints(self)
                 v.box_share, v.last_slices, v.select_cap = self.box_share, self.last_slices, self.select_cap
+                v.spec_wave = self.spec_wave
             return v
 
     def reset(self) -> None:
         with self._lock:
             self.mult, self.age, self.arena_bytes, self._recent, self.box_share = 1, 0, 0, [], None
             self.last_slices, self.select_cap = None, 0
+            self.spec_wave, self.spec_hold = None, False
             self._views.clear()
 
 
 class ViewHints:
 
-    __slots__ = ("scene", "box_share", "last_slices", "select_cap")
+    __slots__ = ("scene", "box_share", "last_slices", "select_cap", "spec_wave", "spec_hold")
 
     def __init__(self, scene: "FrameHints"):
         self.scene = scene
         self.box_share, self.last_slices, self.select_cap = None, None, 0
+        self.spec_wave, self.spec_hold = None, False
 
     arena_bytes = property(lambda self: self.scene.arena_bytes,
                            lambda self, v: setattr(self.scene, "arena_bytes", v))
@@ -112,6 +127,8 @@
     arena_retries = property(lambda self: self.scene.arena_retries)
     select_misses = property(lambda self: self.scene.select_misses)
     select_overflows = property(lambda self: self.scene.select_overflows)
+    spec_plans = property(lambda self: self.scene.spec_plans)
+    spec_plan_misses = property(lambda self: self.scene.spec_plan_misses)
     settled = property(lambda self: self.scene.settled)
 
     def slice_base(self) -> int:
@@ -126,17 +143,34 @@
     def view(self, key) -> "ViewHints":
         return self.scene.view(key)
 
+    def spec_promise(self) -> Optional[int]:
+        return _spec_promise(self)
+
     def feedback(self, n_issued: int, retries: int = 0, box_share: Optional[float] = None, select_state: int = 0,
-                 open_after_first: Optional[float] = None, max_selected: int = 0, select_overflow: int = 0) -> None:
+                 open_after_first: Optional[float] = None, max_selected: int = 0, select_overflow: int = 0,
+                 first_wave: Optional[int] = None, spec_plan: int = 0, spec_plan_miss: int = 0) -> None:
         sc = self.scene
         with sc._lock:
+            _spec_feedback(self, first_wave, spec_plan_miss)
             self.last_slices = int(n_issued)
             if box_share is not None:
                 self.box_share = float(box_share)
             if max_selected > 0:
                 want = int(1.5 * max_selected) + 4096
                 self.select_cap = want if (select_overflow or want > self.select_cap) else max(want, int(0.9 * self.select_cap))
-        sc.feedback(n_issued, retries, box_share, select_state, open_after_first, max_selected, select_overflow)
+        sc.feedback(n_issued, retries, box_share, select_state, open_after_first, max_selected, select_overflow,
+                    first_wave, spec_plan, spec_plan_miss)
+
+
+def _spec_promise(h) -> Optional[int]:
+    if h.spec_hold or h.spec_wave is None or h.select_cap <= 0:
+        return None
+    return int(h.spec_wave)
+
+
+def _spec_feedback(h, first_wave: Optional[int], spec_plan_miss: int) -> None:
+    h.spec_wave = None if first_wave is None else int(bool(first_wave))
+    h.spec_hold = bool(spec_plan_miss)
 
 
 _hints = {}
@@ -182,6 +216,7 @@
 BAND_AWARE = int(os.environ.get("GSD_BAND_AWARE", "1"))
 LAZY_RECORDS = int(os.environ.get("GSD_LAZY_RECORDS", "1"))
 DEPTH_SELECT = int(os.environ.get("GSD_DEPTH_SELECT", "1"))
+SPEC_PLAN = int(os.environ.get("GSD_SPEC_PLAN", "1"))
 NEEDLE_HP = int(os.environ.get("GSD_NEEDLE_HP", "1"))
 
 
@@ -216,6 +251,7 @@
 profiler: Optional[StageProfiler] = None
 last_num_intersects: int = 0
 last_depth_select: int = 0
+last_spec_plan: tuple = (0, 0, 0)
 
 
 def _stage(name: str):
@@ -441,7 +477,9 @@
                                                                                      ("sweep_t_min", ctypes.c_float),
                                                                                      ("sweep_t_max", ctypes.c_float),
                                                                                      ("lazy_records", ctypes.c_void_p),
-                                                                                     ("cameras", ctypes.c_int)]
+                                                                                     ("cameras", ctypes.c_int),
+                                                                                     ("spec_plan", ctypes.c_int),
+                                                                                     ("spec_wave_per_g", ctypes.c_int)]
 
 
 class _ProjectInputs(ctypes.Structure):
@@ -461,7 +499,8 @@
                 [("rolling_shutter_time", ctypes.c_float), ("shared_list", ctypes.c_int), ("depth_select", ctypes.c_int),
                  ("select_overflow", ctypes.c_int), ("open_after_first", ctypes.c_float)] +
                 [(k, ctypes.c_longlong) for k in ("n_total", "max_selected", "arena_used", "arena_required")] +
-                [("slice", _FrameSlice * 16), ("cameras", ctypes.c_int)])
+                [("slice", _FrameSlice * 16), ("cameras", ctypes.c_int), ("spec_plan", ctypes.c_int),
+                 ("spec_plan_miss", ctypes.c_int), ("spec_plan_why", ctypes.c_int)])
 
 
 def _box_share(state) -> Optional[float]:
@@ -655,7 +694,7 @@
                          out_depth: Optional[Tensor] = None, reserve_backward: bool = True, rs=None, combine=None,
                          hints: Optional[FrameHints] = None, band_clipped: bool = False, lazy=None,
                          depth_select: Optional[bool] = None, cameras: int = 1):
-    global last_num_intersects, _slice_totals, last_depth_select
+    global last_num_intersects, _slice_totals, last_depth_select, last_spec_plan
     L = _L()
     dev = records.device
     tx, ty = _tiles(H, W)
@@ -664,6 +703,10 @@
         hints = hints_for((str(dev), N, P, S, H, W, shared))
     if depth_select is None:
         depth_select = bool(DEPTH_SELECT == 2 or (DEPTH_SELECT and hints.depth_select()))
+    spec = None
+    if (SPEC_PLAN and depth_select and slice_base > 0 and rs is None and R == 1 and cameras == 1
+            and hints.select_cap > 0):
+        spec = hints.spec_promise()
     n = P * N
     nbytes = hints.arena_bytes
     if not nbytes:
@@ -683,7 +726,8 @@
                       int(bool(band_clipped)), int(bool(depth_select and slice_base > 0)),
                       int(min(hints.select_cap, 2 ** 31 - 1)) if depth_select else 0,
                       float(rs[3][0]) if shared and len(rs) > 3 else 0.0, float(rs[3][1]) if shared and len(rs) > 3 else 0.0,
-                      ctypes.addressof(lazy) if lazy is not None else None, int(cameras))
+                      ctypes.addressof(lazy) if lazy is not None else None, int(cameras), int(spec is not None),
+                      int(spec or 0))
     state = _FrameState()
     out_img = torch.empty(S, H, W, 3, device=dev)
     out_T = torch.empty(S, H, W, device=dev)
@@ -707,6 +751,7 @@
                             int((state.arena_used + L.gs_frame_backward_bytes(ctypes.byref(state))) * 1.15))
     last_num_intersects = int(state.n_total)
     last_depth_select = int(state.depth_select)
+    last_spec_plan = (int(state.spec_plan), int(state.spec_plan_miss), int(state.spec_plan_why))
     _slice_totals = [arena[sl.n_emitted_dev:sl.n_emitted_dev + 4].view(torch.int32)
                      for sl in (state.slice[i] for i in range(state.n_slices))]
     return out_img, out_T, dict(arena=arena, arena_obj=lease.arena, lease=lease, gen=lease.gen, state=state,
@@ -1286,7 +1331,11 @@
                                                              averaged, hints, bool(defer_flags & 4), lazy, cameras=B)
                 st = frame["state"]
                 hints.feedback(int(st.n_slices), retries, _box_share(st), int(st.depth_select),
-                               float(st.open_after_first), int(st.max_selected), int(st.select_overflow))
+                               float(st.open_after_first), int(st.max_selected), int(st.select_overflow),
+                               int(st.slice[0].wave_per_gaussian)
+                               if (st.depth_select and st.n_slices > 0 and st.slice[0].first
+                                   and int(st.slice[0].I) < int(st.n_total)) else None,
+                               int(st.spec_plan), int(st.spec_plan_miss))
                 break
             except _ArenaTooSmall:
                 retries += 1
diff --git a/include/gsdeblur.h b/include/gsdeblur.h
--- a/include/gsdeblur.h
+++ b/include/gsdeblur.h
@@ -339,6 +339,8 @@
   float sweep_t_min, sweep_t_max;
   const struct gs_project_inputs* lazy_records;
   int cameras;
+  int spec_plan;
+  int spec_wave_per_g;
 } gs_frame_desc;
 typedef struct gs_frame_slice {
   long long I;
@@ -358,6 +360,9 @@
   long long arena_required;
   gs_frame_slice slice[GS_FRAME_MAX_SLICES];
   int cameras;
+  int spec_plan;
+  int spec_plan_miss;
+  int spec_plan_why;
 } gs_frame_state;
 int gs_frame_forward(const gs_frame_desc* desc, float* records, unsigned* depth_keys, const int* num_tiles_hit,
                      const float* background , const int* band_edges , const unsigned char* band_tile_done,
```

Result: no change. 1235 (-0.0%).
